# ziyaad30/ForwardTacotron

Hardware: AMD Instinct MI355X
Metric: mel_frames_per_sec_train_step (higher is better)
Workload: dtype f32

## Files before the change

forwardtacotron_amd/csrc/ft_bn.hip:

```cpp
#include <string.h>

#include "ft_common.h"

namespace {

__device__ __forceinline__ int tvalid_of(int c, int Tbuf, int group) {
  return (group > 0 && (((c / group) + 1) & 1)) ? Tbuf - 1 : Tbuf;
}

struct BnAff4 { float4 mu, rs, ga, be; };
__device__ __forceinline__ float4 bn_z4(const float4& v, const BnAff4& a) {
  float4 o;
  o.x = (v.x - a.mu.x) * a.rs.x * a.ga.x + a.be.x;
  o.y = (v.y - a.mu.y) * a.rs.y * a.ga.y + a.be.y;
  o.z = (v.z - a.mu.z) * a.rs.z * a.ga.z + a.be.z;
  o.w = (v.w - a.mu.w) * a.rs.w * a.ga.w + a.be.w;
  return o;
}
__device__ __forceinline__ float4 pool_grad4(const float* __restrict__ yrow, const float* __restrict__ drow,
                                             const float4& vt, int t, int Tout, int C, const BnAff4& a) {
  const float4 z = bn_z4(vt, a);
  const float4 d0 = *reinterpret_cast<const float4*>(drow);
  float4 g;
  if (t == 0) {
    g = d0;
  } else {
    const float4 p = bn_z4(*reinterpret_cast<const float4*>(yrow - C), a);
    g.x = z.x > p.x ? d0.x : 0.f;
    g.y = z.y > p.y ? d0.y : 0.f;
    g.z = z.z > p.z ? d0.z : 0.f;
    g.w = z.w > p.w ? d0.w : 0.f;
  }
  if (t + 1 < Tout) {
    const float4 n = bn_z4(*reinterpret_cast<const float4*>(yrow + C), a);
    const float4 d1 = *reinterpret_cast<const float4*>(drow + C);
    g.x += !(n.x > z.x) ? d1.x : 0.f;
    g.y += !(n.y > z.y) ? d1.y : 0.f;
    g.z += !(n.z > z.z) ? d1.z : 0.f;
    g.w += !(n.w > z.w) ? d1.w : 0.f;
  }
  return g;
}

template <int MODE>
__global__ __launch_bounds__(256) void ft_col_partial_kernel(const float* __restrict__ y, long ldy,
                                                             const float* __restrict__ dout,
                                                             const float* __restrict__ mean,
                                                             const float* __restrict__ rstd, int B, int Tbuf, int Tout,
                                                             int C, int group, int rows_per_chunk,
                                                             double* __restrict__ partial) {
  __shared__ double red[2][4][64];
  const int cl = threadIdx.x & 63, rl = threadIdx.x >> 6;
  const int c = blockIdx.x * 64 + cl;
  const long rows = (long)B * Tbuf;
  long r0 = (long)blockIdx.y * rows_per_chunk;
  long r1 = r0 + rows_per_chunk;
  if (r1 > rows) r1 = rows;
  double s0 = 0.0, s1 = 0.0;
  if (c < C) {
    const int tv = tvalid_of(c, Tbuf, group);
    float mu = 0.f, rs = 0.f;
    if (MODE == 1) {
      mu = mean[c];
      rs = rstd[c];
    }
    long r = r0 + rl;
    int b = (int)(r / Tbuf);
    int t = (int)(r - (long)b * Tbuf);
    for (; r < r1; r += 4) {
      if (t < tv) {
        float v = y[r * ldy + c];
        if (MODE == 0) {
          s0 += (double)v;
          s1 += (double)v * (double)v;
        } else if (MODE == 1) {
          if (t < Tout) {
            float g = dout[((long)b * Tout + t) * C + c];
            s0 += (double)g;
            s1 += (double)g * (double)((v - mu) * rs);
          }
        } else {
          s0 += (double)v;
        }
      }
      t += 4;
      while (t >= Tbuf) {
        t -= Tbuf;
        ++b;
      }
    }
  }
  red[0][rl][cl] = s0;
  red[1][rl][cl] = s1;
  __syncthreads();
  if (rl == 0 && c < C) {
    double a0 = red[0][0][cl] + red[0][1][cl] + red[0][2][cl] + red[0][3][cl];
    double a1 = red[1][0][cl] + red[1][1][cl] + red[1][2][cl] + red[1][3][cl];
    partial[((long)blockIdx.y * C + c) * 2 + 0] = a0;
    partial[((long)blockIdx.y * C + c) * 2 + 1] = a1;
  }
}

__global__ __launch_bounds__(256) void ft_colsum4_partial_kernel(const float* __restrict__ x, long ldx, long rows, int C,
                                                                 int rows_per_chunk, double* __restrict__ partial,
                                                                 const float* __restrict__ x1) {
  if (x1) {
    if (blockIdx.z == 1) x = x1;
  }
  const int slot = x1 ? (int)blockIdx.z : 0;
  __shared__ double red[16][65];
  const int cq = threadIdx.x & 15, rl = threadIdx.x >> 4;
  const int c = blockIdx.x * 64 + cq * 4;
  const long r0 = (long)blockIdx.y * rows_per_chunk;
  long r1 = r0 + rows_per_chunk;
  if (r1 > rows) r1 = rows;
  double s[4] = {0.0, 0.0, 0.0, 0.0};
  if (c < C) {
    for (long r = r0 + rl; r < r1; r += 64) {
      float4 v[4];
#pragma unroll
      for (int u = 0; u < 4; ++u) {
        const long rr = r + 16 * u;
        v[u] = rr < r1 ? *reinterpret_cast<const float4*>(x + rr * ldx + c) : make_float4(0.f, 0.f, 0.f, 0.f);
      }
#pragma unroll
      for (int u = 0; u < 4; ++u) {
        s[0] += (double)v[u].x;
        s[1] += (double)v[u].y;
        s[2] += (double)v[u].z;
        s[3] += (double)v[u].w;
      }
    }
  }
#pragma unroll
  for (int e = 0; e < 4; ++e) red[rl][cq * 4 + e] = s[e];
  __syncthreads();
  if (threadIdx.x < 64) {
    const int cc = blockIdx.x * 64 + threadIdx.x;
    if (cc < C) {
      double a = 0.0;
#pragma unroll
      for (int i = 0; i < 16; ++i) a += red[i][threadIdx.x];
      partial[((long)blockIdx.y * C + cc) * 2 + slot] = a;
      if (!x1) partial[((long)blockIdx.y * C + cc) * 2 + 1] = 0.0;
    }
  }
}

template <int MODE>
__global__ __launch_bounds__(256) void ft_col_partial4_kernel(const float* __restrict__ y, const float* __restrict__ dout,
                                                              const float* __restrict__ mean,
                                                              const float* __restrict__ rstd, int B, int Tbuf, int Tout,
                                                              int C, int group, int rows_per_chunk,
                                                              double* __restrict__ partial,
                                                              const float* __restrict__ gamma = nullptr,
                                                              const float* __restrict__ beta = nullptr) {
  __shared__ double red[2][16][65];
  const int cq = threadIdx.x & 15, rl = threadIdx.x >> 4;
  const int c = blockIdx.x * 64 + cq * 4;
  const long rows = (long)B * Tbuf;
  const long r0 = (long)blockIdx.y * rows_per_chunk;
  long r1 = r0 + rows_per_chunk;
  if (r1 > rows) r1 = rows;
  double s0[4] = {0.0, 0.0, 0.0, 0.0}, s1[4] = {0.0, 0.0, 0.0, 0.0};
  if (c < C) {
    const int tv = tvalid_of(c, Tbuf, group);
    float4 mu = make_float4(0.f, 0.f, 0.f, 0.f), rs = mu;
    BnAff4 aff;
    if (MODE >= 1) {
      mu = *reinterpret_cast<const float4*>(mean + c);
      rs = *reinterpret_cast<const float4*>(rstd + c);
    }
    if (MODE == 2) {
      aff.mu = mu;
      aff.rs = rs;
      aff.ga = *reinterpret_cast<const float4*>(gamma + c);
      aff.be = *reinterpret_cast<const float4*>(beta + c);
    }
    int bb[4], tt[4];
#pragma unroll
    for (int u = 0; u < 4; ++u) {
      const long r = r0 + rl + 16 * u;
      bb[u] = (int)(r / Tbuf);
      tt[u] = (int)(r - (long)bb[u] * Tbuf);
    }
    for (long r = r0 + rl; r < r1; r += 64) {
      float4 v[4], g[4];
      bool ok[4];
#pragma unroll
      for (int u = 0; u < 4; ++u) {
        const long rr = r + 16 * u;
        ok[u] = rr < r1 && tt[u] < tv && (MODE == 0 || tt[u] < Tout);
        v[u] = ok[u] ? *reinterpret_cast<const float4*>(y + rr * C + c) : make_float4(0.f, 0.f, 0.f, 0.f);
        if (MODE == 1)
          g[u] = ok[u] ? *reinterpret_cast<const float4*>(dout + ((long)bb[u] * Tout + tt[u]) * C + c)
                       : make_float4(0.f, 0.f, 0.f, 0.f);
        if (MODE == 2)
          g[u] = ok[u] ? pool_grad4(y + rr * C + c, dout + ((long)bb[u] * Tout + tt[u]) * C + c, v[u], tt[u], Tout, C, aff)
                       : make_float4(0.f, 0.f, 0.f, 0.f);
      }
#pragma unroll
      for (int u = 0; u < 4; ++u) {
        if (MODE == 0) {
          s0[0] += (double)v[u].x; s1[0] += (double)v[u].x * (double)v[u].x;
          s0[1] += (double)v[u].y; s1[1] += (double)v[u].y * (double)v[u].y;
          s0[2] += (double)v[u].z; s1[2] += (double)v[u].z * (double)v[u].z;
          s0[3] += (double)v[u].w; s1[3] += (double)v[u].w * (double)v[u].w;
        } else if (ok[u]) {
          s0[0] += (double)g[u].x; s1[0] += (double)g[u].x * (double)((v[u].x - mu.x) * rs.x);
          s0[1] += (double)g[u].y; s1[1] += (double)g[u].y * (double)((v[u].y - mu.y) * rs.y);
          s0[2] += (double)g[u].z; s1[2] += (double)g[u].z * (double)((v[u].z - mu.z) * rs.z);
          s0[3] += (double)g[u].w; s1[3] += (double)g[u].w * (double)((v[u].w - mu.w) * rs.w);
        }
        tt[u] += 64;
        while (tt[u] >= Tbuf) {
          tt[u] -= Tbuf;
          ++bb[u];
        }
      }
    }
  }
#pragma unroll
  for (int e = 0; e < 4; ++e) {
    red[0][rl][cq * 4 + e] = s0[e];
    red[1][rl][cq * 4 + e] = s1[e];
  }
  __syncthreads();
  if (threadIdx.x < 64) {
    const int cc = blockIdx.x * 64 + threadIdx.x;
    if (cc < C) {
      double a0 = 0.0, a1 = 0.0;
#pragma unroll
      for (int i = 0; i < 16; ++i) {
        a0 += red[0][i][threadIdx.x];
        a1 += red[1][i][threadIdx.x];
      }
      partial[((long)blockIdx.y * C + cc) * 2 + 0] = a0;
      partial[((long)blockIdx.y * C + cc) * 2 + 1] = a1;
    }
  }
}

constexpr int FIN_PARTS = 8;
__device__ __forceinline__ void sum_partials(const double* __restrict__ partial, int nchunks, int C, int c, int part,
                                             double (*sh)[FIN_PARTS][2], int slot, double& s0, double& s1) {
  double a0 = 0.0, a1 = 0.0;
  if (c < C) {
    const int per = (nchunks + FIN_PARTS - 1) / FIN_PARTS;
    const int i0 = part * per, i1 = min(nchunks, i0 + per);
    for (int i = i0; i < i1; ++i) {
      a0 += partial[((long)i * C + c) * 2 + 0];
      a1 += partial[((long)i * C + c) * 2 + 1];
    }
  }
  sh[slot][part][0] = a0;
  sh[slot][part][1] = a1;
  __syncthreads();
  s0 = 0.0;
  s1 = 0.0;
  if (part == 0) {
#pragma unroll
    for (int p = 0; p < FIN_PARTS; ++p) {
      s0 += sh[slot][p][0];
      s1 += sh[slot][p][1];
    }
  }
}

__global__ __launch_bounds__(256) void ft_bn_finalize_kernel(const double* __restrict__ partial, int nchunks, int B,
                                                             int Tbuf, int C, int group, float momentum, float eps,
                                                             float* __restrict__ running_mean,
                                                             float* __restrict__ running_var, long* __restrict__ nbt,
                                                             float* __restrict__ save_mean,
                                                             float* __restrict__ save_rstd) {
  __shared__ double sh[32][FIN_PARTS][2];
  const int slot = threadIdx.x >> 3, part = threadIdx.x & 7;
  const int c = blockIdx.x * 32 + slot;
  if (blockIdx.x == 0 && threadIdx.x == 0 && nbt) *nbt += 1;
  double s0, s1;
  sum_partials(partial, nchunks, C, c, part, sh, slot, s0, s1);
  if (part != 0 || c >= C) return;
  double n = (double)B * (double)tvalid_of(c, Tbuf, group);
  double mu = s0 / n;
  double var = s1 / n - mu * mu;
  if (var < 0.0) var = 0.0;
  save_mean[c] = (float)mu;
  save_rstd[c] = (float)(1.0 / sqrt(var + (double)eps));
  if (running_mean) {
    double unb = n > 1.0 ? var * n / (n - 1.0) : var;
    running_mean[c] = (float)((1.0 - momentum) * (double)running_mean[c] + momentum * mu);
    running_var[c] = (float)((1.0 - momentum) * (double)running_var[c] + momentum * unb);
  }
}

__global__ __launch_bounds__(256) void ft_col_finalize_kernel(const double* __restrict__ partial, int nchunks, int C,
                                                              float* __restrict__ out0, float* __restrict__ out1,
                                                              float scale0, int accumulate) {
  __shared__ double sh[32][FIN_PARTS][2];
  const int slot = threadIdx.x >> 3, part = threadIdx.x & 7;
  const int c = blockIdx.x * 32 + slot;
  double s0, s1;
  sum_partials(partial, nchunks, C, c, part, sh, slot, s0, s1);
  if (part != 0 || c >= C) return;
  if (out0) out0[c] = (accumulate ? out0[c] : 0.f) + (float)(s0 * scale0);
  if (out1) out1[c] = (accumulate ? out1[c] : 0.f) + (float)s1;
}

__global__ __launch_bounds__(256) void ft_bn_apply_kernel(const float* __restrict__ y, const float* __restrict__ mean,
                                                          const float* __restrict__ rstd,
                                                          const float* __restrict__ gamma,
                                                          const float* __restrict__ beta,
                                                          const float* __restrict__ residual, float* __restrict__ out,
                                                          int B, int Tbuf, int Tout, int C) {
  long idx = (long)blockIdx.x * blockDim.x + threadIdx.x;
  long total = (long)B * Tout * C;
  if (idx >= total) return;
  int c = (int)(idx % C);
  long row = idx / C;
  int b = (int)(row / Tout), t = (int)(row - (long)b * Tout);
  float v = y[((long)b * Tbuf + t) * C + c];
  float o = (v - mean[c]) * rstd[c] * gamma[c] + beta[c];
  if (residual) o += residual[idx];
  out[idx] = o;
}

__global__ __launch_bounds__(256) void ft_bn_bwd_apply_kernel(const float* __restrict__ dout, const float* __restrict__ y,
                                                              const float* __restrict__ mean,
                                                              const float* __restrict__ rstd,
                                                              const float* __restrict__ gamma,
                                                              const float* __restrict__ dgamma,
                                                              const float* __restrict__ dbeta, float* __restrict__ dy,
                                                              int B, int Tbuf, int Tout, int C, int group, int relu) {
  long idx = (long)blockIdx.x * blockDim.x + threadIdx.x;
  long total = (long)B * Tbuf * C;
  if (idx >= total) return;
  int c = (int)(idx % C);
  long row = idx / C;
  int b = (int)(row / Tbuf), t = (int)(row - (long)b * Tbuf);
  int tv = tvalid_of(c, Tbuf, group);
  float r = 0.f;
  if (t < tv) {
    float v = y[idx];
    float g = t < Tout ? dout[((long)b * Tout + t) * C + c] : 0.f;
    float inv_n = 1.0f / ((float)B * (float)tv);
    float xh = (v - mean[c]) * rstd[c];
    r = gamma[c] * rstd[c] * (g - dbeta[c] * inv_n - xh * dgamma[c] * inv_n);
    if (relu && !(v > 0.f)) r = 0.f;
  }
  dy[idx] = r;
}

__global__ __launch_bounds__(256) void ft_bn_apply4_kernel(const float4* __restrict__ y, const float4* __restrict__ mean,
                                                           const float4* __restrict__ rstd,
                                                           const float4* __restrict__ gamma,
                                                           const float4* __restrict__ beta,
                                                           const float4* __restrict__ residual, float4* __restrict__ out,
                                                           long total4, int Tbuf, int Tout, int C4) {
  const long idx = (long)blockIdx.x * blockDim.x + threadIdx.x;
  if (idx >= total4) return;
  const int c = (int)(idx % C4);
  const long row = idx / C4;
  const int b = (int)(row / Tout), t = (int)(row - (long)b * Tout);
  const float4 v = y[((long)b * Tbuf + t) * C4 + c];
  const float4 mu = mean[c], rs = rstd[c], ga = gamma[c], be = beta[c];
  float4 o;
  o.x = (v.x - mu.x) * rs.x * ga.x + be.x;
  o.y = (v.y - mu.y) * rs.y * ga.y + be.y;
  o.z = (v.z - mu.z) * rs.z * ga.z + be.z;
  o.w = (v.w - mu.w) * rs.w * ga.w + be.w;
  if (residual) {
    const float4 r = residual[idx];
    o.x += r.x; o.y += r.y; o.z += r.z; o.w += r.w;
  }
  out[idx] = o;
}

__global__ __launch_bounds__(256) void ft_bn_apply_pool4_kernel(const float* __restrict__ y, const float* __restrict__ mean,
                                                                const float* __restrict__ rstd,
                                                                const float* __restrict__ gamma,
                                                                const float* __restrict__ beta, float4* __restrict__ out,
                                                                long total4, int Tbuf, int Tout, int C) {
  const long idx = (long)blockIdx.x * blockDim.x + threadIdx.x;
  if (idx >= total4) return;
  const int C4 = C / 4;
  const int c = (int)(idx % C4) * 4;
  const long row = idx / C4;
  const int b = (int)(row / Tout), t = (int)(row - (long)b * Tout);
  BnAff4 a;
  a.mu = *reinterpret_cast<const float4*>(mean + c);
  a.rs = *reinterpret_cast<const float4*>(rstd + c);
  a.ga = *reinterpret_cast<const float4*>(gamma + c);
  a.be = *reinterpret_cast<const float4*>(beta + c);
  const float* yrow = y + ((long)b * Tbuf + t) * C + c;
  float4 z = bn_z4(*reinterpret_cast<const float4*>(yrow), a);
  if (t > 0) {
    const float4 p = bn_z4(*reinterpret_cast<const float4*>(yrow - C), a);
    z.x = z.x > p.x ? z.x : p.x;
    z.y = z.y > p.y ? z.y : p.y;
    z.z = z.z > p.z ? z.z : p.z;
    z.w = z.w > p.w ? z.w : p.w;
  }
  out[idx] = z;
}

template <bool POOL>
__global__ __launch_bounds__(256) void ft_bn_bwd_apply4_kernel(const float4* __restrict__ dout, const float4* __restrict__ y,
                                                               const float4* __restrict__ mean,
                                                               const float4* __restrict__ rstd,
                                                               const float4* __restrict__ gamma,
                                                               const float4* __restrict__ dgamma,
                                                               const float4* __restrict__ dbeta, float4* __restrict__ dy,
                                                               long total4, int B, int Tbuf, int Tout, int C4, int group,
                                                               int relu, const float4* __restrict__ beta = nullptr) {
  const long idx = (long)blockIdx.x * blockDim.x + threadIdx.x;
  if (idx >= total4) return;
  const int c = (int)(idx % C4);
  const long row = idx / C4;
  const int b = (int)(row / Tbuf), t = (int)(row - (long)b * Tbuf);
  const int tv = tvalid_of(4 * c, Tbuf, group);
  float4 r = make_float4(0.f, 0.f, 0.f, 0.f);
  if (t < tv) {
    const float4 v = y[idx];
    const float4 mu = mean[c], rs = rstd[c], ga = gamma[c], dg = dgamma[c], db = dbeta[c];
    float4 g = make_float4(0.f, 0.f, 0.f, 0.f);
    if (t < Tout) {
      if constexpr (POOL) {
        BnAff4 a;
        a.mu = mu; a.rs = rs; a.ga = ga; a.be = beta[c];
        g = pool_grad4(reinterpret_cast<const float*>(y + idx), reinterpret_cast<const float*>(dout + ((long)b * Tout + t) * C4 + c),
                       v, t, Tout, 4 * C4, a);
      } else {
        g = dout[((long)b * Tout + t) * C4 + c];
      }
    }
    const float inv_n = 1.0f / ((float)B * (float)tv);
#define FT_BN_BWD1(f)                                                                \
  {                                                                                  \
    const float xh = (v.f - mu.f) * rs.f;                                            \
    r.f = ga.f * rs.f * (g.f - db.f * inv_n - xh * dg.f * inv_n);                    \
    if (relu && !(v.f > 0.f)) r.f = 0.f;                                             \
  }
    FT_BN_BWD1(x) FT_BN_BWD1(y) FT_BN_BWD1(z) FT_BN_BWD1(w)
#undef FT_BN_BWD1
  }
  dy[idx] = r;
}

__global__ void ft_bn_fold_kernel(const float* gamma, const float* beta, const float* rm, const float* rv, float eps,
                                  float* scale, float* shift, int C) {
  int c = blockIdx.x * blockDim.x + threadIdx.x;
  if (c >= C) return;
  float s = gamma[c] / sqrtf(rv[c] + eps);
  scale[c] = s;
  shift[c] = beta[c] - rm[c] * s;
}

template <typename... P>
bool all16(P... ptrs) {
  return (((uintptr_t)(const void*)ptrs % 16 == 0) && ...);
}

constexpr int CSB_MAX = 16;
struct ColsumBatch {
  const float* x[CSB_MAX];
  float* out[CSB_MAX];
  long ld[CSB_MAX], ws_off[CSB_MAX];
  int C[CSB_MAX], nchunks[CSB_MAX], rpc[CSB_MAX];
  int tile64[CSB_MAX + 1], tile32[CSB_MAX + 1];
  int n;
  long rows;
};

__global__ __launch_bounds__(256) void ft_colsum_batch_partial_kernel(ColsumBatch b, double* __restrict__ ws) {
  int t = 0;
  while (t + 1 < b.n && (int)blockIdx.x >= b.tile64[t + 1]) ++t;
  if ((int)blockIdx.y >= b.nchunks[t]) return;
  const float* __restrict__ x = b.x[t];
  const long ldx = b.ld[t];
  const int C = b.C[t];
  double* __restrict__ partial = ws + b.ws_off[t];
  __shared__ double red[16][65];
  const int cq = threadIdx.x & 15, rl = threadIdx.x >> 4;
  const int tile = blockIdx.x - b.tile64[t];
  const int c = tile * 64 + cq * 4;
  const long r0 = (long)blockIdx.y * b.rpc[t];
  long r1 = r0 + b.rpc[t];
  if (r1 > b.rows) r1 = b.rows;
  double s[4] = {0.0, 0.0, 0.0, 0.0};
  if (c < C) {
    for (long r = r0 + rl; r < r1; r += 64) {
      float4 v[4];
#pragma unroll
      for (int u = 0; u < 4; ++u) {
        const long rr = r + 16 * u;
        v[u] = rr < r1 ? *reinterpret_cast<const float4*>(x + rr * ldx + c) : make_float4(0.f, 0.f, 0.f, 0.f);
      }
#pragma unroll
      for (int u = 0; u < 4; ++u) {
        s[0] += (double)v[u].x;
        s[1] += (double)v[u].y;
        s[2] += (double)v[u].z;
        s[3] += (double)v[u].w;
      }
    }
  }
#pragma unroll
  for (int e = 0; e < 4; ++e) red[rl][cq * 4 + e] = s[e];
  __syncthreads();
  if (threadIdx.x < 64) {
    const int cc = tile * 64 + threadIdx.x;
    if (cc < C) {
      double a = 0.0;
#pragma unroll
      for (int i = 0; i < 16; ++i) a += red[i][threadIdx.x];
      partial[((long)blockIdx.y * C + cc) * 2] = a;
      partial[((long)blockIdx.y * C + cc) * 2 + 1] = 0.0;
    }
  }
}

__global__ __launch_bounds__(256) void ft_colsum_batch_finalize_kernel(ColsumBatch b, const double* __restrict__ ws) {
  int t = 0;
  while (t + 1 < b.n && (int)blockIdx.x >= b.tile32[t + 1]) ++t;
  __shared__ double sh[32][FIN_PARTS][2];
  const int slot = threadIdx.x >> 3, part = threadIdx.x & 7;
  const int c = (blockIdx.x - b.tile32[t]) * 32 + slot;
  double s0, s1;
  sum_partials(ws + b.ws_off[t], b.nchunks[t], b.C[t], c, part, sh, slot, s0, s1);
  if (part != 0 || c >= b.C[t]) return;
  b.out[t][c] = (float)s0;
}

struct ChunkPlan {
  int nchunks, rows_per_chunk;
};
ChunkPlan plan_chunks(long rows, int C) {
  int cb = ft_cdiv(C, 64);
  long want = 1024 / (cb > 0 ? cb : 1);
  if (want < 16) want = 16;
  if (want > 64) want = 64;
  long maxc = (rows + 63) / 64;
  if (maxc < 1) maxc = 1;
  long n = want < maxc ? want : maxc;
  if (n > 65535) n = 65535;
  long rpc = (rows + n - 1) / n;
  rpc = ((rpc + 3) / 4) * 4;
  if (rpc < 4) rpc = 4;
  n = (rows + rpc - 1) / rpc;
  if (n < 1) n = 1;
  ChunkPlan p = {(int)n, (int)rpc};
  return p;
}

}

int ft_bn_stat_partials(const float* y, int B, int Tbuf, int C, int group, double* partial, hipStream_t s) {
  ChunkPlan p = plan_chunks((long)B * Tbuf, C);
  if (C % 4 == 0 && (group == 0 || group % 4 == 0) && all16(y))
    hipLaunchKernelGGL(ft_col_partial4_kernel<0>, dim3(ft_cdiv(C, 64), p.nchunks), dim3(256), 0, s, y, nullptr, nullptr,
                       nullptr, B, Tbuf, Tbuf, C, group, p.rows_per_chunk, partial);
  else
    hipLaunchKernelGGL(ft_col_partial_kernel<0>, dim3(ft_cdiv(C, 64), p.nchunks), dim3(256), 0, s, y, (long)C, nullptr,
                       nullptr, nullptr, B, Tbuf, Tbuf, C, group, p.rows_per_chunk, partial);
  return p.nchunks;
}

extern "C" {

size_t ft_bn_workspace(int B, int Tbuf, int C);

size_t ft_conv_stats_workspace(int B, int Tbuf, int C) {
  const size_t tiles = (size_t)ft_cdiv((long)B * Tbuf, 128) * C * 2 * sizeof(double);
  const size_t chunks = ft_bn_workspace(B, Tbuf, C);
  return tiles > chunks ? tiles : chunks;
}

int ft_bn_train_from_partials(const double* partial, int nchunks, const float* y, const float* gamma, const float* beta,
                              const float* residual, float* out, float* running_mean, float* running_var,
                              long* num_batches_tracked, float* save_mean, float* save_rstd, int B, int Tbuf, int Tout,
                              int C, int group, float momentum, float eps, void* stream) {
  FT_REQUIRE(B > 0 && Tbuf > 0 && C > 0 && Tout <= Tbuf && nchunks >= 1, "bn_train_from_partials: bad dims");
  hipStream_t s = (hipStream_t)stream;
  hipLaunchKernelGGL(ft_bn_finalize_kernel, dim3(ft_cdiv(C, 32)), dim3(256), 0, s, partial, nchunks, B, Tbuf, C, group,
                     momentum, eps, running_mean, running_var, num_batches_tracked, save_mean, save_rstd);
  if (out && Tout > 0) {
    long total = (long)B * Tout * C;
    if (C % 4 == 0 && all16(y, save_mean, save_rstd, gamma, beta, residual, out))
      hipLaunchKernelGGL(ft_bn_apply4_kernel, dim3(ft_cdiv(total / 4, 256)), dim3(256), 0, s, (const float4*)y,
                         (const float4*)save_mean, (const float4*)save_rstd, (const float4*)gamma, (const float4*)beta,
                         (const float4*)residual, (float4*)out, total / 4, Tbuf, Tout, C / 4);
    else
      hipLaunchKernelGGL(ft_bn_apply_kernel, dim3(ft_cdiv(total, 256)), dim3(256), 0, s, y, save_mean, save_rstd, gamma,
                         beta, residual, out, B, Tbuf, Tout, C);
  }
  return ft_check_launch("bn_train_from_partials");
}

size_t ft_bn_workspace(int B, int Tbuf, int C) {
  ChunkPlan p = plan_chunks((long)B * Tbuf, C);
  return (size_t)p.nchunks * C * 2 * sizeof(double);
}

int ft_bn_train_fwd(const float* y, const float* gamma, const float* beta, const float* residual, float* out,
                    float* running_mean, float* running_var, long* num_batches_tracked, float* save_mean,
                    float* save_rstd, int B, int Tbuf, int Tout, int C, int group, float momentum, float eps,
                    void* workspace, size_t workspace_bytes, void* stream) {
  FT_REQUIRE(B > 0 && Tbuf > 0 && C > 0 && Tout <= Tbuf, "bn_train_fwd: bad dims");
  FT_REQUIRE(workspace && workspace_bytes >= ft_bn_workspace(B, Tbuf, C), "bn_train_fwd: workspace too small");
  hipStream_t s = (hipStream_t)stream;
  ChunkPlan p = plan_chunks((long)B * Tbuf, C);
  if (C % 4 == 0 && (group == 0 || group % 4 == 0) && all16(y))
    hipLaunchKernelGGL(ft_col_partial4_kernel<0>, dim3(ft_cdiv(C, 64), p.nchunks), dim3(256), 0, s, y, nullptr, nullptr,
                       nullptr, B, Tbuf, Tout, C, group, p.rows_per_chunk, (double*)workspace);
  else
    hipLaunchKernelGGL(ft_col_partial_kernel<0>, dim3(ft_cdiv(C, 64), p.nchunks), dim3(256), 0, s, y, (long)C, nullptr,
                       nullptr, nullptr, B, Tbuf, Tout, C, group, p.rows_per_chunk, (double*)workspace);
  hipLaunchKernelGGL(ft_bn_finalize_kernel, dim3(ft_cdiv(C, 32)), dim3(256), 0, s, (const double*)workspace,
                     p.nchunks, B, Tbuf, C, group, momentum, eps, running_mean, running_var, num_batches_tracked,
                     save_mean, save_rstd);
  if (out && Tout > 0) {
    long total = (long)B * Tout * C;
    if (C % 4 == 0 && all16(y, save_mean, save_rstd, gamma, beta, residual, out))
      hipLaunchKernelGGL(ft_bn_apply4_kernel, dim3(ft_cdiv(total / 4, 256)), dim3(256), 0, s, (const float4*)y,
                         (const float4*)save_mean, (const float4*)save_rstd, (const float4*)gamma, (const float4*)beta,
                         (const float4*)residual, (float4*)out, total / 4, Tbuf, Tout, C / 4);
    else
      hipLaunchKernelGGL(ft_bn_apply_kernel, dim3(ft_cdiv(total, 256)), dim3(256), 0, s, y, save_mean, save_rstd, gamma,
                         beta, residual, out, B, Tbuf, Tout, C);
  }
  return ft_check_launch("bn_train_fwd");
}

int ft_bn_bwd(const float* dout, const float* y, const float* gamma, const float* save_mean, const float* save_rstd,
              float* dy, float* dgamma, float* dbeta, int B, int Tbuf, int Tout, int C, int group, int relu,
              void* workspace, size_t workspace_bytes, void* stream) {
  FT_REQUIRE(B > 0 && Tbuf > 0 && C > 0 && Tout <= Tbuf, "bn_bwd: bad dims");
  FT_REQUIRE(workspace && workspace_bytes >= ft_bn_workspace(B, Tbuf, C), "bn_bwd: workspace too small");
  hipStream_t s = (hipStream_t)stream;
  ChunkPlan p = plan_chunks((long)B * Tbuf, C);
  if (C % 4 == 0 && (group == 0 || group % 4 == 0) && all16(y, dout, save_mean, save_rstd))
    hipLaunchKernelGGL(ft_col_partial4_kernel<1>, dim3(ft_cdiv(C, 64), p.nchunks), dim3(256), 0, s, y, dout, save_mean,
                       save_rstd, B, Tbuf, Tout, C, group, p.rows_per_chunk, (double*)workspace);
  else
    hipLaunchKernelGGL(ft_col_partial_kernel<1>, dim3(ft_cdiv(C, 64), p.nchunks), dim3(256), 0, s, y, (long)C, dout,
                       save_mean, save_rstd, B, Tbuf, Tout, C, group, p.rows_per_chunk, (double*)workspace);
  hipLaunchKernelGGL(ft_col_finalize_kernel, dim3(ft_cdiv(C, 32)), dim3(256), 0, s, (const double*)workspace,
                     p.nchunks, C, dbeta, dgamma, 1.0f, 0);
  long total = (long)B * Tbuf * C;
  if (C % 4 == 0 && (group == 0 || group % 4 == 0) && all16(dout, y, save_mean, save_rstd, gamma, dgamma, dbeta, dy))
    hipLaunchKernelGGL(ft_bn_bwd_apply4_kernel<false>, dim3(ft_cdiv(total / 4, 256)), dim3(256), 0, s, (const float4*)dout,
                       (const float4*)y, (const float4*)save_mean, (const float4*)save_rstd, (const float4*)gamma,
                       (const float4*)dgamma, (const float4*)dbeta, (float4*)dy, total / 4, B, Tbuf, Tout, C / 4, group,
                       relu, nullptr);
  else
    hipLaunchKernelGGL(ft_bn_bwd_apply_kernel, dim3(ft_cdiv(total, 256)), dim3(256), 0, s, dout, y, save_mean, save_rstd,
                       gamma, dgamma, dbeta, dy, B, Tbuf, Tout, C, group, relu);
  return ft_check_launch("bn_bwd");
}

int ft_bn_pool_from_partials(const double* partial, int nchunks, const float* y, const float* gamma, const float* beta,
                             float* out, float* running_mean, float* running_var, long* num_batches_tracked,
                             float* save_mean, float* save_rstd, int B, int Tbuf, int Tout, int C, int group,
                             float momentum, float eps, void* stream) {
  FT_REQUIRE(B > 0 && Tbuf > 0 && C > 0 && Tout > 0 && Tout <= Tbuf && nchunks >= 1, "bn_pool_from_partials: bad dims");
  FT_REQUIRE(C % 4 == 0 && (group == 0 || group % 4 == 0) && all16(y, save_mean, save_rstd, gamma, beta, out),
             "bn_pool_from_partials: needs C %% 4 == 0 and 16-byte aligned buffers");
  hipStream_t s = (hipStream_t)stream;
  hipLaunchKernelGGL(ft_bn_finalize_kernel, dim3(ft_cdiv(C, 32)), dim3(256), 0, s, partial, nchunks, B, Tbuf, C, group,
                     momentum, eps, running_mean, running_var, num_batches_tracked, save_mean, save_rstd);
  const long total = (long)B * Tout * C;
  hipLaunchKernelGGL(ft_bn_apply_pool4_kernel, dim3(ft_cdiv(total / 4, 256)), dim3(256), 0, s, y, save_mean, save_rstd,
                     gamma, beta, (float4*)out, total / 4, Tbuf, Tout, C);
  return ft_check_launch("bn_pool_from_partials");
}

int ft_bn_pool_bwd(const float* dout, const float* y, const float* gamma, const float* beta, const float* save_mean,
                   const float* save_rstd, float* dy, float* dgamma, float* dbeta, int B, int Tbuf, int Tout, int C,
                   int group, int relu, void* workspace, size_t workspace_bytes, void* stream) {
  FT_REQUIRE(B > 0 && Tbuf > 0 && C > 0 && Tout > 0 && Tout <= Tbuf, "bn_pool_bwd: bad dims");
  FT_REQUIRE(workspace && workspace_bytes >= ft_bn_workspace(B, Tbuf, C), "bn_pool_bwd: workspace too small");
  FT_REQUIRE(C % 4 == 0 && (group == 0 || group % 4 == 0) &&
                 all16(dout, y, save_mean, save_rstd, gamma, beta, dgamma, dbeta, dy),
             "bn_pool_bwd: needs C %% 4 == 0 and 16-byte aligned buffers");
  hipStream_t s = (hipStream_t)stream;
  ChunkPlan p = plan_chunks((long)B * Tbuf, C);
  hipLaunchKernelGGL(ft_col_partial4_kernel<2>, dim3(ft_cdiv(C, 64), p.nchunks), dim3(256), 0, s, y, dout, save_mean,
                     save_rstd, B, Tbuf, Tout, C, group, p.rows_per_chunk, (double*)workspace, gamma, beta);
  hipLaunchKernelGGL(ft_col_finalize_kernel, dim3(ft_cdiv(C, 32)), dim3(256), 0, s, (const double*)workspace,
                     p.nchunks, C, dbeta, dgamma, 1.0f, 0);
  const long total = (long)B * Tbuf * C;
  hipLaunchKernelGGL(ft_bn_bwd_apply4_kernel<true>, dim3(ft_cdiv(total / 4, 256)), dim3(256), 0, s, (const float4*)dout,
                     (const float4*)y, (const float4*)save_mean, (const float4*)save_rstd, (const float4*)gamma,
                     (const float4*)dgamma, (const float4*)dbeta, (float4*)dy, total / 4, B, Tbuf, Tout, C / 4, group, relu,
                     (const float4*)beta);
  return ft_check_launch("bn_pool_bwd");
}

int ft_bn_fold_eval(const float* gamma, const float* beta, const float* running_mean, const float* running_var,
                    float eps, float* scale, float* shift, int C, void* stream) {
  if (C <= 0) return FT_OK;
  hipLaunchKernelGGL(ft_bn_fold_kernel, dim3(ft_cdiv(C, 128)), dim3(128), 0, (hipStream_t)stream, gamma, beta,
                     running_mean, running_var, eps, scale, shift, C);
  return ft_check_launch("bn_fold_eval");
}

size_t ft_colsum_workspace(int rows, int C) { return ft_bn_workspace(1, rows > 0 ? rows : 1, C > 0 ? C : 1); }

int ft_colsum(const float* x, long ldx, float* out, int rows, int C, float scale, int accumulate, void* workspace,
              size_t workspace_bytes, void* stream) {
  FT_REQUIRE(rows >= 0 && C >= 0, "colsum: bad dims");
  if (C == 0) return FT_OK;
  hipStream_t s = (hipStream_t)stream;
  if (rows == 0) {
    if (!accumulate) (void)hipMemsetAsync(out, 0, sizeof(float) * C, s);
    return FT_OK;
  }
  FT_REQUIRE(workspace && workspace_bytes >= ft_colsum_workspace(rows, C), "colsum: workspace too small");
  ChunkPlan p = plan_chunks(rows, C);
  if (C % 4 == 0 && ldx % 4 == 0 && ((uintptr_t)x) % 16 == 0)
    hipLaunchKernelGGL(ft_colsum4_partial_kernel, dim3(ft_cdiv(C, 64), p.nchunks), dim3(256), 0, s, x, ldx, (long)rows, C,
                       p.rows_per_chunk, (double*)workspace, (const float*)nullptr);
  else
    hipLaunchKernelGGL(ft_col_partial_kernel<2>, dim3(ft_cdiv(C, 64), p.nchunks), dim3(256), 0, s, x, ldx, nullptr,
                       nullptr, nullptr, 1, rows, rows, C, 0, p.rows_per_chunk, (double*)workspace);
  hipLaunchKernelGGL(ft_col_finalize_kernel, dim3(ft_cdiv(C, 32)), dim3(256), 0, s, (const double*)workspace,
                     p.nchunks, C, out, nullptr, scale, accumulate);
  return ft_check_launch("colsum");
}

int ft_colsum2(const float* x0, const float* x1, long ldx, float* out0, float* out1, int rows, int C, void* workspace,
               size_t workspace_bytes, void* stream) {
  FT_REQUIRE(rows >= 0 && C >= 0, "colsum2: bad dims");
  if (C == 0) return FT_OK;
  const bool vec = C % 4 == 0 && ldx % 4 == 0 && ((uintptr_t)x0) % 16 == 0 && ((uintptr_t)x1) % 16 == 0;
  if (rows == 0 || !vec) {
    int rc = ft_colsum(x0, ldx, out0, rows, C, 1.0f, 0, workspace, workspace_bytes, stream);
    return rc ? rc : ft_colsum(x1, ldx, out1, rows, C, 1.0f, 0, workspace, workspace_bytes, stream);
  }
  hipStream_t s = (hipStream_t)stream;
  FT_REQUIRE(workspace && workspace_bytes >= ft_colsum_workspace(rows, C), "colsum2: workspace too small");
  ChunkPlan p = plan_chunks(rows, C);
  hipLaunchKernelGGL(ft_colsum4_partial_kernel, dim3(ft_cdiv(C, 64), p.nchunks, 2), dim3(256), 0, s, x0, ldx, (long)rows,
                     C, p.rows_per_chunk, (double*)workspace, x1);
  hipLaunchKernelGGL(ft_col_finalize_kernel, dim3(ft_cdiv(C, 32)), dim3(256), 0, s, (const double*)workspace,
                     p.nchunks, C, out0, out1, 1.0f, 0);
  return ft_check_launch("colsum2");
}

size_t ft_colsum_batch_workspace(int n, const int* C, int rows) {
  size_t total = 0;
  for (int i = 0; i < n; ++i) total += ft_colsum_workspace(rows, C[i]);
  return total;
}

int ft_colsum_batch(int n, const float* const* x, const long* ld, float* const* out, const int* C, int rows,
                    void* workspace, size_t workspace_bytes, void* stream) {
  FT_REQUIRE(n >= 0 && n <= CSB_MAX && rows >= 0, "colsum_batch: n = %d (max %d), rows = %d", n, CSB_MAX, rows);
  if (n == 0) return FT_OK;
  bool vec = rows > 0;
  for (int i = 0; i < n; ++i)
    vec = vec && C[i] > 0 && C[i] % 4 == 0 && ld[i] % 4 == 0 && ((uintptr_t)x[i]) % 16 == 0;
  if (!vec) {
    for (int i = 0; i < n; ++i) {
      const int rc = ft_colsum(x[i], ld[i], out[i], rows, C[i], 1.0f, 0, workspace, workspace_bytes, stream);
      if (rc) return rc;
    }
    return FT_OK;
  }
  FT_REQUIRE(workspace && workspace_bytes >= ft_colsum_batch_workspace(n, C, rows), "colsum_batch: workspace too small");
  ColsumBatch b;
  memset(&b, 0, sizeof(b));
  b.n = n;
  b.rows = rows;
  long off = 0;
  int maxchunks = 1;
  for (int i = 0; i < n; ++i) {
    const ChunkPlan p = plan_chunks(rows, C[i]);
    b.x[i] = x[i]; b.out[i] = out[i]; b.ld[i] = ld[i]; b.C[i] = C[i];
    b.nchunks[i] = p.nchunks; b.rpc[i] = p.rows_per_chunk;
    b.ws_off[i] = off;
    off += (long)(ft_colsum_workspace(rows, C[i]) / sizeof(double));
    b.tile64[i + 1] = b.tile64[i] + ft_cdiv(C[i], 64);
    b.tile32[i + 1] = b.tile32[i] + ft_cdiv(C[i], 32);
    if (p.nchunks > maxchunks) maxchunks = p.nchunks;
  }
  hipStream_t s = (hipStream_t)stream;
  hipLaunchKernelGGL(ft_colsum_batch_partial_kernel, dim3(b.tile64[n], maxchunks), dim3(256), 0, s, b, (double*)workspace);
  hipLaunchKernelGGL(ft_colsum_batch_finalize_kernel, dim3(b.tile32[n]), dim3(256), 0, s, b, (const double*)workspace);
  return ft_check_launch("colsum_batch");
}

}
```

forwardtacotron_amd/csrc/ft_elementwise.hip:

```cpp
#include "ft_common.h"
#include "../../include/fwdtaco_hip.h"

namespace {

__global__ void ft_pack_conv_w_kernel(const float* __restrict__ w, float* __restrict__ wp, int Cout, int Cin, int k) {
  long idx = (long)blockIdx.x * blockDim.x + threadIdx.x;
  long total = (long)Cout * Cin * k;
  if (idx >= total) return;
  int j = (int)(idx / ((long)Cout * Cin));
  long rem = idx - (long)j * Cout * Cin;
  wp[idx] = w[rem * k + j];
}

__global__ void ft_pack_conv_wt_kernel(const float* __restrict__ w, float* __restrict__ wpt, int Cout, int Cin, int k) {
  long idx = (long)blockIdx.x * blockDim.x + threadIdx.x;
  long total = (long)Cout * Cin * k;
  if (idx >= total) return;
  int j = (int)(idx / ((long)Cout * Cin));
  long rem = idx - (long)j * Cout * Cin;
  int ci = (int)(rem / Cout), co = (int)(rem - (long)ci * Cout);
  wpt[idx] = w[((long)co * Cin + ci) * k + j];
}

__global__ __launch_bounds__(256) void ft_pack_weights_kernel(const FtPackDesc* __restrict__ descs, int n) {
  __shared__ float tile[32][33];
  const long bid = blockIdx.x;
  int lo = 0, hi = n - 1;
  while (lo < hi) {
    int mid = (lo + hi + 1) >> 1;
    if (descs[mid].tile_begin <= bid) lo = mid; else hi = mid - 1;
  }
  const FtPackDesc d = descs[lo];
  long t = bid - d.tile_begin;
  const int n1 = (d.d1 + 31) >> 5, n0 = (d.d0 + 31) >> 5;
  const int j1 = (int)(t % n1);
  t /= n1;
  const int j0 = (int)(t % n0), a = (int)(t / n0);
  if (a >= d.k) return;
  const int tx = threadIdx.x & 31, ty = threadIdx.x >> 5;
  const int c1 = j1 * 32 + tx;
  float v[4];
#pragma unroll
  for (int r = 0; r < 4; ++r) {
    int c0 = j0 * 32 + ty + 8 * r;
    v[r] = (c0 < d.d0 && c1 < d.d1) ? d.src[((long)c0 * d.d1 + c1) * d.k + a] : 0.f;
  }
  if (d.dst) {
#pragma unroll
    for (int r = 0; r < 4; ++r) {
      int c0 = j0 * 32 + ty + 8 * r;
      if (c0 < d.d0 && c1 < d.d1) d.dst[((long)a * d.d0 + c0) * d.d1 + c1] = v[r];
    }
  }
  if (d.dst_t) {
#pragma unroll
    for (int r = 0; r < 4; ++r) tile[ty + 8 * r][tx] = v[r];
    __syncthreads();
    const int o0 = j0 * 32 + tx;
#pragma unroll
    for (int r = 0; r < 4; ++r) {
      int o1 = j1 * 32 + ty + 8 * r;
      if (o1 < d.d1 && o0 < d.d0) d.dst_t[((long)a * d.d1 + o1) * d.d0 + o0] = tile[tx][ty + 8 * r];
    }
  }
}

struct FtSegs {
  const float* src[64];
  float* dst[64];
  long len[64];
};
__global__ __launch_bounds__(256) void ft_copy_segments_kernel(FtSegs sg) {
  const float* s = sg.src[blockIdx.x];
  float* d = sg.dst[blockIdx.x];
  const long n = sg.len[blockIdx.x];
  for (long i = threadIdx.x; i < n; i += 256) d[i] = s[i];
}

__global__ void ft_dropout_kernel(const float* __restrict__ x, float* __restrict__ out, long n, float p,
                                  uint64_t seed) {
  long i = (long)blockIdx.x * blockDim.x + threadIdx.x;
  if (i >= n) return;
  out[i] = ft_dropout_keep(seed, i, p) ? x[i] / (1.0f - p) : 0.f;
}
__global__ void ft_scale_kernel(const float* __restrict__ x, float* __restrict__ out, long n, float s) {
  long i = (long)blockIdx.x * blockDim.x + threadIdx.x;
  if (i < n) out[i] = x[i] * s;
}

__global__ void ft_embedding_fwd_kernel(const long* __restrict__ idx, const float* __restrict__ w,
                                        float* __restrict__ out, long rows, int C, int V, int* __restrict__ err) {
  long i = (long)blockIdx.x * blockDim.x + threadIdx.x;
  if (i >= rows * C) return;
  long r = i / C;
  int c = (int)(i - r * C);
  long v = idx[r];
  if (v < 0 || v >= V) {
    if (c == 0) atomicExch(err, 1);
    out[i] = 0.f;
    return;
  }
  out[i] = w[v * C + c];
}

__global__ void ft_onehot_kernel(const long* __restrict__ idx, float* __restrict__ out, long rows, int V) {
  long i = (long)blockIdx.x * blockDim.x + threadIdx.x;
  if (i >= rows * V) return;
  long r = i / V;
  int v = (int)(i - r * V);
  out[i] = idx[r] == v ? 1.f : 0.f;
}

__global__ void ft_highway_fwd_kernel(const float* __restrict__ x12, const float* __restrict__ x,
                                      float* __restrict__ out, long rows, int C) {
  long i = (long)blockIdx.x * blockDim.x + threadIdx.x;
  if (i >= rows * C) return;
  long r = i / C;
  int c = (int)(i - r * C);
  float x1 = x12[r * 2 * C + c], x2 = x12[r * 2 * C + C + c];
  float g = ft_sigmoid(x2);
  out[i] = g * fmaxf(x1, 0.f) + (1.f - g) * x[i];
}

__global__ void ft_highway_bwd_kernel(const float* __restrict__ dout, const float* __restrict__ x12,
                                      const float* __restrict__ x, float* __restrict__ d12,
                                      float* __restrict__ dx, long rows, int C) {
  long i = (long)blockIdx.x * blockDim.x + threadIdx.x;
  if (i >= rows * C) return;
  long r = i / C;
  int c = (int)(i - r * C);
  float x1 = x12[r * 2 * C + c], x2 = x12[r * 2 * C + C + c];
  float g = ft_sigmoid(x2);
  float d = dout[i];
  float rx1 = fmaxf(x1, 0.f);
  d12[r * 2 * C + c] = x1 > 0.f ? d * g : 0.f;
  d12[r * 2 * C + C + c] = d * (rx1 - x[i]) * g * (1.f - g);
  dx[i] = d * (1.f - g);
}

__global__ void ft_highway_pack_kernel(const float* __restrict__ w1, const float* __restrict__ w2,
                                       float* __restrict__ out, int C) {
  long i = (long)blockIdx.x * blockDim.x + threadIdx.x;
  if (i >= 2L * C * C) return;
  const int n = (int)(i / C), k = (int)(i - (long)n * C);
  const int unit = (n >> 6) * 32 + (n & 31);
  out[i] = ((n & 63) >> 5 ? w2 : w1)[(long)unit * C + k];
}

__global__ void ft_maxpool_fwd_kernel(const float* __restrict__ x, float* __restrict__ out, int B, int T, int C) {
  long i = (long)blockIdx.x * blockDim.x + threadIdx.x;
  long total = (long)B * T * C;
  if (i >= total) return;
  long row = i / C;
  int t = (int)(row % T);
  float v = x[i];
  if (t > 0) {
    float p = x[i - C];
    v = v > p ? v : p;
  }
  out[i] = v;
}
__global__ __launch_bounds__(256) void ft_maxpool_fwd4_kernel(const float4* __restrict__ x, float4* __restrict__ out,
                                                              long total4, int T, int C4) {
  const long i = (long)blockIdx.x * blockDim.x + threadIdx.x;
  if (i >= total4) return;
  const long row = i / C4;
  const int t = (int)(row % T);
  float4 v = x[i];
  if (t > 0) {
    const float4 p = x[i - C4];
    v.x = v.x > p.x ? v.x : p.x;
    v.y = v.y > p.y ? v.y : p.y;
    v.z = v.z > p.z ? v.z : p.z;
    v.w = v.w > p.w ? v.w : p.w;
  }
  out[i] = v;
}
__global__ void ft_maxpool_bwd_kernel(const float* __restrict__ dout, const float* __restrict__ x,
                                      float* __restrict__ dx, int B, int T, int C) {
  long i = (long)blockIdx.x * blockDim.x + threadIdx.x;
  long total = (long)B * T * C;
  if (i >= total) return;
  long row = i / C;
  int t = (int)(row % T);
  float v = x[i];
  float g = 0.f;
  if (t == 0 || v > x[i - C]) g += dout[i];
  if (t + 1 < T && !(x[i + C] > v)) g += dout[i + C];
  dx[i] = g;
}
__global__ __launch_bounds__(256) void ft_maxpool_bwd4_kernel(const float4* __restrict__ dout,
                                                              const float4* __restrict__ x, float4* __restrict__ dx,
                                                              long total4, int T, int C4) {
  const long i = (long)blockIdx.x * blockDim.x + threadIdx.x;
  if (i >= total4) return;
  const long row = i / C4;
  const int t = (int)(row % T);
  const float4 v = x[i];
  const float4 d0 = dout[i];
  float4 g = make_float4(0.f, 0.f, 0.f, 0.f);
  if (t == 0) {
    g = d0;
  } else {
    const float4 p = x[i - C4];
    g.x = v.x > p.x ? d0.x : 0.f;
    g.y = v.y > p.y ? d0.y : 0.f;
    g.z = v.z > p.z ? d0.z : 0.f;
    g.w = v.w > p.w ? d0.w : 0.f;
  }
  if (t + 1 < T) {
    const float4 n = x[i + C4];
    const float4 d1 = dout[i + C4];
    g.x += !(n.x > v.x) ? d1.x : 0.f;
    g.y += !(n.y > v.y) ? d1.y : 0.f;
    g.z += !(n.z > v.z) ? d1.z : 0.f;
    g.w += !(n.w > v.w) ? d1.w : 0.f;
  }
  dx[i] = g;
}

__global__ void ft_cond_add_kernel(const float* __restrict__ x, const float* __restrict__ pitch,
                                   const float* __restrict__ energy, const float* __restrict__ wp,
                                   const float* __restrict__ bp, const float* __restrict__ we,
                                   const float* __restrict__ be, float sp, float se, float* __restrict__ out, int B,
                                   int T, int C, int x_time_major) {
  long i = (long)blockIdx.x * blockDim.x + threadIdx.x;
  long total = (long)B * T * C;
  if (i >= total) return;
  int c = (int)(i % C);
  long row = i / C;
  int t = (int)(row % T);
  const float xv = x_time_major ? x[((long)t * B + (row / T)) * C + c] : x[i];
  const float* p = pitch + row;
  const float* e = energy + row;
  float pm = t > 0 ? p[-1] : 0.f, pc = p[0], pn = t + 1 < T ? p[1] : 0.f;
  float em = t > 0 ? e[-1] : 0.f, ec = e[0], en = t + 1 < T ? e[1] : 0.f;
  float a = bp[c] + wp[c * 3 + 0] * pm + wp[c * 3 + 1] * pc + wp[c * 3 + 2] * pn;
  float b = be[c] + we[c * 3 + 0] * em + we[c * 3 + 1] * ec + we[c * 3 + 2] * en;
  out[i] = xv + sp * a + se * b;
}
__global__ void ft_cond_taps_kernel(const float* __restrict__ pitch, const float* __restrict__ energy,
                                    float* __restrict__ P, int B, int T) {
  long row = (long)blockIdx.x * blockDim.x + threadIdx.x;
  if (row >= (long)B * T) return;
  int t = (int)(row % T);
  const float* p = pitch + row;
  const float* e = energy + row;
  float* o = P + row * 8;
  o[0] = t > 0 ? p[-1] : 0.f; o[1] = p[0]; o[2] = t + 1 < T ? p[1] : 0.f; o[3] = 1.f;
  o[4] = t > 0 ? e[-1] : 0.f; o[5] = e[0]; o[6] = t + 1 < T ? e[1] : 0.f; o[7] = 1.f;
}

__global__ void ft_concat_cols_kernel(const float* __restrict__ a, int Ca, const float* __restrict__ b2, int Cb,
                                      const float* __restrict__ semb, int S, float* __restrict__ out, int B, int T,
                                      int a_time_major) {
  const int C = Ca + Cb + S;
  long i = (long)blockIdx.x * blockDim.x + threadIdx.x;
  long total = (long)B * T * C;
  if (i >= total) return;
  long row = i / C;
  int c = (int)(i - row * C);
  int b = (int)(row / T), t = (int)(row - (long)b * T);
  float v;
  if (c < Ca) v = a[(a_time_major ? ((long)t * B + b) : row) * Ca + c];
  else if (c < Ca + Cb) v = b2[row * Cb + (c - Ca)];
  else v = semb[(long)b * S + (c - Ca - Cb)];
  out[i] = v;
}
__global__ void ft_slice_cols_kernel(const float* __restrict__ src, long ld, int col0, int C,
                                     float* __restrict__ dst, int B, int T, int dst_time_major) {
  long i = (long)blockIdx.x * blockDim.x + threadIdx.x;
  long total = (long)B * T * C;
  if (i >= total) return;
  long row = i / C;
  int c = (int)(i - row * C);
  long srow = row;
  if (dst_time_major) {
    int t = (int)(row / B), b = (int)(row - (long)t * B);
    srow = (long)b * T + t;
  }
  dst[i] = src[srow * ld + col0 + c];
}

__global__ __launch_bounds__(256) void ft_ce_partial_kernel(const float* __restrict__ logits,
                                                            const long* __restrict__ target, long rows, int K,
                                                            long ignore, double* __restrict__ partial) {
  __shared__ double red[2][4];
  double s = 0.0, n = 0.0;
  for (long r = (long)blockIdx.x * 256 + threadIdx.x; r < rows; r += (long)gridDim.x * 256) {
    long tg = target[r];
    if (tg == ignore || tg < 0 || tg >= K) continue;
    const float* l = logits + r * K;
    float mx = l[0];
    for (int k = 1; k < K; ++k) mx = fmaxf(mx, l[k]);
    float se = 0.f;
    for (int k = 0; k < K; ++k) se += expf(l[k] - mx);
    s += (double)(logf(se) + mx - l[tg]);
    n += 1.0;
  }
  s = ft_wave_sum_d(s);
  n = ft_wave_sum_d(n);
  if ((threadIdx.x & 63) == 0) {
    red[0][threadIdx.x >> 6] = s;
    red[1][threadIdx.x >> 6] = n;
  }
  __syncthreads();
  if (threadIdx.x == 0) {
    partial[2 * blockIdx.x] = red[0][0] + red[0][1] + red[0][2] + red[0][3];
    partial[2 * blockIdx.x + 1] = red[1][0] + red[1][1] + red[1][2] + red[1][3];
  }
}
__global__ void ft_ce_finalize_kernel(const double* __restrict__ partial, int nblocks, float* __restrict__ loss,
                                      float* __restrict__ inv_count) {
  if (threadIdx.x != 0 || blockIdx.x != 0) return;
  double s = 0.0, n = 0.0;
  for (int i = 0; i < nblocks; ++i) {
    s += partial[2 * i];
    n += partial[2 * i + 1];
  }
  *loss = (float)(s / n);
  *inv_count = (float)(1.0 / n);
}
__global__ void ft_ce_bwd_kernel(const float* __restrict__ logits, const long* __restrict__ target,
                                 const float* __restrict__ inv_count, const float* __restrict__ gout,
                                 float* __restrict__ dlogits, long rows, int K, long ignore) {
  long r = (long)blockIdx.x * blockDim.x + threadIdx.x;
  if (r >= rows) return;
  long tg = target[r];
  const float* l = logits + r * K;
  float* d = dlogits + r * K;
  if (tg == ignore || tg < 0 || tg >= K) {
    for (int k = 0; k < K; ++k) d[k] = 0.f;
    return;
  }
  float mx = l[0];
  for (int k = 1; k < K; ++k) mx = fmaxf(mx, l[k]);
  float se = 0.f;
  for (int k = 0; k < K; ++k) se += expf(l[k] - mx);
  const float sc = inv_count[0] * (gout ? gout[0] : 1.f);
  for (int k = 0; k < K; ++k) d[k] = (expf(l[k] - mx) / se - (k == tg ? 1.f : 0.f)) * sc;
}

__global__ __launch_bounds__(256) void ft_transpose_pad_kernel(const float* __restrict__ x, float* __restrict__ out,
                                                               int T, int C, int Tout, float pad) {
  __shared__ float tile[32][33];
  const int b = blockIdx.z;
  const int t0 = blockIdx.x * 32, c0 = blockIdx.y * 32;
  const int tx = threadIdx.x & 31, ty = threadIdx.x >> 5;
  for (int i = ty; i < 32; i += 8) {
    int t = t0 + i, c = c0 + tx;
    tile[i][tx] = (t < T && c < C) ? x[((long)b * T + t) * C + c] : pad;
  }
  __syncthreads();
  for (int i = ty; i < 32; i += 8) {
    int c = c0 + i, t = t0 + tx;
    if (c < C && t < Tout) out[((long)b * C + c) * Tout + t] = tile[tx][i];
  }
}
__global__ __launch_bounds__(256) void ft_transpose_pad_bwd_kernel(const float* __restrict__ dout, float* __restrict__ dx,
                                                                   int T, int C, int Tout) {
  __shared__ float tile[32][33];
  const int b = blockIdx.z;
  const int t0 = blockIdx.x * 32, c0 = blockIdx.y * 32;
  const int tx = threadIdx.x & 31, ty = threadIdx.x >> 5;
  for (int i = ty; i < 32; i += 8) {
    int c = c0 + i, t = t0 + tx;
    tile[i][tx] = (c < C && t < Tout) ? dout[((long)b * C + c) * Tout + t] : 0.f;
  }
  __syncthreads();
  for (int i = ty; i < 32; i += 8) {
    int t = t0 + i, c = c0 + tx;
    if (t < T && c < C) dx[((long)b * T + t) * C + c] = tile[tx][i];
  }
}

__global__ __launch_bounds__(256) void ft_masked_l1_partial_kernel(const float* __restrict__ x,
                                                                   const float* __restrict__ target,
                                                                   const long* __restrict__ lens, int B, int C, int T,
                                                                   double* __restrict__ partial) {
  __shared__ double red[4];
  long total = (long)B * C * T;
  double acc = 0.0;
  for (long i = (long)blockIdx.x * 256 + threadIdx.x; i < total; i += (long)gridDim.x * 256) {
    int t = (int)(i % T);
    int b = (int)(i / ((long)C * T));
    if (t < lens[b]) acc += (double)fabsf(x[i] - target[i]);
  }
  acc = ft_wave_sum_d(acc);
  if ((threadIdx.x & 63) == 0) red[threadIdx.x >> 6] = acc;
  __syncthreads();
  if (threadIdx.x == 0) partial[blockIdx.x] = red[0] + red[1] + red[2] + red[3];
}
__global__ __launch_bounds__(256) void ft_masked_l1_finalize_kernel(const double* __restrict__ partial, int nblocks,
                                                                    const long* __restrict__ lens, int B, int C,
                                                                    int T, float* __restrict__ loss,
                                                                    float* __restrict__ inv_denom) {
  __shared__ double red[2][4];
  double s = 0.0, n = 0.0;
  for (int i = threadIdx.x; i < nblocks; i += 256) s += partial[i];
  for (int b = threadIdx.x; b < B; b += 256) {
    long l = lens[b];
    if (l < 0) l = 0;
    if (l > T) l = T;
    n += (double)l;
  }
  s = ft_wave_sum_d(s);
  n = ft_wave_sum_d(n);
  if ((threadIdx.x & 63) == 0) {
    red[0][threadIdx.x >> 6] = s;
    red[1][threadIdx.x >> 6] = n;
  }
  __syncthreads();
  if (threadIdx.x != 0) return;
  s = red[0][0] + red[0][1] + red[0][2] + red[0][3];
  n = red[1][0] + red[1][1] + red[1][2] + red[1][3];
  n *= (double)C;
  *loss = (float)(s / n);
  *inv_denom = (float)(1.0 / n);
}
__global__ void ft_masked_l1_bwd_kernel(const float* __restrict__ x, const float* __restrict__ target,
                                        const long* __restrict__ lens, const float* __restrict__ inv_denom,
                                        const float* __restrict__ gout, float factor, float* __restrict__ dx, int B,
                                        int C, int T) {
  long i = (long)blockIdx.x * blockDim.x + threadIdx.x;
  long total = (long)B * C * T;
  if (i >= total) return;
  int t = (int)(i % T);
  int b = (int)(i / ((long)C * T));
  float g = 0.f;
  if (t < lens[b]) {
    float d = x[i] - target[i];
    float s = d > 0.f ? 1.f : (d < 0.f ? -1.f : 0.f);
    g = s * inv_denom[0] * (gout ? gout[0] : 1.f) * factor;
  }
  dx[i] = g;
}

}

extern "C" {

int ft_conv_pack_weight(const float* w, float* wp, int Cout, int Cin, int k, void* stream) {
  FT_REQUIRE(Cout >= 0 && Cin >= 0 && k >= 1, "conv_pack_weight: bad dims");
  long total = (long)Cout * Cin * k;
  if (total == 0) return FT_OK;
  hipLaunchKernelGGL(ft_pack_conv_w_kernel, dim3(ft_cdiv(total, 256)), dim3(256), 0, (hipStream_t)stream, w, wp, Cout,
                     Cin, k);
  return ft_check_launch("conv_pack_weight");
}

int ft_conv_pack_weight_t(const float* w, float* wpt, int Cout, int Cin, int k, void* stream) {
  FT_REQUIRE(Cout >= 0 && Cin >= 0 && k >= 1, "conv_pack_weight_t: bad dims");
  long total = (long)Cout * Cin * k;
  if (total == 0) return FT_OK;
  hipLaunchKernelGGL(ft_pack_conv_wt_kernel, dim3(ft_cdiv(total, 256)), dim3(256), 0, (hipStream_t)stream, w, wpt,
                     Cout, Cin, k);
  return ft_check_launch("conv_pack_weight_t");
}

int ft_pack_weights(const FtPackDesc* descs, int n, long total_tiles, void* stream) {
  FT_REQUIRE(n >= 0 && total_tiles >= 0 && total_tiles < (1L << 31), "pack_weights: bad sizes");
  if (n == 0 || total_tiles == 0) return FT_OK;
  FT_REQUIRE(descs != nullptr, "pack_weights: null descriptor array");
  hipLaunchKernelGGL(ft_pack_weights_kernel, dim3((unsigned)total_tiles), dim3(256), 0, (hipStream_t)stream, descs, n);
  return ft_check_launch("pack_weights");
}

int ft_copy_segments(const float* const* src, float* const* dst, const long* len, int n, void* stream) {
  FT_REQUIRE(n >= 0 && n <= 64, "copy_segments: n=%d (max 64)", n);
  if (n == 0) return FT_OK;
  FtSegs sg;
  for (int i = 0; i < n; ++i) {
    FT_REQUIRE(len[i] >= 0 && (len[i] == 0 || (src[i] && dst[i])), "copy_segments: bad segment %d", i);
    sg.src[i] = src[i];
    sg.dst[i] = dst[i];
    sg.len[i] = len[i];
  }
  hipLaunchKernelGGL(ft_copy_segments_kernel, dim3(n), dim3(256), 0, (hipStream_t)stream, sg);
  return ft_check_launch("copy_segments");
}

int ft_dropout(const float* x, float* out, long n, float p, uint64_t seed, void* stream) {
  FT_REQUIRE(p >= 0.f && p < 1.f, "dropout: p must be in [0,1)");
  if (n <= 0) return FT_OK;
  hipLaunchKernelGGL(ft_dropout_kernel, dim3(ft_cdiv(n, 256)), dim3(256), 0, (hipStream_t)stream, x, out, n, p, seed);
  return ft_check_launch("dropout");
}

int ft_scale(const float* x, float* out, long n, float s, void* stream) {
  if (n <= 0) return FT_OK;
  hipLaunchKernelGGL(ft_scale_kernel, dim3(ft_cdiv(n, 256)), dim3(256), 0, (hipStream_t)stream, x, out, n, s);
  return ft_check_launch("scale");
}

int ft_embedding_fwd(const long* idx, const float* w, float* out, long rows, int C, int V, int* err_flag,
                     void* stream) {
  FT_REQUIRE(rows >= 0 && C >= 0 && V > 0, "embedding_fwd: bad dims");
  if (rows * C == 0) return FT_OK;
  hipLaunchKernelGGL(ft_embedding_fwd_kernel, dim3(ft_cdiv(rows * C, 256)), dim3(256), 0, (hipStream_t)stream, idx, w,
                     out, rows, C, V, err_flag);
  return ft_check_launch("embedding_fwd");
}

int ft_onehot(const long* idx, float* out, long rows, int V, void* stream) {
  FT_REQUIRE(rows >= 0 && V > 0, "onehot: bad dims");
  if (rows == 0) return FT_OK;
  hipLaunchKernelGGL(ft_onehot_kernel, dim3(ft_cdiv(rows * V, 256)), dim3(256), 0, (hipStream_t)stream, idx, out, rows,
                     V);
  return ft_check_launch("onehot");
}

int ft_highway_gate_fwd(const float* x12, const float* x, float* out, long rows, int C, void* stream) {
  if (rows * C <= 0) return FT_OK;
  hipLaunchKernelGGL(ft_highway_fwd_kernel, dim3(ft_cdiv(rows * C, 256)), dim3(256), 0, (hipStream_t)stream, x12, x,
                     out, rows, C);
  return ft_check_launch("highway_gate_fwd");
}

int ft_highway_gate_bwd(const float* dout, const float* x12, const float* x, float* d12, float* dx, long rows, int C,
                        void* stream) {
  if (rows * C <= 0) return FT_OK;
  hipLaunchKernelGGL(ft_highway_bwd_kernel, dim3(ft_cdiv(rows * C, 256)), dim3(256), 0, (hipStream_t)stream, dout, x12,
                     x, d12, dx, rows, C);
  return ft_check_launch("highway_gate_bwd");
}

int ft_highway_pack(const float* w1, const float* w2, float* w12i, int C, void* stream) {
  FT_REQUIRE(C > 0 && C % 32 == 0, "highway_pack: the fused highway needs C %% 32 == 0 (C = %d)", C);
  hipLaunchKernelGGL(ft_highway_pack_kernel, dim3(ft_cdiv(2L * C * C, 256)), dim3(256), 0, (hipStream_t)stream, w1, w2,
                     w12i, C);
  return ft_check_launch("highway_pack");
}

int ft_maxpool2_fwd(const float* x, float* out, int B, int T, int C, void* stream) {
  long total = (long)B * T * C;
  if (total <= 0) return FT_OK;
  if (C % 4 == 0 && ((uintptr_t)x % 16) == 0 && ((uintptr_t)out % 16) == 0)
    hipLaunchKernelGGL(ft_maxpool_fwd4_kernel, dim3(ft_cdiv(total / 4, 256)), dim3(256), 0, (hipStream_t)stream,
                       (const float4*)x, (float4*)out, total / 4, T, C / 4);
  else
    hipLaunchKernelGGL(ft_maxpool_fwd_kernel, dim3(ft_cdiv(total, 256)), dim3(256), 0, (hipStream_t)stream, x, out, B,
                       T, C);
  return ft_check_launch("maxpool2_fwd");
}

int ft_maxpool2_bwd(const float* dout, const float* x, float* dx, int B, int T, int C, void* stream) {
  long total = (long)B * T * C;
  if (total <= 0) return FT_OK;
  if (C % 4 == 0 && ((uintptr_t)x % 16) == 0 && ((uintptr_t)dout % 16) == 0 && ((uintptr_t)dx % 16) == 0)
    hipLaunchKernelGGL(ft_maxpool_bwd4_kernel, dim3(ft_cdiv(total / 4, 256)), dim3(256), 0, (hipStream_t)stream,
                       (const float4*)dout, (const float4*)x, (float4*)dx, total / 4, T, C / 4);
  else
    hipLaunchKernelGGL(ft_maxpool_bwd_kernel, dim3(ft_cdiv(total, 256)), dim3(256), 0, (hipStream_t)stream, dout, x,
                       dx, B, T, C);
  return ft_check_launch("maxpool2_bwd");
}

int ft_cond_add_fwd(const float* x, const float* pitch, const float* energy, const float* w_pitch,
                    const float* b_pitch, const float* w_energy, const float* b_energy, float pitch_strength,
                    float energy_strength, float* out, int B, int T, int C, int x_time_major, void* stream) {
  long total = (long)B * T * C;
  if (total <= 0) return FT_OK;
  hipLaunchKernelGGL(ft_cond_add_kernel, dim3(ft_cdiv(total, 256)), dim3(256), 0, (hipStream_t)stream, x, pitch,
                     energy, w_pitch, b_pitch, w_energy, b_energy, pitch_strength, energy_strength, out, B, T, C,
                     x_time_major);
  return ft_check_launch("cond_add_fwd");
}

int ft_cond_taps(const float* pitch, const float* energy, float* taps, int B, int T, void* stream) {
  long rows = (long)B * T;
  if (rows <= 0) return FT_OK;
  hipLaunchKernelGGL(ft_cond_taps_kernel, dim3(ft_cdiv(rows, 256)), dim3(256), 0, (hipStream_t)stream, pitch, energy,
                     taps, B, T);
  return ft_check_launch("cond_taps");
}

int ft_transpose_pad_fwd(const float* x, float* out, int B, int T, int C, int Tout, float pad, void* stream) {
  if (B <= 0 || C <= 0 || Tout <= 0) return FT_OK;
  FT_REQUIRE(B <= 65535 && ft_cdiv(C, 32) <= 65535, "transpose_pad_fwd: grid too large");
  hipLaunchKernelGGL(ft_transpose_pad_kernel, dim3(ft_cdiv(Tout, 32), ft_cdiv(C, 32), B), dim3(256), 0,
                     (hipStream_t)stream, x, out, T, C, Tout, pad);
  return ft_check_launch("transpose_pad_fwd");
}

int ft_transpose_pad_bwd(const float* dout, float* dx, int B, int T, int C, int Tout, void* stream) {
  if (B <= 0 || C <= 0 || T <= 0) return FT_OK;
  FT_REQUIRE(B <= 65535 && ft_cdiv(C, 32) <= 65535, "transpose_pad_bwd: grid too large");
  hipLaunchKernelGGL(ft_transpose_pad_bwd_kernel, dim3(ft_cdiv(T, 32), ft_cdiv(C, 32), B), dim3(256), 0,
                     (hipStream_t)stream, dout, dx, T, C, Tout);
  return ft_check_launch("transpose_pad_bwd");
}

int ft_concat_cols(const float* a, int Ca, const float* b2, int Cb, const float* semb, int S, float* out, int B,
                   int T, int a_time_major, void* stream) {
  FT_REQUIRE(Ca >= 0 && Cb >= 0 && S >= 0 && (Cb == 0 || b2) && (S == 0 || semb), "concat_cols: bad arguments");
  long total = (long)B * T * (Ca + Cb + S);
  if (total <= 0) return FT_OK;
  hipLaunchKernelGGL(ft_concat_cols_kernel, dim3(ft_cdiv(total, 256)), dim3(256), 0, (hipStream_t)stream, a, Ca, b2,
                     Cb, semb, S, out, B, T, a_time_major);
  return ft_check_launch("concat_cols");
}

int ft_slice_cols(const float* src, long ld, int col0, int C, float* dst, int B, int T, int dst_time_major,
                  void* stream) {
  long total = (long)B * T * C;
  if (total <= 0) return FT_OK;
  hipLaunchKernelGGL(ft_slice_cols_kernel, dim3(ft_cdiv(total, 256)), dim3(256), 0, (hipStream_t)stream, src, ld, col0,
                     C, dst, B, T, dst_time_major);
  return ft_check_launch("slice_cols");
}

size_t ft_cross_entropy_workspace(void) { return 2 * 256 * sizeof(double); }

int ft_cross_entropy_fwd(const float* logits, const long* target, long rows, int K, long ignore_index, float* loss,
                         float* inv_count, void* workspace, size_t workspace_bytes, void* stream) {
  FT_REQUIRE(rows > 0 && K > 0, "cross_entropy_fwd: bad dims");
  FT_REQUIRE(workspace && workspace_bytes >= ft_cross_entropy_workspace(), "cross_entropy_fwd: workspace too small");
  int nb = ft_cdiv(rows, 256);
  if (nb > 256) nb = 256;
  hipLaunchKernelGGL(ft_ce_partial_kernel, dim3(nb), dim3(256), 0, (hipStream_t)stream, logits, target, rows, K,
                     ignore_index, (double*)workspace);
  hipLaunchKernelGGL(ft_ce_finalize_kernel, dim3(1), dim3(64), 0, (hipStream_t)stream, (const double*)workspace, nb,
                     loss, inv_count);
  return ft_check_launch("cross_entropy_fwd");
}

int ft_cross_entropy_bwd(const float* logits, const long* target, const float* inv_count, const float* grad_out,
                         float* dlogits, long rows, int K, long ignore_index, void* stream) {
  if (rows <= 0) return FT_OK;
  hipLaunchKernelGGL(ft_ce_bwd_kernel, dim3(ft_cdiv(rows, 256)), dim3(256), 0, (hipStream_t)stream, logits, target,
                     inv_count, grad_out, dlogits, rows, K, ignore_index);
  return ft_check_launch("cross_entropy_bwd");
}

size_t ft_masked_l1_workspace(void) { return 1024 * sizeof(double); }

int ft_masked_l1_fwd(const float* x, const float* target, const long* lens, float* loss, float* inv_denom, int B,
                     int C, int T, void* workspace, size_t workspace_bytes, void* stream) {
  FT_REQUIRE(B > 0 && C > 0 && T > 0, "masked_l1_fwd: bad dims");
  FT_REQUIRE(workspace && workspace_bytes >= ft_masked_l1_workspace(), "masked_l1_fwd: workspace too small");
  long total = (long)B * C * T;
  int nb = ft_cdiv(total, 256 * 8);
  if (nb > 1024) nb = 1024;
  if (nb < 1) nb = 1;
  hipLaunchKernelGGL(ft_masked_l1_partial_kernel, dim3(nb), dim3(256), 0, (hipStream_t)stream, x, target, lens, B, C, T,
                     (double*)workspace);
  hipLaunchKernelGGL(ft_masked_l1_finalize_kernel, dim3(1), dim3(256), 0, (hipStream_t)stream,
                     (const double*)workspace, nb, lens, B, C, T, loss, inv_denom);
  return ft_check_launch("masked_l1_fwd");
}

int ft_masked_l1_bwd(const float* x, const float* target, const long* lens, const float* inv_denom,
                     const float* grad_out, float factor, float* dx, int B, int C, int T, void* stream) {
  long total = (long)B * C * T;
  if (total <= 0) return FT_OK;
  hipLaunchKernelGGL(ft_masked_l1_bwd_kernel, dim3(ft_cdiv(total, 256)), dim3(256), 0, (hipStream_t)stream, x, target,
                     lens, inv_denom, grad_out, factor, dx, B, C, T);
  return ft_check_launch("masked_l1_bwd");
}

}
```

forwardtacotron_amd/fastpitch.py:

```python
import copy
import functools
import math
import os
from pathlib import Path
from typing import Any, Callable, Dict, Optional, Union

import torch
import torch.nn as nn
from torch.autograd import Function

from . import _lib
from . import hip as H
from . import ops
from .model import LengthRegulator, NUM_CHARS_DEFAULT, PAD_VALUE, _dropout, _seed
from .ops import _c, _emit, _emit_multi

_F4 = 4


def _p(t):
    return None if t is None else t.data_ptr()


def _bgemm(kind, A_ptr, lda, sA0, sA1, B_ptr, ldb, sB0, sB1, C_ptr, ldc, sC0, sC1, M, N, K, nb0, nb1, device,
           padded: bool = False):
    if kind == 'tn':
        nbytes = _lib.query('ft_bgemm_tn_workspace', M, N, K, nb0, nb1)
        ws = H.workspace(nbytes, device)
        _lib.call('ft_bgemm_tn', A_ptr, lda, sA0, sA1, B_ptr, ldb, sB0, sB1, C_ptr, ldc, sC0, sC1, M, N, K, nb0, nb1,
                  int(padded), ws.data_ptr(), ws.numel(), H._stream())
    elif kind == 'nn':
        _lib.call('ft_bgemm_nn', A_ptr, lda, sA0, sA1, B_ptr, ldb, sB0, sB1, C_ptr, ldc, sC0, sC1, M, N, K, nb0, nb1,
                  int(padded), H._stream())
    else:
        _lib.call('ft_bgemm_nt', A_ptr, lda, sA0, sA1, B_ptr, ldb, sB0, sB1, C_ptr, ldc, sC0, sC1, M, N, K, nb0, nb1,
                  H._stream())


def precision_scoped(fn):
    @functools.wraps(fn)
    def wrapped(self, *a, **k):
        with H.gemm_precision(getattr(self, 'matmul_dtype', 'fp32')):
            return fn(self, *a, **k)
    return wrapped


def mha_fwd(x, key_pad, in_w, in_b, out_w, out_b, nheads, p_drop, seed):
    B, T, d = x.shape
    nh = int(nheads)
    hd = d // nh
    scale = 1.0 / math.sqrt(hd)
    qkv = H.linear_fwd(x, in_w, in_b)
    tape = dict(x=x, qkv=qkv, key_pad=key_pad, nh=nh, hd=hd, scale=scale, p=float(p_drop), seed=int(seed))
    if H.gemm_precision_mode() == 'bf16' and hd in (64, 128) and os.environ.get('FT_ATTN_FUSED', '1') == '1':
        att, lse2 = H.attn_fwd(qkv, key_pad, nh, scale, p_drop, seed)
        tape.update(fused=True, att=att, lse2=lse2)
        return H.linear_fwd(att, out_w, out_b), tape
    Tp = (T + 3) // 4 * 4
    P = torch.empty(B, nh, T, Tp, device=x.device, dtype=x.dtype)
    q0 = qkv.data_ptr()
    _bgemm('nt', q0, 3 * d, T * 3 * d, hd, q0 + d * _F4, 3 * d, T * 3 * d, hd, P.data_ptr(), Tp, nh * T * Tp, T * Tp,
           T, T, hd, B, nh, x.device)
    Pd = torch.empty_like(P) if p_drop > 0 else P
    _lib.call('ft_softmax_fwd', P.data_ptr(), _p(key_pad), B, nh, T, T, Tp, scale,
              Pd.data_ptr() if p_drop > 0 else None, float(p_drop), int(seed), H._stream())
    att = torch.empty(B, T, d, device=x.device, dtype=x.dtype)
    _bgemm('nn', Pd.data_ptr(), Tp, nh * T * Tp, T * Tp, q0 + 2 * d * _F4, 3 * d, T * 3 * d, hd, att.data_ptr(), d,
           T * d, hd, T, hd, T, B, nh, x.device, padded=True)
    tape.update(fused=False, att=att, P=P, Pd=Pd)
    return H.linear_fwd(att, out_w, out_b), tape


def mha_bwd(tape, dout, in_w, in_b, out_w, out_b, need_dx=True, dx_into=None):
    x, qkv, att, key_pad = tape['x'], tape['qkv'], tape['att'], tape['key_pad']
    nh, hd, scale, p_drop, seed = tape['nh'], tape['hd'], tape['scale'], tape['p'], tape['seed']
    B, T, d = x.shape
    rows = B * T
    dev = x.device
    datt = H.linear_bwd_data(dout, out_w)
    g_ow = _emit(out_w, lambda o: H.linear_bwd_weight_raw(dout.data_ptr(), d, att.data_ptr(), d, o, rows, d, d),
                 (dout, att))
    g_ob = _emit(out_b, lambda o: H.colsum_raw(dout.data_ptr(), d, o, rows, d), (dout,), heavy='light')
    if tape['fused']:
        dqkv = H.attn_bwd(qkv, att, datt, key_pad, tape['lse2'], nh, scale, p_drop, seed)
        g0 = dqkv.data_ptr()
    else:
        P, Pd = tape['P'], tape['Pd']
        q0 = qkv.data_ptr()
        dqkv = torch.empty_like(qkv)
        g0 = dqkv.data_ptr()
        Tp = P.shape[-1]
        dP = torch.empty_like(P)
        _bgemm('nt', datt.data_ptr(), d, T * d, hd, q0 + 2 * d * _F4, 3 * d, T * 3 * d, hd, dP.data_ptr(), Tp,
               nh * T * Tp, T * Tp, T, T, hd, B, nh, dev)
        _bgemm('tn', Pd.data_ptr(), Tp, nh * T * Tp, T * Tp, datt.data_ptr(), d, T * d, hd, g0 + 2 * d * _F4, 3 * d,
               T * 3 * d, hd, T, hd, T, B, nh, dev, padded=True)
        _lib.call('ft_softmax_bwd', P.data_ptr(), dP.data_ptr(), B, nh, T, T, Tp, scale, p_drop, seed, H._stream())
        _bgemm('nn', dP.data_ptr(), Tp, nh * T * Tp, T * Tp, q0 + d * _F4, 3 * d, T * 3 * d, hd, g0, 3 * d, T * 3 * d,
               hd, T, hd, T, B, nh, dev, padded=True)
        _bgemm('tn', dP.data_ptr(), Tp, nh * T * Tp, T * Tp, q0, 3 * d, T * 3 * d, hd, g0 + d * _F4, 3 * d, T * 3 * d,
               hd, T, hd, T, B, nh, dev, padded=True)
    dx = None
    if need_dx:
        dx = H.linear_bwd_data(dqkv, in_w, dx=dx_into, accumulate=dx_into is not None)
    g_iw = _emit(in_w, lambda o: H.linear_bwd_weight_raw(g0, 3 * d, x.data_ptr(), d, o, rows, d, 3 * d), (dqkv, x))
    g_ib = _emit(in_b, lambda o: H.colsum_raw(g0, 3 * d, o, rows, 3 * d), (dqkv,), heavy='light')
    return dx, g_iw, g_ib, g_ow, g_ob


class MHAFn(Function):

    @staticmethod
    def forward(ctx, x, key_pad, in_w, in_b, out_w, out_b, nheads, p_drop, seed):
        out, ctx.tape = mha_fwd(_c(x), key_pad, in_w, in_b, out_w, out_b, nheads, p_drop, seed)
        ctx.params = (in_w, in_b, out_w, out_b)
        return out

    @staticmethod
    def backward(ctx, dout):
        dx, g_iw, g_ib, g_ow, g_ob = mha_bwd(ctx.tape, _c(dout), *ctx.params, need_dx=ctx.needs_input_grad[0])
        ctx.tape = None
        return dx, None, g_iw, g_ib, g_ow, g_ob, None, None, None


def addln_fwd(x, res, gamma, beta, eps, p=0.0, seed=0):
    D = x.shape[-1]
    rows = x.numel() // D
    s = torch.empty_like(x) if res is not None else x
    y = torch.empty_like(x)
    mean = torch.empty(rows, device=x.device, dtype=x.dtype)
    rstd = torch.empty(rows, device=x.device, dtype=x.dtype)
    p = float(p) if res is not None else 0.0
    _lib.call('ft_layernorm_fwd', x.data_ptr(), _p(_c(res) if res is not None else None), gamma.data_ptr(),
              beta.data_ptr(), s.data_ptr() if res is not None else None, y.data_ptr(), mean.data_ptr(),
              rstd.data_ptr(), rows, D, float(eps), p, int(seed), H._stream())
    return y, dict(s=s, mean=mean, rstd=rstd, has_res=res is not None, p=p, seed=int(seed))


def addln_bwd(tape, dy, gamma, beta, own_dres=False):
    s, mean, rstd = tape['s'], tape['mean'], tape['rstd']
    D = s.shape[-1]
    rows = s.numel() // D
    dx = torch.empty_like(s)
    t = torch.empty_like(s)
    dres = torch.empty_like(s) if tape['has_res'] and (tape['p'] > 0 or own_dres) else None
    _lib.call('ft_layernorm_bwd', dy.data_ptr(), s.data_ptr(), gamma.data_ptr(), mean.data_ptr(), rstd.data_ptr(),
              dx.data_ptr(), t.data_ptr(), _p(dres), rows, D, tape['p'], tape['seed'], H._stream())
    dg, db = _emit_multi([gamma, beta], lambda o: H.colsum2_raw(t.data_ptr(), dy.data_ptr(), D, o[0], o[1], rows, D),
                         (t, dy), heavy='light')
    return dx, ((dres if dres is not None else dx) if tape['has_res'] else None), dg, db


def convbias_fwd(x, w, b, relu):
    B, T, Cin = x.shape
    Cout, _, k = w.shape
    wp = H.conv_pack_weight(w)
    y = torch.empty(B, T, Cout, device=x.device, dtype=x.dtype)
    _lib.call('ft_conv1d_bias_fwd', x.data_ptr(), Cin, wp.data_ptr(), b.data_ptr(), y.data_ptr(), Cout, B, T, Cin,
              Cout, k, int(relu), H._stream())
    return y, dict(x=x, wp=wp, y=y if relu else None, relu=bool(relu))


def convbias_bwd(tape, dy, w, b, need_dx=True, dx_into=None):
    x, wp, y = tape['x'], tape['wp'], tape['y']
    B, T, Cin = x.shape
    Cout = w.shape[0]
    if tape['relu']:
        g = torch.empty_like(dy)
        _lib.call('ft_relu_bwd', dy.data_ptr(), y.data_ptr(), g.data_ptr(), dy.numel(), H._stream())
        dy = g
    dx = None
    if need_dx:
        dx = dx_into if dx_into is not None else torch.empty_like(x)
        H.conv1d_bwd_data_raw(dy.data_ptr(), Cout, wp, dx, B, T, T, T, dx_into is not None, w=w)
    dw = _emit(w, lambda o: H.conv1d_bwd_weight_raw(dy.data_ptr(), Cout, x, o, T, T), (dy, x))
    db = _emit(b, lambda o: H.colsum_raw(dy.data_ptr(), Cout, o, B * T, Cout), (dy,), heavy='light')
    return dx, dw, db


class AddLayerNormFn(Function):

    @staticmethod
    def forward(ctx, x, res, gamma, beta, eps, p=0.0, seed=0):
        y, ctx.tape = addln_fwd(_c(x), res, gamma, beta, eps, p, seed)
        ctx.params = (gamma, beta)
        return y

    @staticmethod
    def backward(ctx, dy):
        dx, dres, dg, db = addln_bwd(ctx.tape, _c(dy), *ctx.params)
        ctx.tape = None
        return dx, dres, dg, db, None, None, None


class ConvBiasFn(Function):

    @staticmethod
    def forward(ctx, x, w, b, relu):
        y, ctx.tape = convbias_fwd(_c(x), w, b, relu)
        ctx.params = (w, b)
        return y

    @staticmethod
    def backward(ctx, dy):
        dx, dw, db = convbias_bwd(ctx.tape, _c(dy), *ctx.params, need_dx=ctx.needs_input_grad[0])
        ctx.tape = None
        return dx, dw, db, None


def check_posenc_length(T: int, pe: torch.Tensor) -> None:
    if T > pe.shape[0] or pe.numel() < T * pe.shape[-1]:
        raise _lib.FtError(f'PositionalEncoding: sequence of {T} positions exceeds the pe buffer ({pe.shape[0]})')


class PosEncFn(Function):

    @staticmethod
    def forward(ctx, x, pe, scale):
        x = _c(x)
        B, T, D = x.shape
        check_posenc_length(T, pe)
        out = torch.empty_like(x)
        _lib.call('ft_posenc_fwd', x.data_ptr(), pe.data_ptr(), scale.data_ptr(), out.data_ptr(), B, T, D, H._stream())
        ctx.save_for_backward(pe, scale)
        return out

    @staticmethod
    def backward(ctx, dout):
        pe, scale = ctx.saved_tensors
        dout = _c(dout)
        B, T, D = dout.shape

        def dscale(o):
            ws = H.workspace(_lib.query('ft_posenc_workspace'), dout.device)
            _lib.call('ft_posenc_bwd_scale', dout.data_ptr(), pe.data_ptr(), o.data_ptr(), B, T, D, ws.data_ptr(),
                      ws.numel(), H._stream())

        return dout, None, _emit(scale, dscale, heavy=False)


import ctypes as _ct

_FP = _ct.c_void_p


class _CBlock(_ct.Structure):
    _fields_ = ([(n, _ct.c_int) for n in ('B', 'T', 'd', 'nheads', 'dfft', 'k1', 'k2')]
                + [(n, _ct.c_float) for n in ('p_drop', 'eps1', 'eps2')]
                + [(n, _ct.c_uint64) for n in ('seed_attn', 'seed_ln1', 'seed_ln2')]
                + [(n, _FP) for n in ('key_pad', 'in_w', 'in_b', 'out_w', 'out_b', 'c1_wp', 'c1_b', 'c2_wp', 'c2_b', 'n1_g',
                                      'n1_b', 'n2_g', 'n2_b', 'in_wT', 'out_wT', 'c1_wpt', 'c2_wpt', 'x', 'qkv', 'att',
                                      'lse2', 'sa', 's1', 'mean1', 'rstd1', 'y1', 'h1', 'h2', 's2', 'mean2', 'rstd2', 'y2')])


class _CGrads(_ct.Structure):
    _fields_ = [(n, _FP) for n in ('dy2', 'dx', 't2', 'd_y1', 'd_h2', 'd_h1', 'g_h1', 't1', 'd_h', 'd_sa', 'datt', 'dqkv',
                                   'g_in_w', 'g_in_b', 'g_out_w', 'g_out_b', 'g_c1_w', 'g_c1_b', 'g_c2_w', 'g_c2_b',
                                   'g_n1_g', 'g_n1_b', 'g_n2_g', 'g_n2_b')]


_sums_streams = {}


def _sums_stream(device) -> 'torch.cuda.Stream':
    key = torch.device(device).index or 0
    if key not in _sums_streams:
        _sums_streams[key] = torch.cuda.Stream(device=device, priority=-1)
    return _sums_streams[key]


_GRAD_FIELDS = ('g_in_w', 'g_in_b', 'g_out_w', 'g_out_b', 'g_c1_w', 'g_c1_b', 'g_c2_w', 'g_c2_b', 'g_n1_g', 'g_n1_b', 'g_n2_g',
                'g_n2_b')
_side_ws = {}


def _carve(buf: torch.Tensor, sizes):
    base, off, out, offs = buf.data_ptr(), 0, [], []
    for n in sizes:
        out.append(base + 4 * off)
        offs.append(off)
        off += (n + 3) // 4 * 4
    return out, offs


def _arena(sizes, device):
    return torch.empty(sum((n + 3) // 4 * 4 for n in sizes), device=device, dtype=torch.float32)


def composite_ok(d: int, nheads: int) -> bool:
    return (H.gemm_precision_mode() == 'bf16' and d % nheads == 0 and d // nheads in (64, 128)
            and os.environ.get('FT_ATTN_FUSED', '1') == '1' and os.environ.get('FT_FFT_COMPOSITE', '1') == '1')


def blocks_fwd_composite(h, key_pad, params, nhead, p, eps1, eps2, seeds):
    B, T, d = h.shape
    R = B * T
    n = len(params) // 12
    f = params[4].shape[0]
    k1, k2 = params[4].shape[2], params[6].shape[2]
    sizes = [3 * R * d, R * d, B * nhead * T, R * d, R * d, R, R, R * d, R * f, R * d, R * d, R, R, R * d]
    names = ('qkv', 'att', 'lse2', 'sa', 's1', 'mean1', 'rstd1', 'y1', 'h1', 'h2', 's2', 'mean2', 'rstd2', 'y2')
    blocks = (_CBlock * n)()
    arenas, keep = [], []
    x_ptr = h.data_ptr()
    for i in range(n):
        in_w, in_b, out_w, out_b, c1w, c1b, c2w, c2b, n1g, n1b, n2g, n2b = params[12 * i:12 * i + 12]
        ar = _arena(sizes, h.device)
        arenas.append(ar)
        addr, offs = _carve(ar, sizes)
        ptrs = dict(zip(names, addr))
        y2_off = offs[-1]
        c1p, c2p = H.conv_pack_weight(c1w), H.conv_pack_weight(c2w)
        keep += [c1p, c2p]
        b = blocks[i]
        b.B, b.T, b.d, b.nheads, b.dfft, b.k1, b.k2 = B, T, d, nhead, f, k1, k2
        b.p_drop, b.eps1, b.eps2 = p, eps1, eps2
        b.seed_attn, b.seed_ln1, b.seed_ln2 = seeds[3 * i], seeds[3 * i + 1], seeds[3 * i + 2]
        b.key_pad = _p(key_pad)
        b.in_w, b.in_b, b.out_w, b.out_b = in_w.data_ptr(), in_b.data_ptr(), out_w.data_ptr(), out_b.data_ptr()
        b.c1_wp, b.c1_b, b.c2_wp, b.c2_b = c1p.data_ptr(), c1b.data_ptr(), c2p.data_ptr(), c2b.data_ptr()
        b.n1_g, b.n1_b, b.n2_g, b.n2_b = n1g.data_ptr(), n1b.data_ptr(), n2g.data_ptr(), n2b.data_ptr()
        b.x = x_ptr
        for k_, v_ in ptrs.items():
            setattr(b, k_, v_)
        x_ptr = ptrs['y2']
    _lib.call('ft_fft_blocks_fwd', _ct.byref(blocks), n, H._stream())
    y = arenas[-1][y2_off:y2_off + R * d].view(B, T, d)
    return y, dict(blocks=blocks, arenas=arenas, keep=keep, h=h, key_pad=key_pad, dims=(B, T, d, f, k1, k2, nhead))


def blocks_bwd_composite(state, dy, params):
    blocks = state['blocks']
    B, T, d, f, k1, k2, nhead = state['dims']
    R = B * T
    n = len(params) // 12
    dev = dy.device
    sizes = [R * d, R * d, R * d, R * f, R * f, R * d, R * d, R * d, R * d, 3 * R * d]
    names = ('t2', 'd_y1', 'd_h2', 'd_h1', 'g_h1', 't1', 'd_h', 'd_sa', 'datt', 'dqkv')
    grads = (_CGrads * n)()
    scratch, outs, sunk = [], [None] * (12 * n), []
    sink = ops._SINK
    dy_ptr = dy.data_ptr()
    last_dh = None
    for i in range(n - 1, -1, -1):
        ps = params[12 * i:12 * i + 12]
        b, g = blocks[i], grads[i]
        wit, wot = H.transpose2d(ps[0]), H.transpose2d(ps[2])
        c1t, c2t = H.conv_pack_weight_t(ps[4]), H.conv_pack_weight_t(ps[6])
        scratch += [wit, wot, c1t, c2t]
        b.in_wT, b.out_wT = wit.data_ptr(), wot.data_ptr()
        b.c1_wpt, b.c2_wpt = c1t.data_ptr(), c2t.data_ptr()
        ar = _arena(sizes, dev)
        scratch.append(ar)
        addr, offs = _carve(ar, sizes)
        ptrs = dict(zip(names, addr))
        for k_, v_ in ptrs.items():
            setattr(g, k_, v_)
        g.dy2, g.dx = dy_ptr, ptrs['d_h']
        dy_ptr = ptrs['d_h']
        last_dh = (ar, offs[names.index('d_h')])
        for j, name in enumerate(_GRAD_FIELDS):
            ent = ops._sink_view(ps[j])
            if ent is not None:
                sink.written.add(ent[0])
                sunk.append(ent[0])
                setattr(g, name, ent[1].data_ptr())
            else:
                t = torch.empty_like(ps[j])
                outs[12 * i + j] = t
                setattr(g, name, t.data_ptr())
    ws = H.workspace(_lib.query('ft_attn_workspace', B, T, nhead), dev)
    side = sink.stream if (sink is not None and sink.stream is not None) else None
    side_raw = side.cuda_stream if side is not None else H._stream()
    def side_buffer(raw, nbytes):
        key = (dev.index or 0, raw)
        buf = _side_ws.get(key)
        if buf is None or buf.numel() < nbytes:
            buf = _side_ws[key] = torch.empty(max(nbytes, 1 << 20), dtype=torch.uint8, device=dev)
        return buf

    wws = side_buffer(side_raw, _lib.query('ft_fft_block_wgrad_workspace', B, T, d, f, k1, k2))
    sums = _sums_stream(dev) if side is not None and os.environ.get('FT_FFT_SUMS_STREAM', '0') == '1' else None
    sums_raw = sums.cuda_stream if sums is not None else None
    sws = side_buffer(('sums', sums_raw), _lib.query('ft_fft_block_sums_workspace', B, T, d, f)) if sums is not None else None
    _lib.call('ft_fft_blocks_bwd', _ct.byref(blocks), _ct.byref(grads), n, ws.data_ptr(), ws.numel(), wws.data_ptr(),
              wws.numel(), _p(sws), sws.numel() if sws is not None else 0, H._stream(), side_raw, sums_raw)
    if sums is not None:
        sink.used.add(sums)
        if sink.reducer_streams is not None:
            sink.reducer_streams.add(sums)
    dx = last_dh[0][last_dh[1]:last_dh[1] + R * d].view(B, T, d)
    if sink is None:
        dx._ft_keep = (scratch, state['arenas'], state['keep'])
    if sink is not None:
        sink.keep.append((scratch, state['arenas'], state['keep'], dy))
        if side is not None:
            sink.used.add(side)
        for idx in sunk:
            sink.used.add(torch.cuda.current_stream())
            if sink.on_write is not None:
                sink.on_write(idx)
    return dx, outs


class TransformerFn(Function):

    @staticmethod
    def forward(ctx, x, key_pad, pe, pe_scale, norm_g, norm_b, cfg, *params):
        nhead, p_blk, p_pe, training, eps1, eps2, eps_f = cfg
        x = _c(x)
        B, T, D = x.shape
        check_posenc_length(T, pe)
        h = torch.empty_like(x)
        _lib.call('ft_posenc_fwd', x.data_ptr(), pe.data_ptr(), pe_scale.data_ptr(), h.data_ptr(), B, T, D, H._stream())
        pe_seed = 0
        if training and p_pe > 0:
            pe_seed = _seed()
            h = H.dropout(h, p_pe, pe_seed)
        p = p_blk if training else 0.0
        tapes = []
        ctx.comp = None
        if composite_ok(D, nhead) and len(params) >= 12:
            seeds = [(_seed() if p > 0 else 0) for _ in range(3 * (len(params) // 12))]
            h, ctx.comp = blocks_fwd_composite(h, key_pad, params, nhead, p, eps1, eps2, seeds)
            params_loop = ()
        else:
            params_loop = params
        for i in range(len(params_loop) // 12):
            in_w, in_b, out_w, out_b, c1w, c1b, c2w, c2b, n1g, n1b, n2g, n2b = params[12 * i:12 * i + 12]
            s0 = _seed() if p > 0 else 0
            sa, t_mha = mha_fwd(h, key_pad, in_w, in_b, out_w, out_b, nhead, p, s0)
            y1, t_n1 = addln_fwd(h, sa, n1g, n1b, eps1, p, _seed() if p > 0 else 0)
            h1, t_c1 = convbias_fwd(y1, c1w, c1b, True)
            h2, t_c2 = convbias_fwd(h1, c2w, c2b, False)
            h, t_n2 = addln_fwd(y1, h2, n2g, n2b, eps2, p, _seed() if p > 0 else 0)
            tapes.append((t_mha, t_n1, t_c1, t_c2, t_n2))
        y, t_f = addln_fwd(h, None, norm_g, norm_b, eps_f)
        ctx.tapes, ctx.t_f, ctx.params = tapes, t_f, params
        ctx.head = (pe, pe_scale, norm_g, norm_b, p_pe if training else 0.0, pe_seed)
        return y

    @staticmethod
    def backward(ctx, dy):
        pe, pe_scale, norm_g, norm_b, p_pe, pe_seed = ctx.head
        params = ctx.params
        grads = [None] * len(params)
        d, _, g_ng, g_nb = addln_bwd(ctx.t_f, _c(dy), norm_g, norm_b)
        if ctx.comp is not None:
            d, grads = blocks_bwd_composite(ctx.comp, d, params)
            ctx.comp = None
        for i in range(len(ctx.tapes) - 1, -1, -1):
            in_w, in_b, out_w, out_b, c1w, c1b, c2w, c2b, n1g, n1b, n2g, n2b = params[12 * i:12 * i + 12]
            t_mha, t_n1, t_c1, t_c2, t_n2 = ctx.tapes[i]
            with ops.batched_side_launches():
                d_y1, d_h2, g_n2g, g_n2b = addln_bwd(t_n2, d, n2g, n2b, own_dres=True)
                d_h1, g_c2w, g_c2b = convbias_bwd(t_c2, d_h2, c2w, c2b)
                d_y1, g_c1w, g_c1b = convbias_bwd(t_c1, d_h1, c1w, c1b, dx_into=d_y1)
                d_h, d_sa, g_n1g, g_n1b = addln_bwd(t_n1, d_y1, n1g, n1b, own_dres=True)
                d, g_iw, g_ib, g_ow, g_ob = mha_bwd(t_mha, d_sa, in_w, in_b, out_w, out_b, dx_into=d_h)
            grads[12 * i:12 * i + 12] = [g_iw, g_ib, g_ow, g_ob, g_c1w, g_c1b, g_c2w, g_c2b, g_n1g, g_n1b, g_n2g, g_n2b]
        ctx.tapes = None
        if p_pe > 0:
            d = H.dropout(d, p_pe, pe_seed)
        B, T, D = d.shape

        def dscale(o):
            ws = H.workspace(_lib.query('ft_posenc_workspace'), d.device)
            _lib.call('ft_posenc_bwd_scale', d.data_ptr(), pe.data_ptr(), o.data_ptr(), B, T, D, ws.data_ptr(),
                      ws.numel(), H._stream())

        g_scale = _emit(pe_scale, dscale, heavy=False)
        return (d if ctx.needs_input_grad[0] else None, None, None, g_scale, g_ng, g_nb, None, *grads)


class PositionalEncoding(nn.Module):

    def __init__(self, d_model: int, dropout=0.1, max_len=5000) -> None:
        super().__init__()
        self.p = dropout
        self.scale = nn.Parameter(torch.ones(1))
        pe = torch.zeros(max_len, d_model)
        position = torch.arange(0, max_len, dtype=torch.float).unsqueeze(1)
        div_term = torch.exp(torch.arange(0, d_model, 2).float() * (-math.log(10000.0) / d_model))
        pe[:, 0::2] = torch.sin(position * div_term)
        pe[:, 1::2] = torch.cos(position * div_term)
        self.register_buffer('pe', pe.unsqueeze(0).transpose(0, 1))

    def forward(self, x: torch.Tensor) -> torch.Tensor:
        if x.shape[1] > self.pe.shape[0]:
            raise _lib.FtError(f'sequence length {x.shape[1]} exceeds PositionalEncoding max_len {self.pe.shape[0]}')
        x = PosEncFn.apply(x, self.pe, self.scale)
        return _dropout(x, self.p, self.training)


class FFTBlock(nn.Module):

    def __init__(self, d_model: int, nhead: int, conv1_kernel: int, conv2_kernel: int, d_fft: int,
                 dropout: float = 0.1):
        super().__init__()
        self.self_attn = nn.MultiheadAttention(d_model, nhead, dropout=dropout)
        self.conv1 = nn.Conv1d(in_channels=d_model, out_channels=d_fft, kernel_size=conv1_kernel, stride=1,
                               padding=conv1_kernel // 2)
        self.conv2 = nn.Conv1d(in_channels=d_fft, out_channels=d_model, kernel_size=conv2_kernel, stride=1,
                               padding=conv2_kernel // 2)
        self.norm1 = nn.LayerNorm(d_model)
        self.norm2 = nn.LayerNorm(d_model)
        self.nhead = nhead
        self.p = dropout

    def forward(self, src: torch.Tensor, key_pad: Optional[torch.Tensor] = None) -> torch.Tensor:
        a = self.self_attn
        p = self.p if self.training else 0.0
        seed = _seed() if p > 0 else 0
        src2 = MHAFn.apply(src, key_pad, a.in_proj_weight, a.in_proj_bias, a.out_proj.weight, a.out_proj.bias,
                           self.nhead, p, seed)
        src = AddLayerNormFn.apply(src, src2, self.norm1.weight, self.norm1.bias, self.norm1.eps, p,
                                   _seed() if p > 0 else 0)
        src2 = ConvBiasFn.apply(src, self.conv1.weight, self.conv1.bias, True)
        src2 = ConvBiasFn.apply(src2, self.conv2.weight, self.conv2.bias, False)
        return AddLayerNormFn.apply(src, src2, self.norm2.weight, self.norm2.bias, self.norm2.eps, p,
                                    _seed() if p > 0 else 0)


class ForwardTransformer(nn.Module):

    def __init__(self, d_model: int, d_fft: int, layers: int, heads: int, conv1_kernel: int, conv2_kernel: int,
                 dropout: float = 0.1) -> None:
        super().__init__()
        self.d_model = d_model
        self.pos_encoder = PositionalEncoding(d_model, dropout)
        encoder_layer = FFTBlock(d_model=d_model, nhead=heads, d_fft=d_fft, conv1_kernel=conv1_kernel,
                                 conv2_kernel=conv2_kernel, dropout=dropout)
        encoder_norm = nn.LayerNorm(d_model)
        self.layers = nn.ModuleList([copy.deepcopy(encoder_layer) for _ in range(layers)])
        self.norm = encoder_norm

    def forward(self, x: torch.Tensor, src_pad_mask: Optional[torch.Tensor] = None) -> torch.Tensor:
        key_pad = None
        if src_pad_mask is not None:
            key_pad = src_pad_mask.to(torch.uint8).contiguous()
        node = os.environ.get('FT_TRANSFORMER_NODE')
        if (node != '1') if node is not None else (H.gemm_precision_mode() != 'bf16'):
            x = self.pos_encoder(x)
            for layer in self.layers:
                x = layer(x, key_pad)
            return AddLayerNormFn.apply(x, None, self.norm.weight, self.norm.bias, self.norm.eps)
        if x.shape[1] > self.pos_encoder.pe.shape[0]:
            raise _lib.FtError(f'sequence length {x.shape[1]} exceeds PositionalEncoding max_len '
                               f'{self.pos_encoder.pe.shape[0]}')
        flat = []
        for l in self.layers:
            a = l.self_attn
            flat += [a.in_proj_weight, a.in_proj_bias, a.out_proj.weight, a.out_proj.bias, l.conv1.weight, l.conv1.bias,
                     l.conv2.weight, l.conv2.bias, l.norm1.weight, l.norm1.bias, l.norm2.weight, l.norm2.bias]
        l0 = self.layers[0]
        cfg = (l0.nhead, l0.p, self.pos_encoder.p, self.training, l0.norm1.eps, l0.norm2.eps, self.norm.eps)
        return TransformerFn.apply(x, key_pad, self.pos_encoder.pe, self.pos_encoder.scale, self.norm.weight,
                                   self.norm.bias, cfg, *flat)


class SeriesPredictor(nn.Module):

    def __init__(self, num_chars: int, d_model: int, n_heads: int, d_fft: int, layers: int, conv1_kernel: int,
                 conv2_kernel: int, dropout=0.1):
        super().__init__()
        self.embedding = nn.Embedding(num_chars, d_model)
        self.transformer = ForwardTransformer(heads=n_heads, dropout=dropout, d_model=d_model, d_fft=d_fft,
                                              conv1_kernel=conv1_kernel, conv2_kernel=conv2_kernel, layers=layers)
        self.lin = nn.Linear(d_model, 1)

    def forward(self, x: torch.Tensor, src_pad_mask: Optional[torch.Tensor] = None, alpha: float = 1.0):
        x = ops.EmbeddingFn.apply(x, self.embedding.weight)
        x = self.transformer(x, src_pad_mask=src_pad_mask)
        x = ops.LinearFn.apply(x, self.lin.weight, self.lin.bias)
        if alpha != 1.0:
            x = ops.ScaleFn.apply(x, 1.0 / alpha)
        return x


class FastPitch(nn.Module):

    def __init__(self, num_chars: int,
                 durpred_dropout: float, durpred_d_model: int, durpred_n_heads: int, durpred_layers: int,
                 durpred_d_fft: int,
                 pitch_dropout: float, pitch_d_model: int, pitch_n_heads: int, pitch_layers: int, pitch_d_fft: int,
                 energy_dropout: float, energy_d_model: int, energy_n_heads: int, energy_layers: int,
                 energy_d_fft: int,
                 pitch_strength: float, energy_strength: float, d_model: int, conv1_kernel: int, conv2_kernel: int,
                 prenet_layers: int, prenet_heads: int, prenet_fft: int, prenet_dropout: float,
                 postnet_layers: int, postnet_heads: int, postnet_fft: int, postnet_dropout: float,
                 n_mels: int, padding_value=PAD_VALUE):
        super().__init__()
        self.padding_value = padding_value
        self.matmul_dtype = 'fp32'
        self.lr = LengthRegulator()
        self.independent_predictors = True
        self.dur_pred = SeriesPredictor(num_chars=num_chars, d_model=durpred_d_model, n_heads=durpred_n_heads,
                                        layers=durpred_layers, d_fft=durpred_d_fft, conv1_kernel=conv1_kernel,
                                        conv2_kernel=conv2_kernel, dropout=durpred_dropout)
        self.pitch_pred = SeriesPredictor(num_chars=num_chars, d_model=pitch_d_model, n_heads=pitch_n_heads,
                                          layers=pitch_layers, d_fft=pitch_d_fft, conv1_kernel=conv1_kernel,
                                          conv2_kernel=conv2_kernel, dropout=pitch_dropout)
        self.energy_pred = SeriesPredictor(num_chars=num_chars, d_model=energy_d_model, n_heads=energy_n_heads,
                                           layers=energy_layers, d_fft=energy_d_fft, conv1_kernel=conv1_kernel,
                                           conv2_kernel=conv2_kernel, dropout=energy_dropout)
        self.embedding = nn.Embedding(num_embeddings=num_chars, embedding_dim=d_model)
        self.prenet = ForwardTransformer(heads=prenet_heads, dropout=prenet_dropout, conv1_kernel=conv1_kernel,
                                         conv2_kernel=conv2_kernel, d_model=d_model, d_fft=prenet_fft,
                                         layers=prenet_layers)
        self.postnet = ForwardTransformer(heads=postnet_heads, dropout=postnet_dropout, conv1_kernel=conv1_kernel,
                                          conv2_kernel=conv2_kernel, d_model=d_model, d_fft=postnet_fft,
                                          layers=postnet_layers)
        self.lin = nn.Linear(d_model, n_mels)
        self.register_buffer('step', torch.zeros(1, dtype=torch.long))
        self.pitch_strength = pitch_strength
        self.energy_strength = energy_strength
        self.pitch_proj = nn.Conv1d(1, d_model, kernel_size=3, padding=1)
        self.energy_proj = nn.Conv1d(1, d_model, kernel_size=3, padding=1)

    def __repr__(self):
        return f'FastPitch, num params: {sum(p.numel() for p in self.parameters())}'

    def _require_device(self, t: torch.Tensor) -> None:
        if not t.is_cuda or not self.embedding.weight.is_cuda:
            raise _lib.FtError('FastPitch runs on an MI355X (HIP) device only; there is no CPU fallback')

    def _mel(self, x_idx, tok_mask, dur, pitch, energy, frame_lens: Optional[torch.Tensor]):
        x = ops.EmbeddingFn.apply(x_idx, self.embedding.weight)
        x = self.prenet(x, src_pad_mask=tok_mask)
        x = ops.CondAddFn.apply(x, pitch, energy, self.pitch_proj.weight, self.pitch_proj.bias,
                                self.energy_proj.weight, self.energy_proj.bias, self.pitch_strength,
                                self.energy_strength, False)
        x = self.lr(x, dur)
        frame_mask = None
        if frame_lens is not None:
            T = x.shape[1]
            frame_mask = torch.arange(T, device=x.device).unsqueeze(0) >= frame_lens.unsqueeze(1)
        x = self.postnet(x, src_pad_mask=frame_mask)
        return ops.LinearFn.apply(x, self.lin.weight, self.lin.bias)

    @precision_scoped
    def forward(self, batch: Dict[str, torch.Tensor]) -> Dict[str, torch.Tensor]:
        x = batch['x']
        mel = batch['mel']
        dur = batch['dur']
        mel_lens = batch['mel_len']
        self._require_device(x)
        if self.training:
            self.step += 1
        len_mask = x == 0
        main = torch.cuda.current_stream()
        side = self._side_stream(x.device)
        side.wait_stream(main)
        with torch.cuda.stream(side):
            dur_hat = self.dur_pred(x, src_pad_mask=len_mask).squeeze(-1)
            pitch_hat = self.pitch_pred(x, src_pad_mask=len_mask).transpose(1, 2)
            energy_hat = self.energy_pred(x, src_pad_mask=len_mask).transpose(1, 2)
            hook = getattr(self, 'predictor_hook', None)
            if hook is not None:
                hook({'dur': dur_hat, 'pitch': pitch_hat, 'energy': energy_hat})
        mel_cl = self._mel(x, len_mask, dur, batch['pitch'], batch['energy'],
                           mel_lens.to(device=x.device, dtype=torch.long))
        x_mel = ops.TransposePadFn.apply(mel_cl, mel.size(2), self.padding_value)
        main.wait_stream(side)
        for t in (dur_hat, pitch_hat, energy_hat):
            t.record_stream(main)
        return {'mel': x_mel, 'mel_post': x_mel, 'dur': dur_hat, 'pitch': pitch_hat, 'energy': energy_hat}

    @precision_scoped
    def generate(self, x: torch.Tensor, alpha=1.0,
                 pitch_function: Callable[[torch.Tensor], torch.Tensor] = lambda x: x,
                 energy_function: Callable[[torch.Tensor], torch.Tensor] = lambda x: x) -> Dict[str, torch.Tensor]:
        self.eval()
        with torch.no_grad():
            self._require_device(x)
            B = x.shape[0]
            dur_hat = self.dur_pred(x, alpha=alpha).squeeze(2)
            if torch.sum(dur_hat.long()) <= 0:
                torch.fill_(dur_hat, value=2.)
            pitch_hat = pitch_function(self.pitch_pred(x).transpose(1, 2))
            energy_hat = energy_function(self.energy_pred(x).transpose(1, 2))
            dur_in = dur_hat.contiguous()
            mel_cl = self._mel(x, x == 0, dur_in, pitch_hat.reshape(B, -1).contiguous(),
                               energy_hat.reshape(B, -1).contiguous(), None)
            m = H.transpose_pad_fwd(mel_cl, mel_cl.shape[1], 0.0)
            return {'mel': m, 'mel_post': m, 'dur': dur_in, 'pitch': pitch_hat, 'energy': energy_hat}

    def pad(self, x: torch.Tensor, max_len: int) -> torch.Tensor:
        x = x[:, :, :max_len]
        return torch.nn.functional.pad(x, [0, max_len - x.size(2), 0, 0], 'constant', self.padding_value)

    def _side_stream(self, device) -> 'torch.cuda.Stream':
        key = torch.device(device).index or 0
        if not hasattr(self, '_streams'):
            self._streams = {}
        if key not in self._streams:
            from .model import _side_priority
            self._streams[key] = torch.cuda.Stream(device=device, priority=_side_priority())
        return self._streams[key]

    def get_step(self) -> int:
        return self.step.data.item()

    @classmethod
    def from_config(cls, config: Dict[str, Any]) -> 'FastPitch':
        model_config = config['fast_pitch']['model']
        model_config['num_chars'] = config.get('num_chars', NUM_CHARS_DEFAULT)
        model_config['n_mels'] = config['dsp']['num_mels']
        return FastPitch(**model_config)

    @classmethod
    def from_checkpoint(cls, path: Union[Path, str]) -> 'FastPitch':
        checkpoint = torch.load(path, map_location=torch.device('cpu'), weights_only=True)
        model = FastPitch.from_config(checkpoint['config'])
        model.load_state_dict(checkpoint['model'])
        return model
```

forwardtacotron_amd/hip.py:

```python
import contextlib
import ctypes
import os
from typing import List, Optional, Sequence

import torch

from . import _lib

c_void_p = ctypes.c_void_p


def _p(t: Optional[torch.Tensor]):
    return None if t is None else t.data_ptr()


_raw_stream = getattr(torch._C, '_cuda_getCurrentRawStream', None)
_cur_device = getattr(torch._C, '_cuda_getDevice', None)


def _stream():
    if _raw_stream is not None and _cur_device is not None:
        return _raw_stream(_cur_device())
    return torch.cuda.current_stream().cuda_stream


def _chk(t: torch.Tensor, name: str, dtype=torch.float32):
    if not t.is_cuda:
        raise _lib.FtError(f'{name}: expected a device tensor (the HIP path has no CPU fallback)')
    if t.dtype != dtype:
        raise _lib.FtError(f'{name}: expected {dtype}, got {t.dtype}')
    if not t.is_contiguous():
        raise _lib.FtError(f'{name}: expected a contiguous tensor')
    return t


_workspaces = {}


def workspace(nbytes: int, device) -> torch.Tensor:
    key = (torch.device(device).index or 0, _stream())
    buf = _workspaces.get(key)
    if buf is None or buf.numel() < nbytes:
        buf = torch.empty(max(nbytes, 1 << 20), dtype=torch.uint8, device=device)
        _workspaces[key] = buf
    return buf


def _ptr_array(ts: Sequence[Optional[torch.Tensor]]):
    arr = (ctypes.c_void_p * len(ts))(*[_p(t) for t in ts])
    return arr


_PRECISIONS = {'fp32': 0, 'bf16': 1}
_precision_now = 'fp32'


def gemm_precision_mode() -> str:
    return _precision_now


def set_gemm_precision(mode: str) -> str:
    if mode not in _PRECISIONS:
        raise _lib.FtError(f"gemm precision must be 'fp32' or 'bf16', got {mode!r}")
    global _precision_now
    old = _lib.lib().ft_set_gemm_precision(_PRECISIONS[mode])
    _precision_now = mode
    return 'bf16' if old else 'fp32'


@contextlib.contextmanager
def gemm_precision(mode: str):
    old = set_gemm_precision(mode)
    try:
        yield
    finally:
        set_gemm_precision(old)


def attn_fwd(qkv: torch.Tensor, key_pad: Optional[torch.Tensor], nheads: int, scale: float, p_drop: float, seed: int):
    _chk(qkv, 'qkv')
    B, T, d3 = qkv.shape
    d = d3 // 3
    att = torch.empty(B, T, d, device=qkv.device, dtype=qkv.dtype)
    lse2 = torch.empty(B, nheads, T, device=qkv.device, dtype=qkv.dtype)
    _lib.call('ft_attn_fwd', _p(qkv), _p(key_pad), _p(att), _p(lse2), B, T, nheads, d // nheads, float(scale),
              float(p_drop), int(seed) & 0xFFFFFFFFFFFFFFFF, _stream())
    return att, lse2


def attn_bwd(qkv, att, datt, key_pad, lse2, nheads: int, scale: float, p_drop: float, seed: int) -> torch.Tensor:
    _chk(datt, 'datt')
    B, T, d3 = qkv.shape
    d = d3 // 3
    dqkv = torch.empty_like(qkv)
    ws = workspace(_lib.query('ft_attn_workspace', B, T, nheads), qkv.device)
    _lib.call('ft_attn_bwd', _p(qkv), _p(att), _p(datt), _p(key_pad), _p(lse2), _p(dqkv), B, T, nheads, d // nheads,
              float(scale), float(p_drop), int(seed) & 0xFFFFFFFFFFFFFFFF, _p(ws), ws.numel(), _stream())
    return dqkv


def linear_fwd(x: torch.Tensor, w: torch.Tensor, bias: Optional[torch.Tensor] = None, relu: bool = False,
               out: Optional[torch.Tensor] = None, x_tm_B: int = 0, y_tm_B: int = 0) -> torch.Tensor:
    _chk(x, 'x'); _chk(w, 'w')
    in_f = x.shape[-1]
    rows = x.numel() // max(in_f, 1) if in_f else 0
    out_f = w.shape[0]
    assert w.shape[1] == in_f
    if out is not None:
        y = out
    elif bool(x_tm_B) != bool(y_tm_B):
        Bq = x_tm_B or y_tm_B
        lead = (rows // Bq, Bq) if y_tm_B else (Bq, rows // Bq)
        y = torch.empty(*lead, out_f, device=x.device, dtype=x.dtype)
    else:
        y = torch.empty(*x.shape[:-1], out_f, device=x.device, dtype=x.dtype)
    _lib.call('ft_linear_fwd', _p(x), in_f, _p(w), _p(bias), _p(y), out_f, rows, in_f, out_f, int(relu), 0,
              x_tm_B, y_tm_B, _stream())
    return y


def linear_multi_fwd(x: torch.Tensor, ws: List[torch.Tensor], biases: Optional[List[Optional[torch.Tensor]]],
                     relu: bool = False, y_tm_B: int = 0, as_rows: int = 0) -> torch.Tensor:
    _chk(x, 'x')
    in_f = x.shape[-1]
    rows = x.numel() // max(in_f, 1)
    outs = [int(w.shape[0]) for w in ws]
    offs = [sum(outs[:i]) for i in range(len(outs))]
    lead = (rows // y_tm_B, y_tm_B) if y_tm_B else tuple(x.shape[:-1])
    y = torch.empty(*lead, sum(outs), device=x.device, dtype=x.dtype)
    n = len(ws)
    wa = _ptr_array(ws)
    ba = _ptr_array(biases) if biases is not None else None
    oa = (ctypes.c_int * n)(*offs)
    fa = (ctypes.c_int * n)(*outs)
    if as_rows:
        assert not relu and not y_tm_B
        _lib.call('ft_linear_multi_fwd_as', _p(x), in_f, n, ctypes.cast(wa, c_void_p),
                  ctypes.cast(ba, c_void_p) if ba is not None else None, _p(y), sum(outs),
                  ctypes.cast(oa, c_void_p), ctypes.cast(fa, c_void_p), rows, in_f, max(int(as_rows), 1), _stream())
        return y
    _lib.call('ft_linear_multi_fwd', _p(x), in_f, n, ctypes.cast(wa, c_void_p),
              ctypes.cast(ba, c_void_p) if ba is not None else None, _p(y), sum(outs),
              ctypes.cast(oa, c_void_p), ctypes.cast(fa, c_void_p), rows, in_f, int(relu), 0, y_tm_B, _stream())
    return y


NT_GRADS = True


def _wt(w: torch.Tensor):
    if NT_GRADS and w.shape[0] % 4 == 0:
        return transpose2d(w), 1
    return w, 0


def linear_bwd_data(dy: torch.Tensor, w: torch.Tensor, dx: Optional[torch.Tensor] = None, accumulate: bool = False,
                    dy_tm_B: int = 0, dx_tm_B: int = 0) -> torch.Tensor:
    _chk(w, 'w'); _chk(dy, 'dy')
    out_f = dy.shape[-1]
    in_f = w.shape[1]
    rows = dy.numel() // max(out_f, 1)
    if dx is None:
        if bool(dy_tm_B) != bool(dx_tm_B):
            Bq = dy_tm_B or dx_tm_B
            lead = (rows // Bq, Bq) if dx_tm_B else (Bq, rows // Bq)
        else:
            lead = tuple(dy.shape[:-1])
        dx = torch.empty(*lead, in_f, device=dy.device, dtype=dy.dtype)
    wt, flag = _wt(w)
    _lib.call('ft_linear_bwd_data', _p(dy), out_f, _p(wt), _p(dx), in_f, rows, in_f, out_f, int(accumulate),
              dy_tm_B, dx_tm_B, flag, _stream())
    return dx


def linear_bwd_data_raw(dy_ptr: int, lddy: int, w: torch.Tensor, dx: torch.Tensor, rows: int, out_f: int,
                        accumulate: bool, dy_tm_B: int = 0, dx_tm_B: int = 0) -> None:
    in_f = w.shape[1]
    wt, flag = _wt(w)
    _lib.call('ft_linear_bwd_data', dy_ptr, lddy, _p(wt), _p(dx), in_f, rows, in_f, out_f, int(accumulate),
              dy_tm_B, dx_tm_B, flag, _stream())


def linear_bwd_data_multi(dy_ptrs: Sequence[int], lddy: int, ws: Sequence[torch.Tensor], dx: torch.Tensor, rows: int,
                          out_f: int, accumulate: bool = False, dy_tm_B: int = 0, dx_tm_B: int = 0) -> None:
    n = len(ws)
    in_f = ws[0].shape[1]
    da = (ctypes.c_void_p * n)(*[int(p) for p in dy_ptrs])
    flag = 1 if NT_GRADS and all(w.shape[0] % 4 == 0 for w in ws) else 0
    wts = [transpose2d(w) for w in ws] if flag else list(ws)
    wa = _ptr_array(wts)
    nbytes = _lib.lib().ft_linear_bwd_data_multi_workspace(n, rows, in_f, out_f, _stream()) if flag else 0
    if nbytes:
        ws = workspace(nbytes, dx.device)
        _lib.call('ft_linear_bwd_data_multi_ws', n, ctypes.cast(da, c_void_p), lddy, ctypes.cast(wa, c_void_p), _p(dx),
                  in_f, rows, in_f, out_f, int(accumulate), dy_tm_B, dx_tm_B, flag, _p(ws), ws.numel(), _stream())
        return
    _lib.call('ft_linear_bwd_data_multi', n, ctypes.cast(da, c_void_p), lddy, ctypes.cast(wa, c_void_p), _p(dx), in_f,
              rows, in_f, out_f, int(accumulate), dy_tm_B, dx_tm_B, flag, _stream())


def linear_bwd_weight_raw(dy_ptr: int, lddy: int, x_ptr: int, ldx: int, dw: torch.Tensor, rows: int, in_f: int,
                          out_f: int, B: int = 1, T: int = 0, x_shift: int = 0, accumulate: bool = False,
                          dy_tm: bool = False, x_tm: bool = False) -> None:
    nbytes = _lib.query('ft_linear_bwd_weight_workspace', rows, in_f, out_f)
    ws = workspace(nbytes, dw.device)
    _lib.call('ft_linear_bwd_weight', dy_ptr, lddy, x_ptr, ldx, _p(dw), rows, in_f, out_f, B, T if T else rows,
              x_shift, int(accumulate), int(dy_tm), int(x_tm), _p(ws), ws.numel(), _stream())


def linear_bwd_weight(dy: torch.Tensor, x: torch.Tensor) -> torch.Tensor:
    _chk(dy, 'dy'); _chk(x, 'x')
    out_f, in_f = dy.shape[-1], x.shape[-1]
    rows = x.numel() // max(in_f, 1)
    dw = torch.empty(out_f, in_f, device=x.device, dtype=x.dtype)
    linear_bwd_weight_raw(_p(dy), out_f, _p(x), in_f, dw, rows, in_f, out_f)
    return dw


class PackCache:

    def __init__(self, mats, convs, banks, device, highways=()):
        import struct
        self.wp, self.wpt, self.t2d, self.bank, self.hw = {}, {}, {}, {}, {}
        self._keep = []
        descs = []
        tiles = 0

        def add(src, dst, dst_t, d0, d1, k):
            nonlocal tiles
            descs.append(struct.pack('PPPqiiii', src.data_ptr(), _p(dst) or 0, _p(dst_t) or 0, tiles, d0, d1, k, 0))
            tiles += k * ((d0 + 31) // 32) * ((d1 + 31) // 32)

        for w in mats:
            _chk(w, 'w')
            R, C = w.shape
            wt = torch.empty(C, R, device=device, dtype=w.dtype)
            self.t2d[(w.data_ptr(), R, C)] = wt
            add(w, None, wt, R, C, 1)
        for w in convs:
            _chk(w, 'w')
            Cout, Cin, k = w.shape
            wp = torch.empty(k, Cout, Cin, device=device, dtype=w.dtype)
            wpt = torch.empty(k, Cin, Cout, device=device, dtype=w.dtype)
            self.wp[w.data_ptr()] = wp
            self.wpt[w.data_ptr()] = wpt
            add(w, wp, wpt, Cout, Cin, k)
        for ws in banks:
            C, Cin = ws[0].shape[0], ws[0].shape[1]
            n = sum(w.shape[2] for w in ws) * C * Cin
            wp_all = torch.empty(n, device=device, dtype=ws[0].dtype)
            wpt_all = torch.empty(n, device=device, dtype=ws[0].dtype)
            off = 0
            for w in ws:
                _chk(w, 'w')
                k = w.shape[2]
                add(w, wp_all[off:off + k * C * Cin], wpt_all[off:off + k * C * Cin], C, Cin, k)
                off += k * C * Cin
            self.bank[tuple(w.data_ptr() for w in ws)] = (wp_all, wpt_all)
        for w1, w2 in highways:
            _chk(w1, 'w1'); _chk(w2, 'w2')
            C = w1.shape[0]
            if w1.shape != (C, C) or w2.shape != (C, C) or C % 32:
                continue
            pack = torch.empty(2 * C, C, device=device, dtype=w1.dtype)
            self.hw[(w1.data_ptr(), w2.data_ptr())] = pack
            for j in range(C // 32):
                add(w1[32 * j:32 * j + 32], pack[64 * j:64 * j + 32], None, 32, C, 1)
                add(w2[32 * j:32 * j + 32], pack[64 * j + 32:64 * j + 64], None, 32, C, 1)
        self.n, self.tiles = len(descs), tiles
        self.descs = torch.frombuffer(bytearray(b''.join(descs)), dtype=torch.uint8).to(device) if descs else None

    def refresh(self) -> None:
        if self.n:
            _lib.call('ft_pack_weights', _p(self.descs), self.n, self.tiles, _stream())

    @staticmethod
    def release() -> None:
        """the weights are about to change (or the step failed): the packs are stale until the next refresh()"""


pack_cache: Optional[PackCache] = None


def bank_packs(ws: Sequence[torch.Tensor], transposed: bool) -> torch.Tensor:
    if pack_cache is not None:
        hit = pack_cache.bank.get(tuple(w.data_ptr() for w in ws))
        if hit is not None:
            return hit[1 if transposed else 0]
    C, Cin = ws[0].shape[0], ws[0].shape[1]
    out = torch.empty(sum(w.shape[2] for w in ws) * C * Cin, device=ws[0].device, dtype=ws[0].dtype)
    off = 0
    for w in ws:
        k = w.shape[2]
        n = k * C * Cin
        if transposed:
            conv_pack_weight_t(w, out=out[off:off + n].view(k, Cin, C))
        else:
            conv_pack_weight(w, out=out[off:off + n].view(k, C, Cin))
        off += n
    return out


def conv_pack_weight(w: torch.Tensor, out: Optional[torch.Tensor] = None) -> torch.Tensor:
    if out is None and pack_cache is not None:
        hit = pack_cache.wp.get(w.data_ptr())
        if hit is not None:
            return hit
    _chk(w, 'w')
    Cout, Cin, k = w.shape
    wp = out if out is not None else torch.empty(k, Cout, Cin, device=w.device, dtype=w.dtype)
    _lib.call('ft_conv_pack_weight', _p(w), _p(wp), Cout, Cin, k, _stream())
    return wp


def conv1d_fwd(x: torch.Tensor, wp: torch.Tensor, relu: bool, Tout: Optional[int] = None,
               scale: Optional[torch.Tensor] = None, shift: Optional[torch.Tensor] = None,
               accumulate_into: Optional[torch.Tensor] = None) -> torch.Tensor:
    _chk(x, 'x'); _chk(wp, 'wp')
    B, T, Cin = x.shape
    k, Cout, _ = wp.shape
    Tout = T if Tout is None else Tout
    y = accumulate_into if accumulate_into is not None else torch.empty(B, Tout, Cout, device=x.device,
                                                                        dtype=x.dtype)
    _lib.call('ft_conv1d_fwd', _p(x), Cin, _p(wp), _p(scale), _p(shift), _p(y), Cout, B, T, Cin, Cout, k, Tout,
              int(relu), int(accumulate_into is not None), _stream())
    return y


def conv_bank_fwd(x: torch.Tensor, wp_all: torch.Tensor, K: int, C: int, relu: bool, Tout: int,
                  scale: Optional[torch.Tensor] = None, shift: Optional[torch.Tensor] = None) -> torch.Tensor:
    _chk(x, 'x'); _chk(wp_all, 'wp_all')
    B, T, Cin = x.shape
    assert wp_all.numel() == C * Cin * K * (K + 1) // 2
    y = torch.empty(B, Tout, K * C, device=x.device, dtype=x.dtype)
    _lib.call('ft_conv_bank_fwd', _p(x), Cin, _p(wp_all), _p(scale), _p(shift), _p(y), B, T, Cin, C, K, Tout,
              int(relu), _stream())
    return y


def conv1d_fwd_stats(x: torch.Tensor, wp: torch.Tensor, relu: bool, Tout: int):
    _chk(x, 'x'); _chk(wp, 'wp')
    B, T, Cin = x.shape
    k, Cout, _ = wp.shape
    y = torch.empty(B, Tout, Cout, device=x.device, dtype=x.dtype)
    nbytes = _lib.query('ft_conv1d_fwd_stats_workspace', B, Tout, Cout, k)
    part = workspace(nbytes, x.device)
    n = ctypes.c_int(0)
    _lib.call('ft_conv1d_fwd_stats', _p(x), Cin, _p(wp), _p(y), Cout, B, T, Cin, Cout, k, Tout, int(relu), _p(part),
              part.numel(), ctypes.byref(n), _stream())
    return y, part, n.value


def conv_bank_fwd_stats(x: torch.Tensor, wp_all: torch.Tensor, K: int, C: int, relu: bool):
    _chk(x, 'x'); _chk(wp_all, 'wp_all')
    B, T, Cin = x.shape
    assert wp_all.numel() == C * Cin * K * (K + 1) // 2
    y = torch.empty(B, T + 1, K * C, device=x.device, dtype=x.dtype)
    nbytes = _lib.query('ft_conv_stats_workspace', B, T + 1, K * C)
    part = workspace(nbytes, x.device)
    n = ctypes.c_int(0)
    _lib.call('ft_conv_bank_fwd_stats', _p(x), Cin, _p(wp_all), _p(y), B, T, Cin, C, K, int(relu), _p(part),
              part.numel(), ctypes.byref(n), _stream())
    return y, part, n.value


def bn_train_from_partials(part: torch.Tensor, nchunks: int, y: torch.Tensor, gamma, beta, running_mean, running_var,
                           Tout: int, group: int = 0, residual: Optional[torch.Tensor] = None,
                           momentum: float = None, eps: float = None):
    B, Tbuf, C = y.shape
    out = torch.empty(B, Tout, C, device=y.device, dtype=y.dtype)
    mean = torch.empty(C, device=y.device, dtype=y.dtype)
    rstd = torch.empty(C, device=y.device, dtype=y.dtype)
    _lib.call('ft_bn_train_from_partials', _p(part), nchunks, _p(y), _p(gamma), _p(beta), _p(residual), _p(out),
              _p(running_mean), _p(running_var), None, _p(mean), _p(rstd), B, Tbuf, Tout, C, group,
              BN_MOMENTUM if momentum is None else momentum, BN_EPS if eps is None else eps, _stream())
    return out, mean, rstd


def conv_pack_weight_t(w: torch.Tensor, out: Optional[torch.Tensor] = None) -> torch.Tensor:
    if out is None and pack_cache is not None:
        hit = pack_cache.wpt.get(w.data_ptr())
        if hit is not None:
            return hit
    _chk(w, 'w')
    Cout, Cin, k = w.shape
    wpt = out if out is not None else torch.empty(k, Cin, Cout, device=w.device, dtype=w.dtype)
    _lib.call('ft_conv_pack_weight_t', _p(w), _p(wpt), Cout, Cin, k, _stream())
    return wpt


def conv1d_bwd_data_raw(dy_ptr: int, lddy: int, wp: torch.Tensor, dx: torch.Tensor, B: int, T: int, Tbuf: int,
                        Tvalid: int, accumulate: bool, w: Optional[torch.Tensor] = None) -> None:
    k, Cout, Cin = wp.shape
    if NT_GRADS and w is not None and Cout % 4 == 0:
        wpt = conv_pack_weight_t(w)
        _lib.call('ft_conv1d_bwd_data', dy_ptr, lddy, _p(wpt), _p(dx), Cin, B, T, Cin, Cout, k, Tbuf, Tvalid,
                  int(accumulate), 1, _stream())
        return
    _lib.call('ft_conv1d_bwd_data', dy_ptr, lddy, _p(wp), _p(dx), Cin, B, T, Cin, Cout, k, Tbuf, Tvalid,
              int(accumulate), 0, _stream())


def conv_bank_bwd_data(dy: torch.Tensor, wp_all: torch.Tensor, K: int, C: int, Cin: int, T: int,
                       ws: Optional[Sequence[torch.Tensor]] = None) -> torch.Tensor:
    _chk(dy, 'dy'); _chk(wp_all, 'wp_all')
    B, Tbuf, _ = dy.shape
    dx = torch.empty(B, T, Cin, device=dy.device, dtype=dy.dtype)
    flag = 0
    if NT_GRADS and ws is not None and C % 4 == 0:
        wp_all, flag = bank_packs(ws, True), 1
    nbytes = _lib.query('ft_conv_bank_bwd_data_workspace', B, T, Cin, K)
    ws = workspace(nbytes, dy.device) if nbytes else None
    _lib.call('ft_conv_bank_bwd_data', _p(dy), K * C, _p(wp_all), _p(dx), Cin, B, T, Cin, C, K, Tbuf, flag,
              _p(ws), ws.numel() if ws is not None else 0, _stream())
    return dx


def conv_bank_bwd_weight(dy: torch.Tensor, x: torch.Tensor, dws: Sequence[torch.Tensor], C: int) -> None:
    _chk(dy, 'dy'); _chk(x, 'x')
    B, T, Cin = x.shape
    Tbuf, K = dy.shape[1], len(dws)
    for i, d in enumerate(dws):
        _chk(d, 'dw')
        if tuple(d.shape) != (C, Cin, i + 1):
            raise _lib.FtError(f'conv_bank_bwd_weight: dw[{i}] has shape {tuple(d.shape)}')
    nbytes = _lib.query('ft_conv_bank_bwd_weight_workspace', B, T, Cin, C, K, Tbuf)
    ws = workspace(nbytes, x.device)
    _lib.call('ft_conv_bank_bwd_weight', _p(dy), K * C, _p(x), Cin, _ptr_array(dws), B, T, Cin, C, K, Tbuf, _p(ws),
              ws.numel(), _stream())


def conv1d_bwd_weight_raw(dy_ptr: int, lddy: int, x: torch.Tensor, dw: torch.Tensor, Tbuf: int, Tvalid: int) -> None:
    B, T, Cin = x.shape
    Cout, _, k = dw.shape
    nbytes = _lib.query('ft_conv1d_bwd_weight_workspace', B, T, Cin, Cout, k, Tvalid)
    ws = workspace(nbytes, x.device)
    _lib.call('ft_conv1d_bwd_weight', dy_ptr, lddy, _p(x), Cin, _p(dw), B, T, Cin, Cout, k, Tbuf, Tvalid, _p(ws),
              ws.numel(), _stream())


def lr_scan(dur: torch.Tensor):
    _chk(dur, 'dur')
    B, Tx = dur.shape
    cum = torch.empty(B, Tx + 1, device=dur.device, dtype=torch.int32)
    total = torch.empty(B, device=dur.device, dtype=torch.int32)
    _lib.call('ft_lr_scan', _p(dur), B, Tx, _p(cum), _p(total), _stream())
    return cum, total


def lr_expand(x: torch.Tensor, cum: torch.Tensor, Tm: int, want_src: bool = False):
    _chk(x, 'x'); _chk(cum, 'cum', torch.int32)
    B, Tx, C = x.shape
    y = torch.empty(B, Tm, C, device=x.device, dtype=x.dtype)
    src = torch.empty(B, Tm, device=x.device, dtype=torch.int32) if want_src else None
    _lib.call('ft_lr_expand', _p(x), _p(cum), _p(y), _p(src), B, Tx, Tm, C, _stream())
    return (y, src) if want_src else y


def lr_bwd(dy: torch.Tensor, cum: torch.Tensor, Tx: int) -> torch.Tensor:
    _chk(dy, 'dy'); _chk(cum, 'cum', torch.int32)
    B, Tm, C = dy.shape
    dx = torch.empty(B, Tx, C, device=dy.device, dtype=dy.dtype)
    _lib.call('ft_lr_bwd', _p(dy), _p(cum), _p(dx), B, Tx, Tm, C, _stream())
    return dx


def lr_expand_tm(x: torch.Tensor, cum: torch.Tensor, Tm: int, pad_row: Optional[torch.Tensor] = None) -> torch.Tensor:
    _chk(x, 'x'); _chk(cum, 'cum', torch.int32)
    B, Tx, C = x.shape
    if pad_row is not None:
        _chk(pad_row, 'pad_row')
        assert pad_row.numel() == C
    y = torch.empty(Tm, B, C, device=x.device, dtype=x.dtype)
    _lib.call('ft_lr_expand_tm', _p(x), _p(cum), _p(pad_row), _p(y), B, Tx, Tm, C, _stream())
    return y


def lr_bwd_tm(dy: torch.Tensor, cum: torch.Tensor, Tx: int):
    _chk(dy, 'dy'); _chk(cum, 'cum', torch.int32)
    Tm, B, C = dy.shape
    rows = torch.empty(B * Tx + B, C, device=dy.device, dtype=dy.dtype)
    dx = rows[:B * Tx].view(B, Tx, C)
    _lib.call('ft_lr_bwd_tm', _p(dy), _p(cum), _p(dx), _p(rows[B * Tx:]), B, Tx, Tm, C, _stream())
    return dx, rows


BN_EPS = 1e-5
BN_MOMENTUM = 0.1


def bn_train_fwd(y: torch.Tensor, gamma, beta, running_mean, running_var, Tout: int, group: int = 0,
                 residual: Optional[torch.Tensor] = None, momentum: float = BN_MOMENTUM, eps: float = BN_EPS):
    _chk(y, 'y')
    B, Tbuf, C = y.shape
    out = torch.empty(B, Tout, C, device=y.device, dtype=y.dtype)
    mean = torch.empty(C, device=y.device, dtype=y.dtype)
    rstd = torch.empty(C, device=y.device, dtype=y.dtype)
    nbytes = _lib.query('ft_bn_workspace', B, Tbuf, C)
    ws = workspace(nbytes, y.device)
    _lib.call('ft_bn_train_fwd', _p(y), _p(gamma), _p(beta), _p(residual), _p(out), _p(running_mean),
              _p(running_var), None, _p(mean), _p(rstd), B, Tbuf, Tout, C, group, momentum, eps, _p(ws), ws.numel(),
              _stream())
    return out, mean, rstd


def bn_bwd(dout: torch.Tensor, y: torch.Tensor, gamma, mean, rstd, group: int, relu: bool,
           dgamma: Optional[torch.Tensor] = None, dbeta: Optional[torch.Tensor] = None):
    _chk(dout, 'dout'); _chk(y, 'y')
    B, Tbuf, C = y.shape
    Tout = dout.shape[1]
    dy = torch.empty_like(y)
    if dgamma is None:
        dgamma = torch.empty(C, device=y.device, dtype=y.dtype)
    if dbeta is None:
        dbeta = torch.empty(C, device=y.device, dtype=y.dtype)
    nbytes = _lib.query('ft_bn_workspace', B, Tbuf, C)
    ws = workspace(nbytes, y.device)
    _lib.call('ft_bn_bwd', _p(dout), _p(y), _p(gamma), _p(mean), _p(rstd), _p(dy), _p(dgamma), _p(dbeta), B, Tbuf,
              Tout, C, group, int(relu), _p(ws), ws.numel(), _stream())
    return dy, dgamma, dbeta


def bn_pool_fusable(y: torch.Tensor, group: int) -> bool:
    return y.shape[-1] % 4 == 0 and group % 4 == 0 and y.data_ptr() % 16 == 0


def bn_pool_from_partials(part: torch.Tensor, nchunks: int, y: torch.Tensor, gamma, beta, running_mean, running_var,
                          Tout: int, group: int = 0, momentum: float = None, eps: float = None):
    B, Tbuf, C = y.shape
    out = torch.empty(B, Tout, C, device=y.device, dtype=y.dtype)
    mean = torch.empty(C, device=y.device, dtype=y.dtype)
    rstd = torch.empty(C, device=y.device, dtype=y.dtype)
    _lib.call('ft_bn_pool_from_partials', _p(part), nchunks, _p(y), _p(gamma), _p(beta), _p(out), _p(running_mean),
              _p(running_var), None, _p(mean), _p(rstd), B, Tbuf, Tout, C, group,
              BN_MOMENTUM if momentum is None else momentum, BN_EPS if eps is None else eps, _stream())
    return out, mean, rstd


def bn_pool_bwd(dout: torch.Tensor, y: torch.Tensor, gamma, beta, mean, rstd, group: int, relu: bool):
    _chk(dout, 'dout'); _chk(y, 'y')
    B, Tbuf, C = y.shape
    Tout = dout.shape[1]
    dy = torch.empty_like(y)
    dgamma = torch.empty(C, device=y.device, dtype=y.dtype)
    dbeta = torch.empty(C, device=y.device, dtype=y.dtype)
    nbytes = _lib.query('ft_bn_workspace', B, Tbuf, C)
    ws = workspace(nbytes, y.device)
    _lib.call('ft_bn_pool_bwd', _p(dout), _p(y), _p(gamma), _p(beta), _p(mean), _p(rstd), _p(dy), _p(dgamma), _p(dbeta),
              B, Tbuf, Tout, C, group, int(relu), _p(ws), ws.numel(), _stream())
    return dy, dgamma, dbeta


def bn_fold_eval(gamma, beta, running_mean, running_var, eps: float = BN_EPS):
    C = gamma.numel()
    scale = torch.empty(C, device=gamma.device, dtype=gamma.dtype)
    shift = torch.empty(C, device=gamma.device, dtype=gamma.dtype)
    _lib.call('ft_bn_fold_eval', _p(gamma), _p(beta), _p(running_mean), _p(running_var), eps, _p(scale), _p(shift),
              C, _stream())
    return scale, shift


def colsum_raw(x_ptr: int, ldx: int, out: torch.Tensor, rows: int, C: int, scale: float = 1.0,
               accumulate: bool = False) -> None:
    nbytes = _lib.query('ft_colsum_workspace', rows, C)
    ws = workspace(nbytes, out.device)
    _lib.call('ft_colsum', x_ptr, ldx, _p(out), rows, C, scale, int(accumulate), _p(ws), ws.numel(), _stream())


def colsum2_raw(x0_ptr: int, x1_ptr: int, ldx: int, out0: torch.Tensor, out1: torch.Tensor, rows: int, C: int) -> None:
    nbytes = _lib.query('ft_colsum_workspace', rows, C)
    ws = workspace(nbytes, out0.device)
    _lib.call('ft_colsum2', x0_ptr, x1_ptr, ldx, _p(out0), _p(out1), rows, C, _p(ws), ws.numel(), _stream())


def colsum(x: torch.Tensor) -> torch.Tensor:
    _chk(x, 'x')
    C = x.shape[-1]
    rows = x.numel() // max(C, 1)
    out = torch.empty(C, device=x.device, dtype=x.dtype)
    colsum_raw(_p(x), C, out, rows, C)
    return out


def colsum_batch(xs: Sequence[torch.Tensor]) -> List[torch.Tensor]:
    rows = xs[0].numel() // xs[0].shape[-1]
    for x in xs:
        _chk(x, 'x')
        assert x.numel() // x.shape[-1] == rows
    n = len(xs)
    outs = [torch.empty(x.shape[-1], device=x.device, dtype=x.dtype) for x in xs]
    Cs = (ctypes.c_int * n)(*[int(x.shape[-1]) for x in xs])
    lds = (ctypes.c_long * n)(*[int(x.shape[-1]) for x in xs])
    nbytes = _lib.lib().ft_colsum_batch_workspace(n, ctypes.cast(Cs, c_void_p), rows)
    ws = workspace(max(int(nbytes), 16), xs[0].device)
    _lib.call('ft_colsum_batch', n, ctypes.cast(_ptr_array(list(xs)), c_void_p), ctypes.cast(lds, c_void_p),
              ctypes.cast(_ptr_array(outs), c_void_p), ctypes.cast(Cs, c_void_p), rows, _p(ws), ws.numel(), _stream())
    return outs


def dropout(x: torch.Tensor, p: float, seed: int) -> torch.Tensor:
    _chk(x, 'x')
    out = torch.empty_like(x)
    _lib.call('ft_dropout', _p(x), _p(out), x.numel(), p, seed & 0xFFFFFFFFFFFFFFFF, _stream())
    return out


def scale(x: torch.Tensor, s: float) -> torch.Tensor:
    _chk(x, 'x')
    out = torch.empty_like(x)
    _lib.call('ft_scale', _p(x), _p(out), x.numel(), s, _stream())
    return out



def embedding_fwd(idx: torch.Tensor, w: torch.Tensor) -> torch.Tensor:
    _chk(idx, 'idx', torch.int64); _chk(w, 'w')
    V, C = w.shape
    out = torch.empty(*idx.shape, C, device=w.device, dtype=w.dtype)
    err = _err_flag(w.device)
    _lib.call('ft_embedding_fwd', _p(idx), _p(w), _p(out), idx.numel(), C, V, _p(err), _stream())
    return out


_err_flags = {}


def _err_flag(device) -> torch.Tensor:
    key = torch.device(device).index or 0
    if key not in _err_flags:
        _err_flags[key] = torch.zeros(1, dtype=torch.int32, device=device)
    return _err_flags[key]


def check_index_errors(device) -> None:
    f = _err_flag(device)
    if int(f.item()) != 0:
        f.zero_()
        raise IndexError('embedding index out of range (set by ft_embedding_fwd)')


def onehot(idx: torch.Tensor, V: int) -> torch.Tensor:
    _chk(idx, 'idx', torch.int64)
    out = torch.empty(idx.numel(), V, device=idx.device, dtype=torch.float32)
    _lib.call('ft_onehot', _p(idx), _p(out), idx.numel(), V, _stream())
    return out


def embedding_bwd(idx: torch.Tensor, dout: torch.Tensor, V: int,
                  onehot_cache: Optional[dict] = None, out: Optional[torch.Tensor] = None) -> torch.Tensor:
    _chk(idx, 'idx', torch.int64); _chk(dout, 'dout')
    C = dout.shape[-1]
    key = (idx.data_ptr(), idx.numel(), V, _stream())
    oh = onehot_cache.get(key) if onehot_cache is not None else None
    if oh is None:
        oh = onehot(idx, V)
        if onehot_cache is not None:
            onehot_cache[key] = oh
    dw = out if out is not None else torch.empty(V, C, device=dout.device, dtype=dout.dtype)
    linear_bwd_weight_raw(_p(oh), V, _p(dout), C, dw, idx.numel(), C, V)
    return dw


def highway_gate_fwd(x12: torch.Tensor, x: torch.Tensor) -> torch.Tensor:
    _chk(x12, 'x12'); _chk(x, 'x')
    C = x.shape[-1]
    out = torch.empty_like(x)
    _lib.call('ft_highway_gate_fwd', _p(x12), _p(x), _p(out), x.numel() // C, C, _stream())
    return out


def highway_gate_bwd(dout, x12, x):
    _chk(dout, 'dout')
    C = x.shape[-1]
    d12 = torch.empty_like(x12)
    dx = torch.empty_like(x)
    _lib.call('ft_highway_gate_bwd', _p(dout), _p(x12), _p(x), _p(d12), _p(dx), x.numel() // C, C, _stream())
    return d12, dx


def highway_pack(w1: torch.Tensor, w2: torch.Tensor) -> torch.Tensor:
    if pack_cache is not None:
        hit = pack_cache.hw.get((w1.data_ptr(), w2.data_ptr()))
        if hit is not None:
            return hit
    _chk(w1, 'w1'); _chk(w2, 'w2')
    C = w1.shape[0]
    out = torch.empty(2 * C, C, device=w1.device, dtype=w1.dtype)
    _lib.call('ft_highway_pack', _p(w1), _p(w2), _p(out), C, _stream())
    return out


def highway_fwd(x: torch.Tensor, w12i: torch.Tensor, b1: torch.Tensor, b2: torch.Tensor, save: bool):
    _chk(x, 'x'); _chk(w12i, 'w12i')
    C = x.shape[-1]
    rows = x.numel() // C
    out = torch.empty_like(x)
    x12 = torch.empty(*x.shape[:-1], 2 * C, device=x.device, dtype=x.dtype) if save else None
    _lib.call('ft_highway_fwd', _p(x), _p(w12i), _p(b1), _p(b2), _p(out), _p(x12), rows, C, _stream())
    return out, x12


def highway_bwd_data(d12: torch.Tensor, w1: torch.Tensor, w2: torch.Tensor, dx: torch.Tensor,
                     below: Optional[tuple] = None) -> Optional[torch.Tensor]:
    C = dx.shape[-1]
    rows = dx.numel() // C
    flag = 1 if NT_GRADS else 0
    wa, wb = (transpose2d(w1), transpose2d(w2)) if flag else (w1, w2)
    d12b = torch.empty_like(d12) if below is not None else None
    _lib.call('ft_highway_bwd_data', _p(d12), _p(wa), _p(wb), flag, _p(dx), rows, C,
              _p(below[0]) if below else None, _p(below[1]) if below else None, _p(d12b), _stream())
    return d12b


def maxpool2_fwd(x: torch.Tensor) -> torch.Tensor:
    _chk(x, 'x')
    B, T, C = x.shape
    out = torch.empty_like(x)
    _lib.call('ft_maxpool2_fwd', _p(x), _p(out), B, T, C, _stream())
    return out


def maxpool2_bwd(dout: torch.Tensor, x: torch.Tensor) -> torch.Tensor:
    _chk(dout, 'dout')
    B, T, C = x.shape
    dx = torch.empty_like(x)
    _lib.call('ft_maxpool2_bwd', _p(dout), _p(x), _p(dx), B, T, C, _stream())
    return dx


def cond_add_fwd(x, pitch, energy, wp, bp, we, be, sp: float, se: float, x_time_major: bool = False) -> torch.Tensor:
    _chk(x, 'x'); _chk(pitch, 'pitch'); _chk(energy, 'energy')
    B, T = pitch.shape
    C = x.shape[-1]
    out = torch.empty(B, T, C, device=x.device, dtype=x.dtype)
    _lib.call('ft_cond_add_fwd', _p(x), _p(pitch), _p(energy), _p(wp), _p(bp), _p(we), _p(be), sp, se, _p(out), B,
              T, C, int(x_time_major), _stream())
    return out


def cond_taps(pitch, energy) -> torch.Tensor:
    B, T = pitch.shape
    taps = torch.empty(B, T, 8, device=pitch.device, dtype=pitch.dtype)
    _lib.call('ft_cond_taps', _p(pitch), _p(energy), _p(taps), B, T, _stream())
    return taps


def concat_cols(a: torch.Tensor, b2: Optional[torch.Tensor], semb: Optional[torch.Tensor], B: int, T: int,
                a_time_major: bool = False) -> torch.Tensor:
    _chk(a, 'a')
    Ca = a.shape[-1]
    Cb = b2.shape[-1] if b2 is not None else 0
    S = semb.shape[-1] if semb is not None else 0
    out = torch.empty(B, T, Ca + Cb + S, device=a.device, dtype=a.dtype)
    _lib.call('ft_concat_cols', _p(a), Ca, _p(b2), Cb, _p(semb), S, _p(out), B, T, int(a_time_major), _stream())
    return out


def slice_cols(src: torch.Tensor, col0: int, C: int, dst_time_major: bool = False) -> torch.Tensor:
    _chk(src, 'src')
    B, T, ld = src.shape
    dst = torch.empty((T, B, C) if dst_time_major else (B, T, C), device=src.device, dtype=src.dtype)
    _lib.call('ft_slice_cols', _p(src), ld, col0, C, _p(dst), B, T, int(dst_time_major), _stream())
    return dst


def cross_entropy_fwd(logits: torch.Tensor, target: torch.Tensor, ignore_index: int):
    _chk(logits, 'logits'); _chk(target, 'target', torch.int64)
    K = logits.shape[-1]
    rows = logits.numel() // K
    loss = torch.empty((), device=logits.device, dtype=logits.dtype)
    inv = torch.empty(1, device=logits.device, dtype=logits.dtype)
    ws = workspace(_lib.query('ft_cross_entropy_workspace'), logits.device)
    _lib.call('ft_cross_entropy_fwd', _p(logits), _p(target), rows, K, ignore_index, _p(loss), _p(inv), _p(ws),
              ws.numel(), _stream())
    return loss, inv


def cross_entropy_bwd(logits, target, inv, grad_out, ignore_index: int) -> torch.Tensor:
    K = logits.shape[-1]
    rows = logits.numel() // K
    d = torch.empty_like(logits)
    _lib.call('ft_cross_entropy_bwd', _p(logits), _p(target), _p(inv), _p(grad_out), _p(d), rows, K, ignore_index,
              _stream())
    return d


def transpose_pad_fwd(x: torch.Tensor, Tout: int, pad: float) -> torch.Tensor:
    _chk(x, 'x')
    B, T, C = x.shape
    out = torch.empty(B, C, Tout, device=x.device, dtype=x.dtype)
    _lib.call('ft_transpose_pad_fwd', _p(x), _p(out), B, T, C, Tout, pad, _stream())
    return out


def transpose_pad_bwd(dout: torch.Tensor, T: int) -> torch.Tensor:
    _chk(dout, 'dout')
    B, C, Tout = dout.shape
    dx = torch.empty(B, T, C, device=dout.device, dtype=dout.dtype)
    _lib.call('ft_transpose_pad_bwd', _p(dout), _p(dx), B, T, C, Tout, _stream())
    return dx


def copy_segments(srcs: Sequence[torch.Tensor], dsts: Sequence[torch.Tensor]) -> None:
    for i in range(0, len(srcs), 64):
        ss, dd = srcs[i:i + 64], dsts[i:i + 64]
        n = len(ss)
        for a, b in zip(ss, dd):
            _chk(a, 'src'); _chk(b, 'dst')
            if a.numel() != b.numel():
                raise _lib.FtError('copy_segments: size mismatch')
        lens = (ctypes.c_long * n)(*[a.numel() for a in ss])
        _lib.call('ft_copy_segments', _ptr_array(ss), _ptr_array(dd), lens, n, _stream())


def transpose2d(x: torch.Tensor) -> torch.Tensor:
    R, C = x.shape
    if pack_cache is not None:
        hit = pack_cache.t2d.get((x.data_ptr(), R, C))
        if hit is not None:
            return hit
    return transpose_pad_fwd(x.view(1, R, C), R, 0.0).view(C, R)


def masked_l1_fwd(x: torch.Tensor, target: torch.Tensor, lens: torch.Tensor):
    _chk(x, 'x'); _chk(target, 'target'); _chk(lens, 'lens', torch.int64)
    B, C, T = x.shape
    loss = torch.empty((), device=x.device, dtype=x.dtype)
    inv = torch.empty(1, device=x.device, dtype=x.dtype)
    ws = workspace(_lib.query('ft_masked_l1_workspace'), x.device)
    _lib.call('ft_masked_l1_fwd', _p(x), _p(target), _p(lens), _p(loss), _p(inv), B, C, T, _p(ws), ws.numel(),
              _stream())
    return loss, inv


def masked_l1_bwd(x, target, lens, inv, grad_out: Optional[torch.Tensor], factor: float = 1.0) -> torch.Tensor:
    B, C, T = x.shape
    dx = torch.empty_like(x)
    _lib.call('ft_masked_l1_bwd', _p(x), _p(target), _p(lens), _p(inv), _p(grad_out), factor, _p(dx), B, C, T,
              _stream())
    return dx


_rnn_ws = {}


def _rnn_workspace(gates: int, B: int, H: int, device):
    nbytes = _lib.query('ft_rnn_workspace', gates, B, H)
    if nbytes == 0:
        return None, 0
    key = (torch.device(device).index or 0, _stream(), gates, B, H)
    ws = _rnn_ws.get(key)
    if ws is None:
        ws = torch.zeros(nbytes, dtype=torch.uint8, device=device)
        _rnn_ws[key] = ws
    return ws, nbytes


def check_rnn_status(clear: bool = True) -> None:
    _lib.call('ft_rnn_status', int(clear))


def rnn_note_join(waiting: 'torch.cuda.Stream', joined: 'torch.cuda.Stream') -> None:
    _lib.call('ft_rnn_note_join', waiting.cuda_stream, joined.cuda_stream)


def rnn_mode_counts():
    a, b = ctypes.c_long(0), ctypes.c_long(0)
    _lib.call('ft_rnn_mode_counts', ctypes.byref(a), ctypes.byref(b))
    return a.value, b.value


def rnn_counters():
    a, b = ctypes.c_long(0), ctypes.c_long(0)
    _lib.call('ft_rnn_counters', ctypes.byref(a), ctypes.byref(b))
    return a.value, b.value


def rnn_waited_launches() -> int:
    return int(_lib.query('ft_rnn_waited_launches'))


def gru_fwd(xp, whh_f, whh_r, bhh_f, bhh_r, H: int, save_gates: bool):
    _chk(xp, 'xp')
    T, B, _ = xp.shape
    out = torch.empty(T, B, 2 * H, device=xp.device, dtype=xp.dtype)
    gates = torch.empty(T, B, 2, 4 * H, device=xp.device, dtype=xp.dtype) if save_gates else None
    ws, nb = _rnn_workspace(3, B, H, xp.device)
    _lib.call('ft_gru_fwd', _p(xp), _p(whh_f), _p(whh_r), _p(bhh_f), _p(bhh_r), _p(out), _p(gates), B, T, H,
              _p(ws), nb, _stream())
    return out, gates


def gru_bwd(dout, out, gates, whhT_f, whhT_r, H: int):
    _chk(dout, 'dout')
    T, B, _ = out.shape
    dxp = torch.empty(T, B, 6 * H, device=out.device, dtype=out.dtype)
    dhp = torch.empty(T, B, 6 * H, device=out.device, dtype=out.dtype)
    carry = torch.empty(B, 2, H, device=out.device, dtype=out.dtype)
    ws, nb = _rnn_workspace(3, B, H, out.device)
    _lib.call('ft_gru_bwd', _p(dout), _p(out), _p(gates), _p(whhT_f), _p(whhT_r), _p(dxp), _p(dhp), _p(carry), B, T,
              H, _p(ws), nb, _stream())
    return dxp, dhp


def lstm_fwd(xp, whh_f, whh_r, bhh_f, bhh_r, lens: Optional[torch.Tensor], H: int, save_gates: bool):
    _chk(xp, 'xp')
    T, B, _ = xp.shape
    raw = torch.empty(T, B, 2 * H, device=xp.device, dtype=xp.dtype)
    cst = torch.empty(T, B, 2 * H, device=xp.device, dtype=xp.dtype)
    gates = torch.empty(T, B, 2, 4 * H, device=xp.device, dtype=xp.dtype) if save_gates else None
    ws, nb = _rnn_workspace(4, B, H, xp.device)
    _lib.call('ft_lstm_fwd', _p(xp), _p(whh_f), _p(whh_r), _p(bhh_f), _p(bhh_r), _p(lens), _p(raw), _p(cst),
              _p(gates), B, T, H, _p(ws), nb, _stream())
    return raw, cst, gates


_proj_streams = {}


def rnn_overlap(rows: int, T: int) -> int:
    if os.environ.get('FT_RNN_OVERLAP', '0') != '1' or rows < 8192 or T < 256:
        return 0
    return max(2, int(os.environ.get('FT_RNN_CHUNKS', '4')))


def _proj_stream(device) -> 'torch.cuda.Stream':
    key = torch.device(device).index or 0
    st = _proj_streams.get(key)
    if st is None:
        st = torch.cuda.Stream(device=device)
        _proj_streams[key] = st
    return st


def lstm_layer_fwd(x, wih_f, wih_r, bih_f, bih_r, whh_f, whh_r, bhh_f, bhh_r, lens: Optional[torch.Tensor], H: int,
                   save_gates: bool, nchunks: int):
    _chk(x, 'x')
    B, T, I = x.shape
    dev = x.device
    xp = torch.empty(T, B, 8 * H, device=dev, dtype=x.dtype)
    raw = torch.empty(T, B, 2 * H, device=dev, dtype=x.dtype)
    cst = torch.empty(T, B, 2 * H, device=dev, dtype=x.dtype)
    gates = torch.empty(T, B, 2, 4 * H, device=dev, dtype=x.dtype) if save_gates else None
    gate = torch.empty(16, device=dev, dtype=torch.int32)
    ws, nb = _rnn_workspace(4, B, H, dev)
    lead = int(os.environ.get('FT_RNN_REV_LEAD', str(nchunks // 2))) if lens is not None else 0
    _lib.call('ft_lstm_layer_fwd', _p(x), I, _p(wih_f), _p(wih_r), _p(bih_f), _p(bih_r), _p(xp), _p(whh_f), _p(whh_r),
              _p(bhh_f), _p(bhh_r), _p(lens), _p(raw), _p(cst), _p(gates), B, T, H, _p(ws), nb, _p(gate), nchunks, lead,
              _stream(), _proj_stream(dev).cuda_stream)
    return raw, cst, gates


def gru_layer_fwd(x, wih_f, wih_r, bih_f, bih_r, whh_f, whh_r, bhh_f, bhh_r, H: int, save_gates: bool, nchunks: int):
    _chk(x, 'x')
    B, T, I = x.shape
    dev = x.device
    xp = torch.empty(T, B, 6 * H, device=dev, dtype=x.dtype)
    out = torch.empty(T, B, 2 * H, device=dev, dtype=x.dtype)
    gates = torch.empty(T, B, 2, 4 * H, device=dev, dtype=x.dtype) if save_gates else None
    gate = torch.empty(16, device=dev, dtype=torch.int32)
    ws, nb = _rnn_workspace(3, B, H, dev)
    _lib.call('ft_gru_layer_fwd', _p(x), I, _p(wih_f), _p(wih_r), _p(bih_f), _p(bih_r), _p(xp), _p(whh_f), _p(whh_r),
              _p(bhh_f), _p(bhh_r), _p(out), _p(gates), B, T, H, _p(ws), nb, _p(gate), nchunks, _stream(),
              _proj_stream(dev).cuda_stream)
    return out, gates


def lstm_bwd(dout, raw, cst, gates, whhT_f, whhT_r, lens: Optional[torch.Tensor], H: int):
    _chk(dout, 'dout')
    T, B, _ = raw.shape
    dg = torch.empty(T, B, 8 * H, device=raw.device, dtype=raw.dtype)
    carry = torch.empty(B, 2, H, device=raw.device, dtype=raw.dtype)
    ws, nb = _rnn_workspace(4, B, H, raw.device)
    _lib.call('ft_lstm_bwd', _p(dout), _p(raw), _p(cst), _p(gates), _p(whhT_f), _p(whhT_r), _p(lens), _p(dg),
              _p(carry), B, T, H, _p(ws), nb, _stream())
    return dg


def fill_padded(raw_tm: torch.Tensor, lens: Optional[torch.Tensor], pad: float) -> torch.Tensor:
    T, B, C = raw_tm.shape
    out = torch.empty(B, T, C, device=raw_tm.device, dtype=raw_tm.dtype)
    _lib.call('ft_fill_padded', _p(raw_tm), _p(lens), _p(out), B, T, C, pad, _stream())
    return out


def bt_transpose(src: torch.Tensor, to_time_major: bool) -> torch.Tensor:
    _chk(src, 'src')
    if to_time_major:
        B, T, C = src.shape
        dst = torch.empty(T, B, C, device=src.device, dtype=src.dtype)
    else:
        T, B, C = src.shape
        dst = torch.empty(B, T, C, device=src.device, dtype=src.dtype)
    _lib.call('ft_bt_transpose', _p(src), _p(dst), B, T, C, int(to_time_major), _stream())
    return dst


def mask_rows(src: torch.Tensor, lens: torch.Tensor) -> torch.Tensor:
    B, T, C = src.shape
    dst = torch.empty_like(src)
    _lib.call('ft_mask_rows', _p(src), _p(lens), _p(dst), B, T, C, _stream())
    return dst
```

Baseline: 1.015 million.

## Fold column-reduction finalize kernels into partial kernels via last-block atomic counters

Removes the separate finalize launches for batch-norm statistics, column sums, batched column sums and masked L1 loss. Each partial block now stores its result with agent-scope atomics and bumps a per-column-tile counter, and the last block to arrive does the final reduction and writes the stats or sums. This saves one launch per reduction, and many small kernels in the train step become single launches. In exchange it needs zero-initialised counter tails in every workspace, adds fence and atomic overhead, and does the serial finish inside the last block.

```diff
diff --git a/forwardtacotron_amd/csrc/ft_bn.hip b/forwardtacotron_amd/csrc/ft_bn.hip
--- a/forwardtacotron_amd/csrc/ft_bn.hip
+++ b/forwardtacotron_amd/csrc/ft_bn.hip
@@ -1,6 +1,7 @@
 #include <string.h>
 
 #include "ft_common.h"
+#include "ft_fold.h"
 
 namespace {
 
@@ -42,14 +43,150 @@
   return g;
 }
 
+constexpr int FIN_PARTS = 8;
+__device__ __forceinline__ void sum_partials(const double* partial, int nchunks, int C, int c, int part,
+                                             double (*sh)[FIN_PARTS][2], int slot, double& s0, double& s1) {
+  double a0 = 0.0, a1 = 0.0;
+  if (c < C) {
+    const int per = (nchunks + FIN_PARTS - 1) / FIN_PARTS;
+    const int i0 = part * per, i1 = min(nchunks, i0 + per);
+    for (int i = i0; i < i1; ++i) {
+      a0 += partial[((long)i * C + c) * 2 + 0];
+      a1 += partial[((long)i * C + c) * 2 + 1];
+    }
+  }
+  sh[slot][part][0] = a0;
+  sh[slot][part][1] = a1;
+  __syncthreads();
+  s0 = 0.0;
+  s1 = 0.0;
+  if (part == 0) {
+#pragma unroll
+    for (int p = 0; p < FIN_PARTS; ++p) {
+      s0 += sh[slot][p][0];
+      s1 += sh[slot][p][1];
+    }
+  }
+}
+
+__device__ __forceinline__ void bn_stats_store(double s0, double s1, int c, int B, int Tbuf, int group, float momentum,
+                                               float eps, float* running_mean, float* running_var, float* save_mean,
+                                               float* save_rstd) {
+  double n = (double)B * (double)tvalid_of(c, Tbuf, group);
+  double mu = s0 / n;
+  double var = s1 / n - mu * mu;
+  if (var < 0.0) var = 0.0;
+  save_mean[c] = (float)mu;
+  save_rstd[c] = (float)(1.0 / sqrt(var + (double)eps));
+  if (running_mean) {
+    double unb = n > 1.0 ? var * n / (n - 1.0) : var;
+    running_mean[c] = (float)((1.0 - momentum) * (double)running_mean[c] + momentum * mu);
+    running_var[c] = (float)((1.0 - momentum) * (double)running_var[c] + momentum * unb);
+  }
+}
+
+__global__ __launch_bounds__(256) void ft_bn_finalize_kernel(const double* __restrict__ partial, int nchunks, int B,
+                                                             int Tbuf, int C, int group, float momentum, float eps,
+                                                             float* __restrict__ running_mean,
+                                                             float* __restrict__ running_var, long* __restrict__ nbt,
+                                                             float* __restrict__ save_mean,
+                                                             float* __restrict__ save_rstd) {
+  __shared__ double sh[32][FIN_PARTS][2];
+  const int slot = threadIdx.x >> 3, part = threadIdx.x & 7;
+  const int c = blockIdx.x * 32 + slot;
+  if (blockIdx.x == 0 && threadIdx.x == 0 && nbt) *nbt += 1;
+  double s0, s1;
+  sum_partials(partial, nchunks, C, c, part, sh, slot, s0, s1);
+  if (part != 0 || c >= C) return;
+  bn_stats_store(s0, s1, c, B, Tbuf, group, momentum, eps, running_mean, running_var, save_mean, save_rstd);
+}
+
+struct FoldFin {
+  unsigned* cnt;
+  int bn;
+  float* out0;
+  float* out1;
+  float scale0;
+  int accumulate;
+  float momentum, eps;
+  float* running_mean;
+  float* running_var;
+  long* nbt;
+  float* save_mean;
+  float* save_rstd;
+};
+__device__ __forceinline__ void fold_finish64(const FoldFin& f, unsigned* cnt, unsigned arrivals, const double* partial,
+                                              int nchunks, int C, int blk64, int B, int Tbuf, int group, void* lds) {
+  if (!ft_fold_arrive(cnt, arrivals, reinterpret_cast<volatile unsigned*>(lds))) return;
+  double(*sh)[32][FIN_PARTS][2] = reinterpret_cast<double(*)[32][FIN_PARTS][2]>(lds);
+  const int slot = threadIdx.x >> 3, part = threadIdx.x & 7;
+  if (f.bn && blk64 == 0 && threadIdx.x == 0 && f.nbt) *f.nbt += 1;
+  const int per = (nchunks + FIN_PARTS - 1) / FIN_PARTS;
+  const int i0 = part * per, i1 = min(nchunks, i0 + per);
+  if (per <= 8) {
+    double2 v[2][8];
+#pragma unroll
+    for (int h = 0; h < 2; ++h) {
+      const int cc = min(blk64 * 64 + h * 32 + slot, C - 1);
+#pragma unroll
+      for (int k = 0; k < 8; ++k)
+        v[h][k] = *reinterpret_cast<const double2*>(partial + ((long)min(i0 + k, nchunks - 1) * C + cc) * 2);
+    }
+#pragma unroll
+    for (int h = 0; h < 2; ++h) {
+      double a0 = 0.0, a1 = 0.0;
+#pragma unroll
+      for (int k = 0; k < 8; ++k) {
+        const bool ok = i0 + k < i1;
+        a0 += ok ? v[h][k].x : 0.0;
+        a1 += ok ? v[h][k].y : 0.0;
+      }
+      sh[h][slot][part][0] = a0;
+      sh[h][slot][part][1] = a1;
+    }
+  } else {
+    for (int h = 0; h < 2; ++h) {
+      const int c = blk64 * 64 + h * 32 + slot;
+      double a0 = 0.0, a1 = 0.0;
+      if (c < C)
+        for (int i = i0; i < i1; ++i) {
+          a0 += partial[((long)i * C + c) * 2 + 0];
+          a1 += partial[((long)i * C + c) * 2 + 1];
+        }
+      sh[h][slot][part][0] = a0;
+      sh[h][slot][part][1] = a1;
+    }
+  }
+  __syncthreads();
+  if (part != 0) return;
+#pragma unroll
+  for (int h = 0; h < 2; ++h) {
+    const int c = blk64 * 64 + h * 32 + slot;
+    if (c >= C) continue;
+    double s0 = 0.0, s1 = 0.0;
+#pragma unroll
+    for (int q = 0; q < FIN_PARTS; ++q) {
+      s0 += sh[h][slot][q][0];
+      s1 += sh[h][slot][q][1];
+    }
+    if (f.bn) {
+      bn_stats_store(s0, s1, c, B, Tbuf, group, f.momentum, f.eps, f.running_mean, f.running_var, f.save_mean,
+                     f.save_rstd);
+    } else {
+      if (f.out0) f.out0[c] = (f.accumulate ? f.out0[c] : 0.f) + (float)(s0 * f.scale0);
+      if (f.out1) f.out1[c] = (f.accumulate ? f.out1[c] : 0.f) + (float)s1;
+    }
+  }
+}
+
 template <int MODE>
 __global__ __launch_bounds__(256) void ft_col_partial_kernel(const float* __restrict__ y, long ldy,
                                                              const float* __restrict__ dout,
                                                              const float* __restrict__ mean,
                                                              const float* __restrict__ rstd, int B, int Tbuf, int Tout,
                                                              int C, int group, int rows_per_chunk,
-                                                             double* __restrict__ partial) {
-  __shared__ double red[2][4][64];
+                                                             double* partial, FoldFin fin) {
+  __shared__ double red[2][8][64];
   const int cl = threadIdx.x & 63, rl = threadIdx.x >> 6;
   const int c = blockIdx.x * 64 + cl;
   const long rows = (long)B * Tbuf;
@@ -96,14 +233,16 @@
   if (rl == 0 && c < C) {
     double a0 = red[0][0][cl] + red[0][1][cl] + red[0][2][cl] + red[0][3][cl];
     double a1 = red[1][0][cl] + red[1][1][cl] + red[1][2][cl] + red[1][3][cl];
-    partial[((long)blockIdx.y * C + c) * 2 + 0] = a0;
-    partial[((long)blockIdx.y * C + c) * 2 + 1] = a1;
-  }
+    ft_fold_store(&partial[((long)blockIdx.y * C + c) * 2 + 0], a0);
+    ft_fold_store(&partial[((long)blockIdx.y * C + c) * 2 + 1], a1);
+  }
+  if (fin.cnt)
+    fold_finish64(fin, fin.cnt + blockIdx.x, gridDim.y, partial, (int)gridDim.y, C, (int)blockIdx.x, B, Tbuf, group, red);
 }
 
 __global__ __launch_bounds__(256) void ft_colsum4_partial_kernel(const float* __restrict__ x, long ldx, long rows, int C,
-                                                                 int rows_per_chunk, double* __restrict__ partial,
-                                                                 const float* __restrict__ x1) {
+                                                                 int rows_per_chunk, double* partial,
+                                                                 const float* __restrict__ x1, FoldFin fin) {
   if (x1) {
     if (blockIdx.z == 1) x = x1;
   }
@@ -141,10 +280,12 @@
       double a = 0.0;
 #pragma unroll
       for (int i = 0; i < 16; ++i) a += red[i][threadIdx.x];
-      partial[((long)blockIdx.y * C + cc) * 2 + slot] = a;
-      if (!x1) partial[((long)blockIdx.y * C + cc) * 2 + 1] = 0.0;
-    }
-  }
+      ft_fold_store(&partial[((long)blockIdx.y * C + cc) * 2 + slot], a);
+      if (!x1) ft_fold_store(&partial[((long)blockIdx.y * C + cc) * 2 + 1], 0.0);
+    }
+  }
+  fold_finish64(fin, fin.cnt + blockIdx.x, gridDim.y * gridDim.z, partial, (int)gridDim.y, C, (int)blockIdx.x, 1, 1, 0,
+                red);
 }
 
 template <int MODE>
@@ -152,7 +293,7 @@
                                                               const float* __restrict__ mean,
                                                               const float* __restrict__ rstd, int B, int Tbuf, int Tout,
                                                               int C, int group, int rows_per_chunk,
-                                                              double* __restrict__ partial,
+                                                              double* partial, FoldFin fin,
                                                               const float* __restrict__ gamma = nullptr,
                                                               const float* __restrict__ beta = nullptr) {
   __shared__ double red[2][16][65];
@@ -235,75 +376,12 @@
         a0 += red[0][i][threadIdx.x];
         a1 += red[1][i][threadIdx.x];
       }
-      partial[((long)blockIdx.y * C + cc) * 2 + 0] = a0;
-      partial[((long)blockIdx.y * C + cc) * 2 + 1] = a1;
-    }
-  }
-}
-
-constexpr int FIN_PARTS = 8;
-__device__ __forceinline__ void sum_partials(const double* __restrict__ partial, int nchunks, int C, int c, int part,
-                                             double (*sh)[FIN_PARTS][2], int slot, double& s0, double& s1) {
-  double a0 = 0.0, a1 = 0.0;
-  if (c < C) {
-    const int per = (nchunks + FIN_PARTS - 1) / FIN_PARTS;
-    const int i0 = part * per, i1 = min(nchunks, i0 + per);
-    for (int i = i0; i < i1; ++i) {
-      a0 += partial[((long)i * C + c) * 2 + 0];
-      a1 += partial[((long)i * C + c) * 2 + 1];
-    }
-  }
-  sh[slot][part][0] = a0;
-  sh[slot][part][1] = a1;
-  __syncthreads();
-  s0 = 0.0;
-  s1 = 0.0;
-  if (part == 0) {
-#pragma unroll
-    for (int p = 0; p < FIN_PARTS; ++p) {
-      s0 += sh[slot][p][0];
-      s1 += sh[slot][p][1];
-    }
-  }
-}
-
-__global__ __launch_bounds__(256) void ft_bn_finalize_kernel(const double* __restrict__ partial, int nchunks, int B,
-                                                             int Tbuf, int C, int group, float momentum, float eps,
-                                                             float* __restrict__ running_mean,
-                                                             float* __restrict__ running_var, long* __restrict__ nbt,
-                                                             float* __restrict__ save_mean,
-                                                             float* __restrict__ save_rstd) {
-  __shared__ double sh[32][FIN_PARTS][2];
-  const int slot = threadIdx.x >> 3, part = threadIdx.x & 7;
-  const int c = blockIdx.x * 32 + slot;
-  if (blockIdx.x == 0 && threadIdx.x == 0 && nbt) *nbt += 1;
-  double s0, s1;
-  sum_partials(partial, nchunks, C, c, part, sh, slot, s0, s1);
-  if (part != 0 || c >= C) return;
-  double n = (double)B * (double)tvalid_of(c, Tbuf, group);
-  double mu = s0 / n;
-  double var = s1 / n - mu * mu;
-  if (var < 0.0) var = 0.0;
-  save_mean[c] = (float)mu;
-  save_rstd[c] = (float)(1.0 / sqrt(var + (double)eps));
-  if (running_mean) {
-    double unb = n > 1.0 ? var * n / (n - 1.0) : var;
-    running_mean[c] = (float)((1.0 - momentum) * (double)running_mean[c] + momentum * mu);
-    running_var[c] = (float)((1.0 - momentum) * (double)running_var[c] + momentum * unb);
-  }
-}
-
-__global__ __launch_bounds__(256) void ft_col_finalize_kernel(const double* __restrict__ partial, int nchunks, int C,
-                                                              float* __restrict__ out0, float* __restrict__ out1,
-                                                              float scale0, int accumulate) {
-  __shared__ double sh[32][FIN_PARTS][2];
-  const int slot = threadIdx.x >> 3, part = threadIdx.x & 7;
-  const int c = blockIdx.x * 32 + slot;
-  double s0, s1;
-  sum_partials(partial, nchunks, C, c, part, sh, slot, s0, s1);
-  if (part != 0 || c >= C) return;
-  if (out0) out0[c] = (accumulate ? out0[c] : 0.f) + (float)(s0 * scale0);
-  if (out1) out1[c] = (accumulate ? out1[c] : 0.f) + (float)s1;
+      ft_fold_store(&partial[((long)blockIdx.y * C + cc) * 2 + 0], a0);
+      ft_fold_store(&partial[((long)blockIdx.y * C + cc) * 2 + 1], a1);
+    }
+  }
+  if (fin.cnt)
+    fold_finish64(fin, fin.cnt + blockIdx.x, gridDim.y, partial, (int)gridDim.y, C, (int)blockIdx.x, B, Tbuf, group, red);
 }
 
 __global__ __launch_bounds__(256) void ft_bn_apply_kernel(const float* __restrict__ y, const float* __restrict__ mean,
@@ -466,19 +544,20 @@
   float* out[CSB_MAX];
   long ld[CSB_MAX], ws_off[CSB_MAX];
   int C[CSB_MAX], nchunks[CSB_MAX], rpc[CSB_MAX];
-  int tile64[CSB_MAX + 1], tile32[CSB_MAX + 1];
+  int tile64[CSB_MAX + 1];
   int n;
   long rows;
+  unsigned* cnt;
 };
 
-__global__ __launch_bounds__(256) void ft_colsum_batch_partial_kernel(ColsumBatch b, double* __restrict__ ws) {
+__global__ __launch_bounds__(256) void ft_colsum_batch_partial_kernel(ColsumBatch b, double* ws) {
   int t = 0;
   while (t + 1 < b.n && (int)blockIdx.x >= b.tile64[t + 1]) ++t;
   if ((int)blockIdx.y >= b.nchunks[t]) return;
   const float* __restrict__ x = b.x[t];
   const long ldx = b.ld[t];
   const int C = b.C[t];
-  double* __restrict__ partial = ws + b.ws_off[t];
+  double* partial = ws + b.ws_off[t];
   __shared__ double red[16][65];
   const int cq = threadIdx.x & 15, rl = threadIdx.x >> 4;
   const int tile = blockIdx.x - b.tile64[t];
@@ -513,22 +592,14 @@
       double a = 0.0;
 #pragma unroll
       for (int i = 0; i < 16; ++i) a += red[i][threadIdx.x];
-      partial[((long)blockIdx.y * C + cc) * 2] = a;
-      partial[((long)blockIdx.y * C + cc) * 2 + 1] = 0.0;
-    }
-  }
-}
-
-__global__ __launch_bounds__(256) void ft_colsum_batch_finalize_kernel(ColsumBatch b, const double* __restrict__ ws) {
-  int t = 0;
-  while (t + 1 < b.n && (int)blockIdx.x >= b.tile32[t + 1]) ++t;
-  __shared__ double sh[32][FIN_PARTS][2];
-  const int slot = threadIdx.x >> 3, part = threadIdx.x & 7;
-  const int c = (blockIdx.x - b.tile32[t]) * 32 + slot;
-  double s0, s1;
-  sum_partials(ws + b.ws_off[t], b.nchunks[t], b.C[t], c, part, sh, slot, s0, s1);
-  if (part != 0 || c >= b.C[t]) return;
-  b.out[t][c] = (float)s0;
+      ft_fold_store(&partial[((long)blockIdx.y * C + cc) * 2], a);
+      ft_fold_store(&partial[((long)blockIdx.y * C + cc) * 2 + 1], 0.0);
+    }
+  }
+  FoldFin fin = {};
+  fin.out0 = b.out[t];
+  fin.scale0 = 1.0f;
+  fold_finish64(fin, b.cnt + blockIdx.x, b.nchunks[t], partial, b.nchunks[t], C, tile, 1, 1, 0, red);
 }
 
 struct ChunkPlan {
@@ -551,6 +622,17 @@
   ChunkPlan p = {(int)n, (int)rpc};
   return p;
 }
+size_t partial_bytes(long rows, int C) { return (size_t)plan_chunks(rows, C).nchunks * C * 2 * sizeof(double); }
+
+FoldFin fold_cols(void* workspace, size_t workspace_bytes, float* out0, float* out1, float scale0, int accumulate) {
+  FoldFin f = {};
+  f.cnt = ft_fold_counters(workspace, workspace_bytes);
+  f.out0 = out0; f.out1 = out1; f.scale0 = scale0; f.accumulate = accumulate;
+  return f;
+}
+#define FT_REQUIRE_FOLD_WS(what, payload, C)                                                                        \
+  FT_REQUIRE(workspace && workspace_bytes >= ft_fold_ws_bytes(payload) && (unsigned)ft_cdiv(C, 64) <= FT_FOLD_COUNTERS, \
+             what ": workspace too small")
 
 }
 
@@ -558,10 +640,10 @@
   ChunkPlan p = plan_chunks((long)B * Tbuf, C);
   if (C % 4 == 0 && (group == 0 || group % 4 == 0) && all16(y))
     hipLaunchKernelGGL(ft_col_partial4_kernel<0>, dim3(ft_cdiv(C, 64), p.nchunks), dim3(256), 0, s, y, nullptr, nullptr,
-                       nullptr, B, Tbuf, Tbuf, C, group, p.rows_per_chunk, partial);
+                       nullptr, B, Tbuf, Tbuf, C, group, p.rows_per_chunk, partial, FoldFin{});
   else
     hipLaunchKernelGGL(ft_col_partial_kernel<0>, dim3(ft_cdiv(C, 64), p.nchunks), dim3(256), 0, s, y, (long)C, nullptr,
-                       nullptr, nullptr, B, Tbuf, Tbuf, C, group, p.rows_per_chunk, partial);
+                       nullptr, nullptr, B, Tbuf, Tbuf, C, group, p.rows_per_chunk, partial, FoldFin{});
   return p.nchunks;
 }
 
@@ -596,28 +678,28 @@
   return ft_check_launch("bn_train_from_partials");
 }
 
-size_t ft_bn_workspace(int B, int Tbuf, int C) {
-  ChunkPlan p = plan_chunks((long)B * Tbuf, C);
-  return (size_t)p.nchunks * C * 2 * sizeof(double);
-}
+size_t ft_bn_workspace(int B, int Tbuf, int C) { return ft_fold_ws_bytes(partial_bytes((long)B * Tbuf, C)); }
 
 int ft_bn_train_fwd(const float* y, const float* gamma, const float* beta, const float* residual, float* out,
                     float* running_mean, float* running_var, long* num_batches_tracked, float* save_mean,
                     float* save_rstd, int B, int Tbuf, int Tout, int C, int group, float momentum, float eps,
                     void* workspace, size_t workspace_bytes, void* stream) {
   FT_REQUIRE(B > 0 && Tbuf > 0 && C > 0 && Tout <= Tbuf, "bn_train_fwd: bad dims");
-  FT_REQUIRE(workspace && workspace_bytes >= ft_bn_workspace(B, Tbuf, C), "bn_train_fwd: workspace too small");
+  FT_REQUIRE_FOLD_WS("bn_train_fwd", partial_bytes((long)B * Tbuf, C), C);
   hipStream_t s = (hipStream_t)stream;
   ChunkPlan p = plan_chunks((long)B * Tbuf, C);
+  FoldFin fin = {};
+  fin.cnt = ft_fold_counters(workspace, workspace_bytes);
+  fin.bn = 1;
+  fin.momentum = momentum; fin.eps = eps;
+  fin.running_mean = running_mean; fin.running_var = running_var; fin.nbt = num_batches_tracked;
+  fin.save_mean = save_mean; fin.save_rstd = save_rstd;
   if (C % 4 == 0 && (group == 0 || group % 4 == 0) && all16(y))
     hipLaunchKernelGGL(ft_col_partial4_kernel<0>, dim3(ft_cdiv(C, 64), p.nchunks), dim3(256), 0, s, y, nullptr, nullptr,
-                       nullptr, B, Tbuf, Tout, C, group, p.rows_per_chunk, (double*)workspace);
+                       nullptr, B, Tbuf, Tout, C, group, p.rows_per_chunk, (double*)workspace, fin);
   else
     hipLaunchKernelGGL(ft_col_partial_kernel<0>, dim3(ft_cdiv(C, 64), p.nchunks), dim3(256), 0, s, y, (long)C, nullptr,
-                       nullptr, nullptr, B, Tbuf, Tout, C, group, p.rows_per_chunk, (double*)workspace);
-  hipLaunchKernelGGL(ft_bn_finalize_kernel, dim3(ft_cdiv(C, 32)), dim3(256), 0, s, (const double*)workspace,
-                     p.nchunks, B, Tbuf, C, group, momentum, eps, running_mean, running_var, num_batches_tracked,
-                     save_mean, save_rstd);
+                       nullptr, nullptr, B, Tbuf, Tout, C, group, p.rows_per_chunk, (double*)workspace, fin);
   if (out && Tout > 0) {
     long total = (long)B * Tout * C;
     if (C % 4 == 0 && all16(y, save_mean, save_rstd, gamma, beta, residual, out))
@@ -635,17 +717,16 @@
               float* dy, float* dgamma, float* dbeta, int B, int Tbuf, int Tout, int C, int group, int relu,
               void* workspace, size_t workspace_bytes, void* stream) {
   FT_REQUIRE(B > 0 && Tbuf > 0 && C > 0 && Tout <= Tbuf, "bn_bwd: bad dims");
-  FT_REQUIRE(workspace && workspace_bytes >= ft_bn_workspace(B, Tbuf, C), "bn_bwd: workspace too small");
+  FT_REQUIRE_FOLD_WS("bn_bwd", partial_bytes((long)B * Tbuf, C), C);
   hipStream_t s = (hipStream_t)stream;
   ChunkPlan p = plan_chunks((long)B * Tbuf, C);
+  const FoldFin fin = fold_cols(workspace, workspace_bytes, dbeta, dgamma, 1.0f, 0);
   if (C % 4 == 0 && (group == 0 || group % 4 == 0) && all16(y, dout, save_mean, save_rstd))
     hipLaunchKernelGGL(ft_col_partial4_kernel<1>, dim3(ft_cdiv(C, 64), p.nchunks), dim3(256), 0, s, y, dout, save_mean,
-                       save_rstd, B, Tbuf, Tout, C, group, p.rows_per_chunk, (double*)workspace);
+                       save_rstd, B, Tbuf, Tout, C, group, p.rows_per_chunk, (double*)workspace, fin);
   else
     hipLaunchKernelGGL(ft_col_partial_kernel<1>, dim3(ft_cdiv(C, 64), p.nchunks), dim3(256), 0, s, y, (long)C, dout,
-                       save_mean, save_rstd, B, Tbuf, Tout, C, group, p.rows_per_chunk, (double*)workspace);
-  hipLaunchKernelGGL(ft_col_finalize_kernel, dim3(ft_cdiv(C, 32)), dim3(256), 0, s, (const double*)workspace,
-                     p.nchunks, C, dbeta, dgamma, 1.0f, 0);
+                       save_mean, save_rstd, B, Tbuf, Tout, C, group, p.rows_per_chunk, (double*)workspace, fin);
   long total = (long)B * Tbuf * C;
   if (C % 4 == 0 && (group == 0 || group % 4 == 0) && all16(dout, y, save_mean, save_rstd, gamma, dgamma, dbeta, dy))
     hipLaunchKernelGGL(ft_bn_bwd_apply4_kernel<false>, dim3(ft_cdiv(total / 4, 256)), dim3(256), 0, s, (const float4*)dout,
@@ -678,16 +759,15 @@
                    const float* save_rstd, float* dy, float* dgamma, float* dbeta, int B, int Tbuf, int Tout, int C,
                    int group, int relu, void* workspace, size_t workspace_bytes, void* stream) {
   FT_REQUIRE(B > 0 && Tbuf > 0 && C > 0 && Tout > 0 && Tout <= Tbuf, "bn_pool_bwd: bad dims");
-  FT_REQUIRE(workspace && workspace_bytes >= ft_bn_workspace(B, Tbuf, C), "bn_pool_bwd: workspace too small");
+  FT_REQUIRE_FOLD_WS("bn_pool_bwd", partial_bytes((long)B * Tbuf, C), C);
   FT_REQUIRE(C % 4 == 0 && (group == 0 || group % 4 == 0) &&
                  all16(dout, y, save_mean, save_rstd, gamma, beta, dgamma, dbeta, dy),
              "bn_pool_bwd: needs C %% 4 == 0 and 16-byte aligned buffers");
   hipStream_t s = (hipStream_t)stream;
   ChunkPlan p = plan_chunks((long)B * Tbuf, C);
   hipLaunchKernelGGL(ft_col_partial4_kernel<2>, dim3(ft_cdiv(C, 64), p.nchunks), dim3(256), 0, s, y, dout, save_mean,
-                     save_rstd, B, Tbuf, Tout, C, group, p.rows_per_chunk, (double*)workspace, gamma, beta);
-  hipLaunchKernelGGL(ft_col_finalize_kernel, dim3(ft_cdiv(C, 32)), dim3(256), 0, s, (const double*)workspace,
-                     p.nchunks, C, dbeta, dgamma, 1.0f, 0);
+                     save_rstd, B, Tbuf, Tout, C, group, p.rows_per_chunk, (double*)workspace,
+                     fold_cols(workspace, workspace_bytes, dbeta, dgamma, 1.0f, 0), gamma, beta);
   const long total = (long)B * Tbuf * C;
   hipLaunchKernelGGL(ft_bn_bwd_apply4_kernel<true>, dim3(ft_cdiv(total / 4, 256)), dim3(256), 0, s, (const float4*)dout,
                      (const float4*)y, (const float4*)save_mean, (const float4*)save_rstd, (const float4*)gamma,
@@ -705,6 +785,7 @@
 }
 
 size_t ft_colsum_workspace(int rows, int C) { return ft_bn_workspace(1, rows > 0 ? rows : 1, C > 0 ? C : 1); }
+static size_t colsum_payload(int rows, int C) { return partial_bytes(rows > 0 ? rows : 1, C > 0 ? C : 1); }
 
 int ft_colsum(const float* x, long ldx, float* out, int rows, int C, float scale, int accumulate, void* workspace,
               size_t workspace_bytes, void* stream) {
@@ -715,16 +796,15 @@
     if (!accumulate) (void)hipMemsetAsync(out, 0, sizeof(float) * C, s);
     return FT_OK;
   }
-  FT_REQUIRE(workspace && workspace_bytes >= ft_colsum_workspace(rows, C), "colsum: workspace too small");
+  FT_REQUIRE_FOLD_WS("colsum", colsum_payload(rows, C), C);
   ChunkPlan p = plan_chunks(rows, C);
+  const FoldFin fin = fold_cols(workspace, workspace_bytes, out, nullptr, scale, accumulate);
   if (C % 4 == 0 && ldx % 4 == 0 && ((uintptr_t)x) % 16 == 0)
     hipLaunchKernelGGL(ft_colsum4_partial_kernel, dim3(ft_cdiv(C, 64), p.nchunks), dim3(256), 0, s, x, ldx, (long)rows, C,
-                       p.rows_per_chunk, (double*)workspace, (const float*)nullptr);
+                       p.rows_per_chunk, (double*)workspace, (const float*)nullptr, fin);
   else
     hipLaunchKernelGGL(ft_col_partial_kernel<2>, dim3(ft_cdiv(C, 64), p.nchunks), dim3(256), 0, s, x, ldx, nullptr,
-                       nullptr, nullptr, 1, rows, rows, C, 0, p.rows_per_chunk, (double*)workspace);
-  hipLaunchKernelGGL(ft_col_finalize_kernel, dim3(ft_cdiv(C, 32)), dim3(256), 0, s, (const double*)workspace,
-                     p.nchunks, C, out, nullptr, scale, accumulate);
+                       nullptr, nullptr, 1, rows, rows, C, 0, p.rows_per_chunk, (double*)workspace, fin);
   return ft_check_launch("colsum");
 }
 
@@ -738,19 +818,17 @@
     return rc ? rc : ft_colsum(x1, ldx, out1, rows, C, 1.0f, 0, workspace, workspace_bytes, stream);
   }
   hipStream_t s = (hipStream_t)stream;
-  FT_REQUIRE(workspace && workspace_bytes >= ft_colsum_workspace(rows, C), "colsum2: workspace too small");
+  FT_REQUIRE_FOLD_WS("colsum2", colsum_payload(rows, C), C);
   ChunkPlan p = plan_chunks(rows, C);
   hipLaunchKernelGGL(ft_colsum4_partial_kernel, dim3(ft_cdiv(C, 64), p.nchunks, 2), dim3(256), 0, s, x0, ldx, (long)rows,
-                     C, p.rows_per_chunk, (double*)workspace, x1);
-  hipLaunchKernelGGL(ft_col_finalize_kernel, dim3(ft_cdiv(C, 32)), dim3(256), 0, s, (const double*)workspace,
-                     p.nchunks, C, out0, out1, 1.0f, 0);
+                     C, p.rows_per_chunk, (double*)workspace, x1, fold_cols(workspace, workspace_bytes, out0, out1, 1.0f, 0));
   return ft_check_launch("colsum2");
 }
 
 size_t ft_colsum_batch_workspace(int n, const int* C, int rows) {
   size_t total = 0;
-  for (int i = 0; i < n; ++i) total += ft_colsum_workspace(rows, C[i]);
-  return total;
+  for (int i = 0; i < n; ++i) total += colsum_payload(rows, C[i]);
+  return ft_fold_ws_bytes(total);
 }
 
 int ft_colsum_batch(int n, const float* const* x, const long* ld, float* const* out, const int* C, int rows,
@@ -779,14 +857,14 @@
     b.x[i] = x[i]; b.out[i] = out[i]; b.ld[i] = ld[i]; b.C[i] = C[i];
     b.nchunks[i] = p.nchunks; b.rpc[i] = p.rows_per_chunk;
     b.ws_off[i] = off;
-    off += (long)(ft_colsum_workspace(rows, C[i]) / sizeof(double));
+    off += (long)(colsum_payload(rows, C[i]) / sizeof(double));
     b.tile64[i + 1] = b.tile64[i] + ft_cdiv(C[i], 64);
-    b.tile32[i + 1] = b.tile32[i] + ft_cdiv(C[i], 32);
     if (p.nchunks > maxchunks) maxchunks = p.nchunks;
   }
   hipStream_t s = (hipStream_t)stream;
+  FT_REQUIRE((unsigned)b.tile64[n] <= FT_FOLD_COUNTERS, "colsum_batch: %d column blocks (max %u)", b.tile64[n], FT_FOLD_COUNTERS);
+  b.cnt = ft_fold_counters(workspace, workspace_bytes);
   hipLaunchKernelGGL(ft_colsum_batch_partial_kernel, dim3(b.tile64[n], maxchunks), dim3(256), 0, s, b, (double*)workspace);
-  hipLaunchKernelGGL(ft_colsum_batch_finalize_kernel, dim3(b.tile32[n]), dim3(256), 0, s, b, (const double*)workspace);
   return ft_check_launch("colsum_batch");
 }
 
diff --git a/forwardtacotron_amd/csrc/ft_elementwise.hip b/forwardtacotron_amd/csrc/ft_elementwise.hip
--- a/forwardtacotron_amd/csrc/ft_elementwise.hip
+++ b/forwardtacotron_amd/csrc/ft_elementwise.hip
@@ -1,4 +1,5 @@
 #include "ft_common.h"
+#include "ft_fold.h"
 #include "../../include/fwdtaco_hip.h"
 
 namespace {
@@ -374,11 +375,11 @@
   }
 }
 
-__global__ __launch_bounds__(256) void ft_masked_l1_partial_kernel(const float* __restrict__ x,
-                                                                   const float* __restrict__ target,
-                                                                   const long* __restrict__ lens, int B, int C, int T,
-                                                                   double* __restrict__ partial) {
-  __shared__ double red[4];
+__global__ __launch_bounds__(256) void ft_masked_l1_kernel(const float* __restrict__ x, const float* __restrict__ target,
+                                                           const long* __restrict__ lens, int B, int C, int T,
+                                                           double* partial, unsigned* cnt, float* __restrict__ loss,
+                                                           float* __restrict__ inv_denom) {
+  __shared__ double red[2][4];
   long total = (long)B * C * T;
   double acc = 0.0;
   for (long i = (long)blockIdx.x * 256 + threadIdx.x; i < total; i += (long)gridDim.x * 256) {
@@ -387,15 +388,11 @@
     if (t < lens[b]) acc += (double)fabsf(x[i] - target[i]);
   }
   acc = ft_wave_sum_d(acc);
-  if ((threadIdx.x & 63) == 0) red[threadIdx.x >> 6] = acc;
+  if ((threadIdx.x & 63) == 0) red[0][threadIdx.x >> 6] = acc;
   __syncthreads();
-  if (threadIdx.x == 0) partial[blockIdx.x] = red[0] + red[1] + red[2] + red[3];
-}
-__global__ __launch_bounds__(256) void ft_masked_l1_finalize_kernel(const double* __restrict__ partial, int nblocks,
-                                                                    const long* __restrict__ lens, int B, int C,
-                                                                    int T, float* __restrict__ loss,
-                                                                    float* __restrict__ inv_denom) {
-  __shared__ double red[2][4];
+  if (threadIdx.x == 0) ft_fold_store(&partial[blockIdx.x], red[0][0] + red[0][1] + red[0][2] + red[0][3]);
+  if (!ft_fold_arrive(cnt, gridDim.x, reinterpret_cast<volatile unsigned*>(&red[1][0]))) return;
+  const int nblocks = (int)gridDim.x;
   double s = 0.0, n = 0.0;
   for (int i = threadIdx.x; i < nblocks; i += 256) s += partial[i];
   for (int b = threadIdx.x; b < B; b += 256) {
@@ -633,7 +630,7 @@
   return ft_check_launch("cross_entropy_bwd");
 }
 
-size_t ft_masked_l1_workspace(void) { return 1024 * sizeof(double); }
+size_t ft_masked_l1_workspace(void) { return ft_fold_ws_bytes(1024 * sizeof(double)); }
 
 int ft_masked_l1_fwd(const float* x, const float* target, const long* lens, float* loss, float* inv_denom, int B,
                      int C, int T, void* workspace, size_t workspace_bytes, void* stream) {
@@ -643,10 +640,8 @@
   int nb = ft_cdiv(total, 256 * 8);
   if (nb > 1024) nb = 1024;
   if (nb < 1) nb = 1;
-  hipLaunchKernelGGL(ft_masked_l1_partial_kernel, dim3(nb), dim3(256), 0, (hipStream_t)stream, x, target, lens, B, C, T,
-                     (double*)workspace);
-  hipLaunchKernelGGL(ft_masked_l1_finalize_kernel, dim3(1), dim3(256), 0, (hipStream_t)stream,
-                     (const double*)workspace, nb, lens, B, C, T, loss, inv_denom);
+  hipLaunchKernelGGL(ft_masked_l1_kernel, dim3(nb), dim3(256), 0, (hipStream_t)stream, x, target, lens, B, C, T,
+                     (double*)workspace, ft_fold_counters(workspace, workspace_bytes), loss, inv_denom);
   return ft_check_launch("masked_l1_fwd");
 }
 
diff --git a/forwardtacotron_amd/csrc/ft_fold.h b/forwardtacotron_amd/csrc/ft_fold.h
--- /dev/null
+++ b/forwardtacotron_amd/csrc/ft_fold.h
@@ -0,0 +1,35 @@
+#pragma once
+#include "ft_common.h"
+
+constexpr unsigned FT_FOLD_COUNTERS = 4096;
+constexpr size_t FT_FOLD_BYTES = (size_t)FT_FOLD_COUNTERS * sizeof(unsigned);
+
+static inline size_t ft_fold_tail() { return FT_FOLD_BYTES + 16; }
+static inline size_t ft_fold_ws_bytes(size_t payload) { return ((payload + 15) & ~(size_t)15) + ft_fold_tail(); }
+static inline unsigned* ft_fold_counters(void* workspace, size_t workspace_bytes) {
+  return (unsigned*)(((uintptr_t)workspace + workspace_bytes - FT_FOLD_BYTES) & ~(uintptr_t)15);
+}
+
+__device__ __forceinline__ void ft_fold_store(double* p, double v) {
+  __hip_atomic_store(reinterpret_cast<unsigned long long*>(p), (unsigned long long)__double_as_longlong(v),
+                     __ATOMIC_RELAXED, __HIP_MEMORY_SCOPE_AGENT);
+}
+
+__device__ __forceinline__ bool ft_fold_arrive(unsigned* cnt, unsigned arrivals, volatile unsigned* lds_word) {
+  asm volatile("s_waitcnt vmcnt(0)" ::: "memory");
+  __syncthreads();
+  if (threadIdx.x == 0) {
+    const unsigned ticket = __hip_atomic_fetch_add(cnt, 1u, __ATOMIC_RELAXED, __HIP_MEMORY_SCOPE_AGENT);
+    const unsigned last = ticket + 1u == arrivals ? 1u : 0u;
+    if (last) {
+      __hip_atomic_store(cnt, 0u, __ATOMIC_RELAXED, __HIP_MEMORY_SCOPE_AGENT);
+      __builtin_amdgcn_fence(__ATOMIC_ACQUIRE, "agent");
+      asm volatile("s_waitcnt vmcnt(0)" ::: "memory");
+    }
+    *lds_word = last;
+  }
+  __syncthreads();
+  const bool last = *lds_word != 0u;
+  __syncthreads();
+  return last;
+}
diff --git a/forwardtacotron_amd/fastpitch.py b/forwardtacotron_amd/fastpitch.py
--- a/forwardtacotron_amd/fastpitch.py
+++ b/forwardtacotron_amd/fastpitch.py
@@ -375,8 +375,8 @@
     def side_buffer(raw, nbytes):
         key = (dev.index or 0, raw)
         buf = _side_ws.get(key)
-        if buf is None or buf.numel() < nbytes:
-            buf = _side_ws[key] = torch.empty(max(nbytes, 1 << 20), dtype=torch.uint8, device=dev)
+        if buf is None or buf.numel() < nbytes + H.FOLD_TAIL_BYTES:
+            buf = _side_ws[key] = H.alloc_workspace(nbytes, dev)
         return buf
 
     wws = side_buffer(side_raw, _lib.query('ft_fft_block_wgrad_workspace', B, T, d, f, k1, k2))
diff --git a/forwardtacotron_amd/hip.py b/forwardtacotron_amd/hip.py
--- a/forwardtacotron_amd/hip.py
+++ b/forwardtacotron_amd/hip.py
@@ -37,11 +37,18 @@
 _workspaces = {}
 
 
+FOLD_TAIL_BYTES = 32 << 10
+
+
+def alloc_workspace(nbytes: int, device) -> torch.Tensor:
+    return torch.zeros(max(nbytes, 1 << 20) + FOLD_TAIL_BYTES, dtype=torch.uint8, device=device)
+
+
 def workspace(nbytes: int, device) -> torch.Tensor:
     key = (torch.device(device).index or 0, _stream())
     buf = _workspaces.get(key)
-    if buf is None or buf.numel() < nbytes:
-        buf = torch.empty(max(nbytes, 1 << 20), dtype=torch.uint8, device=device)
+    if buf is None or buf.numel() < nbytes + FOLD_TAIL_BYTES:
+        buf = alloc_workspace(nbytes, device)
         _workspaces[key] = buf
     return buf
 
```

Result: no change. 1.015 million (median of 3 runs) (-0.0%).
